# jbelyeu/unfazed

Hardware: AMD Instinct MI355X
Metric: phased DNMs/sec (higher is better)
Workload: dtype u8/int32 (+f64 allele balance); 1 GPU; 100k synthetic SNV/INDEL DNMs, whole-genome sites VCF, --no-extended off (BASELINE configs[2]); staged: H2D of the pre-decoded columns inside the timed region; dnms_per_gpu=100000, sites=20000000, coverage=30x, search_dist=5000, dnm_placement=uniform, read_clusters=67821, alignment_records=186931612, parallelism=dnm-shard x1, no collective

## Files before the change

include/unfazed_hip.h:

```cpp
#ifndef UNFAZED_HIP_H
#define UNFAZED_HIP_H

#include <stddef.h>
#include <stdint.h>

#include "uz_types.h"
#include "uz_bamwalk.h"

#ifdef __cplusplus
extern "C" {
#endif

#define UZ_E_ARG (-1)
#define UZ_E_HIP (-2)
#define UZ_E_NODEVICE (-3)
#define UZ_E_STATE (-4)
#define UZ_E_RANGE (-5)

#define UZ_FIND_WHOLE_REGION 1
#define UZ_FIND_SECOND_WINDOW 2

#define UZ_K_SITE_SCAN 0
#define UZ_K_WINDOW_COUNT 1
#define UZ_K_WINDOW_FILL 2
// ... 22 lines not shown

typedef struct uz_ctx uz_ctx;

int uz_create(int device, uz_ctx **out);
void uz_destroy(uz_ctx *ctx);
const char *uz_last_error(const uz_ctx *ctx);
int uz_sync(uz_ctx *ctx);
int uz_set_params(uz_ctx *ctx, const uz_params *p);

int uz_sites_upload(uz_ctx *ctx, const uz_sites_view *sites, int *sites_id);
int uz_family_upload(uz_ctx *ctx, int sites_id, const uz_family_view *fam, int *fam_id);
int uz_sites_family_upload_async(uz_ctx *ctx, const uz_sites_view *sites, const uz_family_view *fam, int *sites_id, int *fam_id);
int uz_samples_upload(uz_ctx *ctx, int sites_id, const uz_samples_view *samples, int *samples_id);
int uz_families_from_samples(uz_ctx *ctx, int samples_id, int32_t n, const int32_t *kid, const int32_t *dad, const int32_t *mom, int *fam_ids );
int uz_family_fetch(uz_ctx *ctx, int fam_id, uint8_t *gt, uint16_t *cols );
int uz_samples_from_text(uz_ctx *ctx, int sites_id, const uz_vcf_text_view *text, int32_t n_pick, const int32_t *pick, int *samples_id, int64_t *n_unsettled);
int uz_samples_from_bcf(uz_ctx *ctx, int sites_id, const uz_vcf_bcf_view *bcf, int32_t n_pick, const int32_t *pick, int *samples_id, int64_t *n_unsettled);
int uz_samples_unsettled(uz_ctx *ctx, int samples_id, int64_t *site );
int uz_samples_settle(uz_ctx *ctx, int samples_id, int64_t n, const int64_t *site, const uz_samples_view *cells);
int uz_samples_free(uz_ctx *ctx, int samples_id);
int uz_reads_upload(uz_ctx *ctx, const uz_reads_view *reads, int *reads_id);
int uz_reads_upload_packed(uz_ctx *ctx, const uz_reads_packed_view *reads, int *reads_id);
int uz_reads_wait(uz_ctx *ctx, int reads_id);
int uz_reads_headers(uz_ctx *ctx, int reads_id, int32_t *start, int32_t *end, int32_t *tlen, int32_t *mate, uint32_t *qname);
int uz_reads_columns(uz_ctx *ctx, int reads_id, int64_t sizes[4], uint32_t *fm, uint16_t *l_seq, uint16_t *n_cigar, uint32_t *cigar_off, uint32_t *sq_off,
                     uint32_t *qoff, uint32_t *cigar, uint8_t *seq4, uint32_t *qlow);
int uz_reads_marks(uz_ctx *ctx, int reads_id, uint16_t *umask, uint8_t *nlow);
int uz_bgzf_inflate(uz_ctx *ctx, const uint8_t *comp, int64_t comp_bytes, int64_t n_blocks, const int64_t *in_off, const int64_t *out_off,
                    uint8_t *out, int repeat, double *kernel_ms);
int uz_bgzf_inflate_to_host(uz_ctx *ctx, const uint8_t *comp, int64_t comp_bytes, int64_t n_blocks, const int64_t *in_off, const int64_t *out_off,
                            uint8_t *out);
int uz_bam_walk(uz_ctx *ctx, const uint8_t *comp, int64_t comp_bytes, int64_t n_blocks, const int64_t *in_off, const int64_t *out_off, const int64_t *blk_coff,
                const uint32_t *blk_crc ,
                int32_t n_tasks, const int32_t *task, int64_t n_spans, const int64_t *span, int64_t n_reach, const int32_t *reach, int64_t n_fetch,
                const int32_t *fetch, int *walk_id, int64_t *n_desc);
#define UZ_HEAD_NONE 0
#define UZ_HEAD_DONE 1
#define UZ_HEAD_END 2
#define UZ_HEAD_BAD 3
int uz_head_walk(uz_ctx *ctx, int *head_id, int32_t n_files, const uint8_t *comp, int64_t comp_bytes, int64_t n_blocks, const int64_t *in_off,
                 const int32_t *isize, const uint32_t *crc, const int64_t *blk_first, const int64_t *start, const int64_t *want, const int64_t *have,
                 int64_t *taken, int64_t *cursor, int32_t *state);
int uz_head_rank(uz_ctx *ctx, int head_id, int32_t readlen, const int64_t *k, uint32_t *a, uint32_t *b);
int uz_head_fetch(uz_ctx *ctx, int head_id, int32_t file, int32_t *out, int64_t cap, int64_t *n);
int uz_head_free(uz_ctx *ctx, int head_id);
int uz_crc32_blocks(uz_ctx *ctx, const uint8_t *data, int64_t n_blocks, const int64_t *off, const uint32_t *want, int64_t *first_bad);
int uz_bam_walk_many(uz_ctx *ctx, const uint8_t *comp, int64_t comp_bytes, int64_t n_blocks, const int64_t *in_off, const int64_t *out_off, const int64_t *blk_coff,
                     const uint32_t *blk_crc, int32_t n_tasks, const int32_t *task, int64_t n_spans, const int64_t *span, int64_t n_reach, const int32_t *reach,
                     int64_t n_fetch, const int32_t *fetch, int32_t n_files, const int64_t *file_base, const int32_t *ref_base, const uint64_t *salt1,
                     const uint32_t *salt2, int *walk_id, int64_t *n_desc);
int uz_reads_files(uz_ctx *ctx, int reads_id, int32_t n_files, const int32_t *ref_base, int64_t *rec_first, int64_t *name_first);
int uz_bam_walk_fetch(uz_ctx *ctx, int walk_id, uz_walk_desc *desc, int64_t *d_first, int32_t *d_flags, int64_t *d_walked);
int uz_bam_walk_release(uz_ctx *ctx, int walk_id);
int uz_bam_walk_flags(uz_ctx *ctx, int walk_id, int32_t *d_flags, int64_t *d_walked);
int uz_bam_join(uz_ctx *ctx, int walk_id, int32_t n_host, const int32_t *h_flags, int32_t n_ref, int all_bases, const uz_walk_desc *xdesc, int64_t n_x, const uint8_t *xaux,
                int64_t xaux_bytes, const int32_t *look_tid, int64_t n_look, const int32_t *need_jtask, int64_t *n_need, int64_t totals[8]);
int uz_bam_join_needs(uz_ctx *ctx, int walk_id, uz_need_rec *need);
int uz_bam_join_fetch(uz_ctx *ctx, int walk_id, uint64_t *voff, uint32_t *qname, int32_t *mate, uint8_t *bases, uz_kept_rec *kept, int64_t *contig_off, int32_t *max_span);
int uz_reads_from_walk(uz_ctx *ctx, int walk_id, int32_t min_base_qual, int want_names, int *reads_id, int64_t totals[8]);
int uz_reads_names(uz_ctx *ctx, int reads_id, const uint32_t *ids, int64_t n, int64_t *off ,
                   const uint8_t **bytes );
int uz_walk_slot_stats(uz_ctx *ctx, int64_t out[8]);
int uz_walk_reserve(uz_ctx *ctx, int n_slots);
int uz_reads_from_bam(uz_ctx *ctx, int walk_id, const uz_kept_rec *kept, int64_t n, const uint8_t *aux, int64_t aux_bytes, const int64_t *contig_off,
                      const int32_t *max_span, int32_t n_contigs, int64_t n_cigar_total, int64_t n_row_units, int64_t n_seq_units, uint32_t n_qnames,
                      int32_t min_base_qual, uint8_t *names_out ,
                      int64_t names_bytes, int *reads_id);
int uz_pinned_alloc(size_t bytes, void **out);
void uz_pinned_free(void *p);
int uz_sites_adopt_device(uz_ctx *ctx, const uz_sites_view *sites, int *sites_id);
int uz_family_adopt_device(uz_ctx *ctx, int sites_id, const uz_family_view *fam, int *fam_id);
int uz_reads_adopt_device(uz_ctx *ctx, const uz_reads_packed_view *reads, int *reads_id);
int uz_drop_derived(uz_ctx *ctx);
int uz_sites_free(uz_ctx *ctx, int sites_id);
int uz_reads_free(uz_ctx *ctx, int reads_id);

int uz_site_scan(uz_ctx *ctx, int fam_id);
int uz_site_scan_many(uz_ctx *ctx, const int32_t *fam_ids, int32_t n_fam);
int uz_site_classes(uz_ctx *ctx, int fam_id, uint8_t *cls_out );

int uz_find(uz_ctx *ctx, int fam_id, const uz_dnms_view *dnms, int mode,
            int64_t *cand_off , int64_t *het_off );
int uz_find_fetch(uz_ctx *ctx, int32_t *cand_idx, uint8_t *cand_flags, int32_t *het_idx);
int uz_find_cohort(uz_ctx *ctx, const uz_cohort_group *groups, int32_t n_groups, const uz_dnms_view *dnms, int mode,
                   int64_t *cand_off , int64_t *het_off );

int uz_phase(uz_ctx *ctx, int fam_id, int reads_id, const uz_dnms_view *dnms, int find_mode,
             int32_t *status , int32_t *counts ,
             int32_t *origin , int32_t *evidence );
int uz_phase_begin(uz_ctx *ctx, int fam_id, int reads_id, const uz_dnms_view *dnms, int find_mode);
int uz_phase_end(uz_ctx *ctx, int fam_id, int reads_id, const uz_dnms_view *dnms, int find_mode,
                 int32_t *status, int32_t *counts, int32_t *origin, int32_t *evidence);
int uz_phase_cohort(uz_ctx *ctx, const uz_cohort_group *groups, int32_t n_groups, const uz_dnms_view *dnms, int find_mode,
                    int32_t *status, int32_t *counts, int32_t *origin, int32_t *evidence);
int uz_phase_cohort_joined(uz_ctx *ctx, int reads_id, const uz_cohort_group *groups, int32_t n_groups, const int32_t *group_ref_base, const uz_dnms_view *dnms,
                           int find_mode, int32_t *status, int32_t *counts, int32_t *origin, int32_t *evidence);
int uz_phase_votes(uz_ctx *ctx, int64_t *vote_off , int32_t *vote_val);
int uz_phase_groups(uz_ctx *ctx, int64_t *grp_off , int32_t *grp_q);
#define UZ_SIZING_REDUCED_WORDS 263
int uz_phase_sizing_fetch(uz_ctx *ctx, int32_t *bounds , int32_t *pre_win , int32_t *pre_ha ,
                          int32_t *pre_hl , int64_t *reduced );

int uz_bed_rows(uz_ctx *ctx, const uz_bed_view *rows, int verbose, int include_ambiguous, int64_t *off , const uint8_t **bytes);
int uz_bed_rows_lists(uz_ctx *ctx, const uz_bed_view *rows, int verbose, int include_ambiguous, int32_t n_dnms, const int32_t *status,
                      const int64_t *list_off, const int32_t *list_val, uint32_t n_qnames, const uint32_t *name_off, const uint8_t *name_bytes,
                      int32_t evidence_min_ratio, int64_t *off , const uint8_t **bytes);

int uz_vcf_rows(uz_ctx *ctx, const uz_vcf_text_view *text, const int64_t *line_at , const int64_t *ann_off ,
                const int32_t *ann_col, const uint8_t *ann_gt, const int32_t *ann_uops, const int8_t *ann_uet, int64_t *off ,
                const uint8_t **bytes, uint8_t *handed_back );

int uz_bcf_rows(uz_ctx *ctx, const uz_bcf_lines_view *records, int64_t *off , uint64_t *samp_at ,
                const uint8_t **bytes, uint8_t *handed_back );

int uz_bgzf_deflate(uz_ctx *ctx, const uint8_t *data , int64_t n_bytes, int64_t *n_blocks, const uint8_t **bgzf, int64_t *bgzf_bytes,
                    int repeat, double *kernel_ms);

int uz_phase_cnv(uz_ctx *ctx, int fam_id, const uz_dnms_view *dnms, const int32_t *rb_counts, int32_t *cnv_counts ,
                 int32_t *origin , int32_t *evidence , int32_t *etype );
int uz_phase_cnv_cohort(uz_ctx *ctx, const uz_cohort_group *groups, int32_t n_groups, const uz_dnms_view *dnms, const int32_t *rb_counts,
                        int32_t *cnv_counts , int32_t *origin , int32_t *evidence , int32_t *etype );
int uz_phase_cnv_sites(uz_ctx *ctx, int64_t *off , int32_t *pos);

int uz_prof_enable(uz_ctx *ctx, int on);
int uz_prof_reset(uz_ctx *ctx);
int uz_prof_get(uz_ctx *ctx, int kernel, double *total_ms, int64_t *launches);
int uz_prof_units(uz_ctx *ctx, int kernel, int64_t *units);

#ifdef __cplusplus
}
#endif
#endif
```

unfazed_amd/csrc/abi.hip:

```cpp
#include "uz_ctx.hpp"

#include <chrono>
#include <algorithm>
#include <map>
#include <mutex>

void uz_fold_complex(uz_ctx *c, uint8_t *gt, const uint8_t *sflags, int64_t n);
bool uz_site_scan_fresh(const uz_ctx *c, const FamilyDev &f, bool need_cnv);

namespace {

void set_error(uz_ctx *c, const std::string &msg) {
    std::lock_guard<std::mutex> lk(c->err_mu);
    c->err = msg;
}

template <typename F>
int guarded(uz_ctx *c, F &&fn) {
    if (!c) return UZ_E_ARG;
    try {
        (void)hipSetDevice(c->device);
        fn();
        return 0;
    } catch (const UzError &e) {
        set_error(c, e.msg);
        return e.code;
    } catch (const std::exception &e) {
        set_error(c, e.what());
        return UZ_E_ARG;
    } catch (...) {
        set_error(c, "unknown error");
        return UZ_E_ARG;
    }
}

static std::mutex g_pinned_mu;
static std::map<uintptr_t, size_t> g_pinned;
static bool inside_one_pinned_block(const uint8_t *lo, const uint8_t *hi) {
    std::lock_guard<std::mutex> g(g_pinned_mu);
    auto it = g_pinned.upper_bound((uintptr_t)lo);
    if (it == g_pinned.begin()) return false;
    --it;
    return (uintptr_t)lo >= it->first && (uintptr_t)hi <= it->first + it->second;
}

struct SlabPlan {
    int mode = 1;
    const uint8_t *lo = nullptr, *hi = nullptr;
    size_t sum = 0;
    std::vector<const uint8_t *> at;
    uint8_t *dev = nullptr;
    void add(const void *p, size_t bytes) {
        const uint8_t *q = (const uint8_t *)p;
        if (!lo || q < lo) lo = q;
        if (!hi || q + bytes > hi) hi = q + bytes;
        sum += bytes;
        at.push_back(q);
    }
    size_t span() const { return (size_t)(hi - lo); }
    bool worth() const {
        if (at.size() < 2 || span() > sum + sum / 8 + 1024 * at.size()) return false;
        for (const uint8_t *q : at)
            if ((size_t)(q - lo) % 256) return false;
        return inside_one_pinned_block(lo, hi);
    }
};
static thread_local SlabPlan *g_slab = nullptr;
struct SlabScope {
    explicit SlabScope(SlabPlan *p) { g_slab = p; }
    ~SlabScope() { g_slab = nullptr; }
};
static const bool g_slab_off = getenv("UZ_NO_SLAB_COPY") != nullptr;

template <typename T>
const T *h2d(hipStream_t st, T *dst, const T *host, size_t n) {
    if (n) {
        UZ_REQUIRE(host != nullptr, UZ_E_ARG, "null column pointer");
        if (g_slab && g_slab->mode == 1) { g_slab->add(host, n * sizeof(T)); return dst; }
        if (g_slab && g_slab->mode == 2) return reinterpret_cast<const T *>(g_slab->dev + ((const uint8_t *)host - g_slab->lo));
        UZ_HIP(hipMemcpyAsync(dst, host, n * sizeof(T), hipMemcpyHostToDevice, st));
    }
    return dst;
}
// ... 43 lines not shown

void free_family(uz_ctx *c, FamilyDev &f) {
    if (f.ready) { (void)hipEventSynchronize(f.ready); (void)hipEventDestroy(f.ready); f.ready = nullptr; }
    f.pending = false;
    if (f.samples_id >= 0 && f.samples_id < (int)c->samples.size()) c->samples[(size_t)f.samples_id].live_fams--;
    uz_block_put(c, f.block);
    uz_block_put(c, f.wide_block);
    f = FamilyDev();
}
void free_samples(uz_ctx *c, SamplesDev &m) {
    if (m.ready) { (void)hipEventSynchronize(m.ready); (void)hipEventDestroy(m.ready); }
    uz_block_put(c, m.block);
    uz_block_put(c, m.wide_block);
    for (DevBlock &b : m.fam_blocks) uz_block_put(c, b);
    m = SamplesDev();
}
SamplesDev &samples_of(uz_ctx *c, int id) {
    UZ_REQUIRE(id >= 0 && id < (int)c->samples.size() && c->samples[id].live, UZ_E_ARG, "unknown sample table handle");
    return c->samples[id];
}
void free_sites(uz_ctx *c, SitesDev &s) {
    if (s.ready) { (void)hipEventSynchronize(s.ready); (void)hipEventDestroy(s.ready); }
    uz_block_put(c, s.block);
    uz_block_put(c, s.mirror);
    s = SitesDev();
}
void free_reads(uz_ctx *c, ReadsDev &r) {
    if (r.built) { (void)hipEventSynchronize(r.built); (void)hipEventDestroy(r.built); }
    if (r.ready) (void)hipEventDestroy(r.ready);
    uz_block_put(c, r.block);
    uz_block_put(c, r.mirror);
    r = ReadsDev();
}

struct Carver {
    uint8_t *base;
    size_t off = 0;
    explicit Carver(uint8_t *b) : base(b) {}
    template <typename T>
    T *take(size_t n) {
        off = (off + 255) & ~(size_t)255;
        T *p = base ? reinterpret_cast<T *>(base + off) : nullptr;
        off += (n ? n : 1) * sizeof(T) + 64;
        return p;
    }
};

template <typename F>
void samples_from_records(uz_ctx *c, int sites_id, int64_t n_sites, int32_t n_pick, int *id, int64_t *n_unsettled, F parse) {
    size_t chunk = (size_t)32 << 20;
    if (const char *e = getenv("UZ_VCF_CHUNK_BYTES")) {
        const long long v = atoll(e);
        if (v > 0) chunk = (size_t)v;
    }
    chunk = std::min<size_t>(chunk, (size_t)1 << 31);
    const size_t n = (size_t)n_sites, ns = (size_t)n_pick;
    SamplesDev m;
    m.live = true; m.sites_id = sites_id; m.n_samples = n_pick; m.n_wide = 0;
    m.stride = (n + 64 + 255) & ~(size_t)255;
    for (int pass = 0; pass < 2; pass++) {
        Carver cv(pass ? m.block.p : nullptr);
        m.gt = cv.take<uint8_t>(ns * m.stride);
        m.rd = cv.take<uint16_t>(ns * m.stride); m.ad = cv.take<uint16_t>(ns * m.stride); m.gq = cv.take<uint16_t>(ns * m.stride);
        if (!pass) m.block = uz_block_get(c, cv.off + 256);
    }
    try {
        parse(m, chunk);
    } catch (...) { uz_block_put(c, m.block); throw; }
    m.need_settle = !m.unsettled.empty();
    *n_unsettled = (int64_t)m.unsettled.size();
    const int k = new_slot(c->samples);
    c->samples[(size_t)k] = m;
    *id = k;
}

}

template <typename W>
__global__ __launch_bounds__(256) void k_copy(W *__restrict__ dst, const W *__restrict__ src, size_t n) {
    for (size_t i = (size_t)blockIdx.x * 256 + threadIdx.x; i < n; i += (size_t)gridDim.x * 256) dst[i] = src[i];
}
void uz_kcopy(uz_ctx *c, void *dst, const void *src, size_t bytes) {
    if (!bytes) return;
    const uintptr_t a = (uintptr_t)dst | (uintptr_t)src | (uintptr_t)bytes;
    auto grid = [](size_t n) { return dim3((unsigned)std::min<size_t>((n + 255) / 256, 1024)); };
    if (a % 16 == 0) hipLaunchKernelGGL(k_copy<uint4>, grid(bytes / 16), dim3(256), 0, c->stream, (uint4 *)dst, (const uint4 *)src, bytes / 16);
    else if (a % 4 == 0) hipLaunchKernelGGL(k_copy<uint32_t>, grid(bytes / 4), dim3(256), 0, c->stream, (uint32_t *)dst, (const uint32_t *)src, bytes / 4);
    else hipLaunchKernelGGL(k_copy<uint8_t>, grid(bytes), dim3(256), 0, c->stream, (uint8_t *)dst, (const uint8_t *)src, bytes);
    UZ_HIP(hipGetLastError());
}

__global__ __launch_bounds__(1024) void k_scan_len(int64_t n, const uint32_t *__restrict__ len, uint32_t add, int64_t *__restrict__ off) {
    __shared__ unsigned long long wave_sum[16];
    __shared__ unsigned long long carry_s;
    const uint32_t t = threadIdx.x, l = t & 63u, wv = t >> 6;
    if (t == 0) carry_s = 0;
    __syncthreads();
    for (int64_t base = 0; base < n; base += 1024) {
        const int64_t i = base + t;
        const unsigned long long v = i < n ? (unsigned long long)len[i] + add : 0ull;
        unsigned long long x = v;
#pragma unroll
        for (uint32_t d = 1; d < 64; d <<= 1) {
            const unsigned long long y = (unsigned long long)__shfl_up((long long)x, d, 64);
            if (l >= d) x += y;
        }
        if (l == 63) wave_sum[wv] = x;
        __syncthreads();
        unsigned long long before = carry_s;
        for (uint32_t k = 0; k < wv; k++) before += wave_sum[k];
        if (i < n) off[i] = (int64_t)(before + x - v);
        __syncthreads();
        if (t == 1023) carry_s = before + x;
        __syncthreads();
    }
    if (t == 0) off[n] = (int64_t)carry_s;
}
void uz_len_scan(uz_ctx *c, hipStream_t st, int64_t n, const uint32_t *len, uint32_t add, int64_t *off) {
    hipLaunchKernelGGL(k_scan_len, dim3(1), dim3(1024), 0, st, n, len, add, off);
    UZ_HIP(hipGetLastError());
}

DevBlock uz_block_get(uz_ctx *c, size_t bytes) {
    int best = -1;
    for (size_t i = 0; i < c->block_pool.size(); i++)
        if (c->block_pool[i].cap >= bytes && (best < 0 || c->block_pool[i].cap < c->block_pool[best].cap)) best = (int)i;
    if (best >= 0 && c->block_pool[best].cap <= 2 * bytes + (1 << 20)) {
        DevBlock b = c->block_pool[best];
        c->block_pool.erase(c->block_pool.begin() + best);
        return b;
    }
    DevBlock b;
    b.cap = bytes + bytes / 16 + 4096;
    UZ_HIP(hipMalloc((void **)&b.p, b.cap));
    return b;
}
void uz_block_put(uz_ctx *c, DevBlock b) {
    if (!b.p) return;
    c->block_pool.push_back(b);
    while (c->block_pool.size() > 64) {
        size_t k = 0;
        for (size_t i = 1; i < c->block_pool.size(); i++)
            if (c->block_pool[i].cap < c->block_pool[k].cap) k = i;
        (void)hipFree(c->block_pool[k].p);
        c->block_pool.erase(c->block_pool.begin() + k);
    }
}

void uz_prof_begin(uz_ctx *c, int kernel, hipEvent_t *a, hipEvent_t *b) {
    *a = *b = nullptr;
    if (!(c->prof_mask >> kernel & 1u)) return;
    for (hipEvent_t *e : {a, b}) {
        if (!c->event_pool.empty()) { *e = c->event_pool.back(); c->event_pool.pop_back(); }
        else UZ_HIP(hipEventCreate(e));
    }
    UZ_HIP(hipEventRecord(*a, c->stream));
}
void uz_prof_end(uz_ctx *c, int kernel, hipEvent_t a, hipEvent_t b) {
    if (!a) return;
    (void)hipEventRecord(b, c->stream);
    c->prof_pending.push_back(ProfPending{kernel, a, b});
}
void uz_prof_drain(uz_ctx *c) {
    for (auto &p : c->prof_pending) {
        float ms = 0;
        if (hipEventSynchronize(p.b) == hipSuccess && hipEventElapsedTime(&ms, p.a, p.b) == hipSuccess) {
            c->prof[p.kernel].total_ms += ms;
            c->prof[p.kernel].launches += 1;
        }
        c->event_pool.push_back(p.a);
        c->event_pool.push_back(p.b);
// ... 1453 lines not shown
        std::lock_guard<std::mutex> g(g_pinned_mu);
        g_pinned.erase((uintptr_t)p);
    }
    (void)hipHostFree(p);
}

int uz_drop_derived(uz_ctx *c) {
    return guarded(c, [&] {
        for (auto &f : c->fams) f.cls_valid = false;
        find_forget(c, -1);
    });
}

int uz_sites_free(uz_ctx *c, int sites_id) {
    return guarded(c, [&] {
        SitesDev &s = sites_of(c, sites_id);
        UZ_HIP(hipStreamSynchronize(c->stream));
        for (size_t k = 0; k < c->fams.size(); k++)
            if (c->fams[k].live && c->fams[k].sites_id == sites_id) { find_forget(c, (int)k); free_family(c, c->fams[k]); }
        for (auto &m : c->samples)
            if (m.live && m.sites_id == sites_id) free_samples(c, m);
        free_sites(c, s);
    });
}
int uz_reads_free(uz_ctx *c, int reads_id) {
    return guarded(c, [&] {
        ReadsDev &r = reads_of(c, reads_id);
        if (r.ready) UZ_HIP(hipEventSynchronize(r.ready));
        if (r.built) UZ_HIP(hipEventSynchronize(r.built));
        UZ_HIP(hipStreamSynchronize(c->stream));
        const bool member = std::find(c->cohort_ids.begin(), c->cohort_ids.end(), reads_id) != c->cohort_ids.end();
        if (reads_id == c->cohort_reads) { c->cohort_reads = -1; c->cohort_ids.clear(); }
        else if (member && c->cohort_reads >= 0) {
            free_reads(c, c->reads[(size_t)c->cohort_reads]);
            c->cohort_reads = -1;
            c->cohort_ids.clear();
        }
        free_reads(c, r);
    });
}

int uz_site_scan(uz_ctx *c, int fam_id) {
    return guarded(c, [&] {
        FamilyDev &f = fam_of(c, fam_id);
        uz_launch_site_scan(c, f, sites_of(c, f.sites_id), !f.het_only);
    });
}

int uz_site_scan_many(uz_ctx *c, const int32_t *fam_ids, int32_t n_fam) {
    return guarded(c, [&] {
        UZ_REQUIRE(n_fam >= 0 && (n_fam == 0 || fam_ids != nullptr), UZ_E_ARG, "bad family list");
        if (n_fam == 0) return;
        std::vector<FamilyDev *> fams;
        for (int32_t k = 0; k < n_fam; k++) {
            FamilyDev &f = fam_of(c, fam_ids[k]);
            refuse_het_only(f, "uz_site_scan_many");
            UZ_REQUIRE(f.sites_id == fam_of(c, fam_ids[0]).sites_id, UZ_E_ARG, "the families of one cohort scan must share a sites table");
            for (int32_t j = 0; j < k; j++) UZ_REQUIRE(fam_ids[j] != fam_ids[k], UZ_E_ARG, "family listed twice");
            fams.push_back(&f);
        }
        uz_launch_site_scan_many(c, fams.data(), n_fam, sites_of(c, fams[0]->sites_id), true);
    });
}

int uz_site_classes(uz_ctx *c, int fam_id, uint8_t *out) {
    return guarded(c, [&] {
        FamilyDev &f = fam_of(c, fam_id);
        SitesDev &s = sites_of(c, f.sites_id);
        UZ_REQUIRE(out != nullptr, UZ_E_ARG, "null output");
        const bool cnv = !f.het_only;
        if (!uz_site_scan_fresh(c, f, cnv)) uz_launch_site_scan(c, f, s, cnv);
        if (s.n) UZ_HIP(hipMemcpyAsync(out, f.cls, (size_t)s.n, hipMemcpyDeviceToHost, c->stream));
        UZ_HIP(hipStreamSynchronize(c->stream));
        if (f.het_only) uz_check_upload_flag(c);
    });
}

int uz_find(uz_ctx *c, int fam_id, const uz_dnms_view *d, int mode, int64_t *cand_off, int64_t *het_off) {
    return guarded(c, [&] {
        FamilyDev &f = fam_of(c, fam_id);
        SitesDev &s = sites_of(c, f.sites_id);
        UZ_REQUIRE(d != nullptr && d->n >= 0, UZ_E_ARG, "bad DNM view");
        c->phase_valid = false;
        const bool cnv = (mode & UZ_FIND_WHOLE_REGION) != 0;
        if (cnv) refuse_het_only(f, "a whole-region find");
        if (!uz_site_scan_fresh(c, f, cnv)) uz_launch_site_scan(c, f, s, cnv);
        uz_stage_dnms(c, d);
        const FindKey key = find_key_of(c, fam_id, mode, d);
        find_target(c);
        uz_launch_find(c, f, s, mode);
        if (f.het_only) uz_check_upload_flag(c);
        find_done(c, key);
        c->find_fam = fam_id;
        if (cand_off) memcpy(cand_off, c->cand_off_h.data(), ((size_t)d->n + 1) * sizeof(int64_t));
        if (het_off) memcpy(het_off, c->het_off_h.data(), ((size_t)d->n + 1) * sizeof(int64_t));
    });
}

int uz_find_fetch(uz_ctx *c, int32_t *cand_idx, uint8_t *cand_flags, int32_t *het_idx) {
    return guarded(c, [&] {
        UZ_REQUIRE(c->find_valid, UZ_E_STATE, "uz_find_fetch before uz_find");
        const bool pinned = (!cand_idx || !c->n_cand || inside_one_pinned_block((const uint8_t *)cand_idx, (const uint8_t *)(cand_idx + c->n_cand))) &&
                            (!cand_flags || !c->n_cand || inside_one_pinned_block(cand_flags, cand_flags + c->n_cand)) &&
                            (!het_idx || !c->n_het || inside_one_pinned_block((const uint8_t *)het_idx, (const uint8_t *)(het_idx + c->n_het)));
        if (pinned) {
            if (cand_idx && c->n_cand) uz_kcopy(c, cand_idx, c->cand_idx.p, (size_t)c->n_cand * sizeof(int32_t));
            if (cand_flags && c->n_cand) uz_kcopy(c, cand_flags, c->cand_flags.p, (size_t)c->n_cand);
            if (het_idx && c->n_het) uz_kcopy(c, het_idx, c->het_idx.p, (size_t)c->n_het * sizeof(int32_t));
            UZ_HIP(hipStreamSynchronize(c->stream));
            return;
        }
        if (cand_idx && c->n_cand)
            UZ_HIP(hipMemcpyAsync(cand_idx, c->cand_idx.p, (size_t)c->n_cand * sizeof(int32_t), hipMemcpyDeviceToHost, c->stream));
        if (cand_flags && c->n_cand)
            UZ_HIP(hipMemcpyAsync(cand_flags, c->cand_flags.p, (size_t)c->n_cand, hipMemcpyDeviceToHost, c->stream));
        if (het_idx && c->n_het)
            UZ_HIP(hipMemcpyAsync(het_idx, c->het_idx.p, (size_t)c->n_het * sizeof(int32_t), hipMemcpyDeviceToHost, c->stream));
        UZ_HIP(hipStreamSynchronize(c->stream));
    });
}

static void phase_whole(uz_ctx *c, int fam_id, int reads_id, const uz_dnms_view *d, int find_mode, int32_t *status, int32_t *counts, int32_t *origin,
                        int32_t *evidence, bool defer) {
    FamilyDev &f = fam_of(c, fam_id);
    SitesDev &s = sites_of(c, f.sites_id);
    ReadsDev &r = reads_of(c, reads_id);
    UZ_REQUIRE(d != nullptr, UZ_E_ARG, "null DNM view");
    UZ_REQUIRE(!(find_mode & UZ_FIND_WHOLE_REGION), UZ_E_ARG, "the read stage runs on SNV / breakpoint windows");
    c->phase_valid = false;
    c->phase_qbase.clear();
    static const bool trace = getenv("UZ_PHASE_HOST_TRACE") != nullptr;
    const auto t0 = std::chrono::steady_clock::now();
    auto us = [&] { return std::chrono::duration<double, std::micro>(std::chrono::steady_clock::now() - t0).count(); };
    if (!uz_site_scan_fresh(c, f, false)) uz_launch_site_scan(c, f, s, false);
    const double t_scan0 = us();
    uz_stage_dnms(c, d);
    const double t_stage0 = us() - t_scan0, t_scan = us();
    const FindKey key = find_key_of(c, fam_id, find_mode, d);
    const double t_key = us() - t_scan, t_stage = us();
    const bool have = find_recall(c, key);
    if (!have) find_target(c);
    if (!have) {
        uz_launch_find(c, f, s, find_mode, false);
        find_done(c, key);
    }
    const double t_find = us();
    c->find_fam = fam_id;
    uz_launch_phase(c, f, s, r, status, counts, origin, evidence, defer);
    if (trace) fprintf(stderr, "[uz] read-stage call, host us: site scan queued %.0f | stage dnms %.0f | key %.0f | find %.0f | phase (launches, waits, results) %.0f\n", t_scan0,
                       t_stage0, t_key, t_find - t_stage, us() - t_find);
}
int uz_phase(uz_ctx *c, int fam_id, int reads_id, const uz_dnms_view *d, int find_mode, int32_t *status,
             int32_t *counts, int32_t *origin, int32_t *evidence) {
    return guarded(c, [&] {
        UZ_REQUIRE(!c->phase_open, UZ_E_STATE, "uz_phase: a batch is still open (uz_phase_end)");
        phase_whole(c, fam_id, reads_id, d, find_mode, status, counts, origin, evidence, false);
    });
}
int uz_phase_begin(uz_ctx *c, int fam_id, int reads_id, const uz_dnms_view *d, int find_mode) {
    return guarded(c, [&] {
        UZ_REQUIRE(!c->phase_open, UZ_E_STATE, "uz_phase_begin: the batch before this one is still open (uz_phase_end)");
        phase_whole(c, fam_id, reads_id, d, find_mode, nullptr, nullptr, nullptr, nullptr, true);
        c->phase_open = true;
    });
}
int uz_phase_end(uz_ctx *c, int fam_id, int reads_id, const uz_dnms_view *d, int find_mode, int32_t *status, int32_t *counts, int32_t *origin,
                 int32_t *evidence) {
    return guarded(c, [&] {
        UZ_REQUIRE(c->phase_open, UZ_E_STATE, "uz_phase_end without uz_phase_begin");
        c->phase_open = false;
        if (uz_finish_phase(c, status, counts, origin, evidence)) return;
        phase_whole(c, fam_id, reads_id, d, find_mode, status, counts, origin, evidence, false);
    });
}

struct CohortMode {
    uz_ctx *c;
    explicit CohortMode(uz_ctx *c_) : c(c_) { c->cohort_on = true; }
    ~CohortMode() { c->cohort_on = false; }
};
struct ZeroSearchDist {
    uz_ctx *c;
    const int32_t sd;
    explicit ZeroSearchDist(uz_ctx *c_) : c(c_), sd(c_->P.search_dist) { c->P.search_dist = 0; }
    ~ZeroSearchDist() { c->P.search_dist = sd; }
};

struct CohortBatch {
    const uz_cohort_group *groups = nullptr; int32_t n_groups = 0;
    const uz_dnms_view *d = nullptr; bool cnv = false;
    FamilyDev *f0 = nullptr; SitesDev *s = nullptr;
    std::vector<int32_t> fam;
    std::vector<uint8_t *> cls;
    std::vector<FamilyDev *> stale;
};

static CohortBatch cohort_batch(uz_ctx *c, const uz_cohort_group *groups, int32_t n_groups, const uz_dnms_view *d, bool cnv) {
    UZ_REQUIRE(groups && n_groups > 0 && d && d->n >= 0, UZ_E_ARG, "bad cohort batch");
    CohortBatch b;
    b.groups = groups; b.n_groups = n_groups; b.d = d; b.cnv = cnv;
    b.f0 = &fam_of(c, groups[0].fam_id);
// ... 618 lines not shown
```

unfazed_amd/csrc/k_reads.hip:

```cpp
#include "uz_ctx.hpp"
#include "phase_body.hpp"

#include <algorithm>
#include <chrono>
#include <cstdio>
#include <cstdlib>

#define UZ_TRACE(name) do { if (getenv("UZ_TRACE")) { (void)hipStreamSynchronize(c->stream); fprintf(stderr, "[uz] before %s\n", name); fflush(stderr); } } while (0)

namespace {


#ifndef UZ_BW_LANES
#define UZ_BW_LANES 16
#endif
#ifndef UZ_BW_MIN_WAVES
#define UZ_BW_MIN_WAVES 1
#endif
#ifndef UZ_BW_STAGE
#define UZ_BW_STAGE 64
#endif
template <int GL, typename F>
__device__ __forceinline__ int32_t grp_lower_bound(F ld, int32_t a, int32_t b, int32_t v, int lane, int gbase) {
    constexpr int SH = GL == 64 ? 6 : GL == 32 ? 5 : GL == 16 ? 4 : GL == 8 ? 3 : GL == 4 ? 2 : GL == 2 ? 1 : 0;
    const unsigned long long gmask = GL == 64 ? ~0ull : ((1ull << GL) - 1ull);
    while (a < b) {
        const int32_t chunk = ((b - a) + GL - 1) >> SH;
        const int32_t q = a + lane * chunk;
        const bool below = q < b && ld(q) < v;
        const int cnt = __popcll((__ballot(below) >> gbase) & gmask);
        const int32_t a0 = a;
        if (cnt > 0) a = a0 + (cnt - 1) * chunk + 1;
        if (cnt < GL && a0 + cnt * chunk < b) b = a0 + cnt * chunk;
    }
    return a;
}
__global__ __launch_bounds__(256, UZ_BW_MIN_WAVES) void k_phase_bounds(PhaseArgs a, int32_t *bounds ) {
    constexpr int GL = UZ_BW_LANES, NCH = 2 * UZ_BW_SITES;
    static_assert(GL == 1 || GL == 2 || GL == 4 || GL == 8 || GL == 16 || GL == 32 || GL == 64, "a group is a power of two inside a wavefront");
    __shared__ int32_t s_stage[256 / GL][UZ_BW_STAGE];
    const int64_t g = ((int64_t)blockIdx.x * blockDim.x + threadIdx.x) / GL;
    const int lane = threadIdx.x & (GL - 1), gbase = (threadIdx.x & 63) & ~(GL - 1);
    const int d = g < a.n ? (int)g : a.n - 1;
    long long tp = 0;
    int mh = 0;
    int32_t *b = bounds + 5 * (size_t)d;
    if (g < a.n) {
        const int nc = (int)(a.cand_off[d + 1] - a.cand_off[d]), nh = (int)(a.het_off[d + 1] - a.het_off[d]);
        if (lane == 0) {
            b[0] = b[1] = b[4] = 0;
            b[2] = nh; b[3] = nc;
            for (int k = 0; k < 4; k++) a.pre_win[4 * d + k] = 0;
        }
        const RD &R = a.R;
        const int tid = a.rcontig[d];
        const bool tid_ok = tid >= 0 && tid < R.n_contigs;
        const int32_t clo = tid_ok ? (int32_t)R.contig_off[tid] : 0, chi = tid_ok ? (int32_t)R.contig_off[tid + 1] : 0;
        if (nc > 0 && (!R.mid || !tid_ok || chi - clo <= 128)) {
            uz_phase_bounds_w(a, d, b, lane, GL, tp, mh,
                              [&R, clo, chi](const long long (&v)[NCH], const bool (&on)[NCH], long long (&r)[NCH]) { uz_lower_bounds_c<NCH>(R, clo, chi, v, on, r); });
        } else if (nc > 0) {
            const long long span = R.max_span[tid];
            const bool point = a.vartype[d] == UZ_VT_POINT;
            long long vmin_ = 0x7FFFFFFFLL;
            if (point) {
                const long long position = a.dstart[d];
                vmin_ = ((a.dflags[d] & UZ_DF_FETCH_FALLBACK) ? position : position - 1) - span;
            }
            if (!a.no_extended && nh > 0) {
                const long long v0 = (long long)a.spos[a.het_idx[a.het_off[d]]] - span;
                if (v0 < vmin_) vmin_ = v0;
            }
            const int32_t vmin = uz_clamp_i32(vmin_);
            int32_t lo0 = clo, hi0 = chi;
            if (R.coarse && chi - clo > 8192) {
                const int32_t kl = (clo + 4095) >> 12, kh = chi >> 12;
                const int32_t *cx = R.coarse;
                const int32_t a0 = grp_lower_bound<GL>([cx](int32_t k) { return cx[k]; }, kl, kh > kl ? kh : kl, vmin, lane, gbase);
                if (kh > kl) { lo0 = a0 > kl ? ((a0 - 1) << 12) : clo; hi0 = a0 < kh ? (a0 << 12) : chi; }
            }
            const int32_t *mx = R.mid;
            const int32_t kl_m = (clo + 63) >> 6, kh_m = chi >> 6;
            const int32_t ml = (lo0 + 63) >> 6, mhi = hi0 >> 6;
            int32_t lo1 = lo0;
            if (mhi > ml) {
                const int32_t m0 = grp_lower_bound<GL>([mx](int32_t k) { return mx[k]; }, ml, mhi, vmin, lane, gbase);
                if (m0 > ml) lo1 = (m0 - 1) << 6;
            }
            int32_t s0 = (lo1 + 63) >> 6;
            if (s0 < kl_m) s0 = kl_m;
            int32_t s_end = s0 + UZ_BW_STAGE < kh_m ? s0 + UZ_BW_STAGE : kh_m;
            if (s_end < s0) s_end = s0;
            const int32_t cnt = s_end - s0;
            int32_t *sm = s_stage[threadIdx.x / GL];
            for (int i = lane; i < cnt; i += GL) sm[i] = mx[s0 + i];
            __builtin_amdgcn_fence(__ATOMIC_RELEASE, "wavefront");
            __builtin_amdgcn_wave_barrier();
            __builtin_amdgcn_fence(__ATOMIC_ACQUIRE, "wavefront");
            const bool whole = s_end == kh_m;
            uz_phase_bounds_w(a, d, b, lane, GL, tp, mh, [&R, clo, chi, sm, s0, cnt, lo1, whole](const long long (&v_)[NCH], const bool (&on)[NCH], long long (&r)[NCH]) {
                int32_t x[NCH], y[NCH], v[NCH];
                bool far[NCH], any_far = false;
#pragma unroll
                for (int s = 0; s < NCH; s++) { v[s] = uz_clamp_i32(v_[s]); x[s] = 0; y[s] = on[s] ? cnt : 0; }
                uz_lb_level<NCH>([sm](int32_t k) { return sm[k]; }, x, y, v, 0);
#pragma unroll
                for (int s = 0; s < NCH; s++) {
                    const int32_t k = x[s];
                    far[s] = on[s] && k == cnt && !whole;
                    any_far |= far[s];
                    x[s] = k > 0 ? ((s0 + k - 1) << 6) : lo1;
                    y[s] = (on[s] && !far[s]) ? (k < cnt ? ((s0 + k) << 6) : chi) : x[s];
                    if (!on[s]) x[s] = y[s] = clo;
                }
                if (R.mid8) uz_mid8_refine<NCH>(R.mid8, x, y, v);
                const RecA *rx = R.ra;
                uz_lb_level<NCH>([rx](int32_t k) { return rx[k].start; }, x, y, v, clo);
#pragma unroll
                for (int s = 0; s < NCH; s++) r[s] = x[s];
                if (any_far) {
                    long long rf[NCH];
                    uz_lower_bounds_c<NCH>(R, clo, chi, v_, far, rf);
#pragma unroll
                    for (int s = 0; s < NCH; s++) if (far[s]) r[s] = rf[s];
                }
            });
        }
    }
#pragma unroll
    for (int o = GL >> 1; o > 0; o >>= 1) {
        tp += __shfl_xor(tp, o, GL);
        const int m2 = __shfl_xor(mh, o, GL);
        mh = m2 > mh ? m2 : mh;
    }
    if (g < a.n && lane == 0) {
        b[1] = (int32_t)(tp > 0x7FFFFFF0LL ? 0x7FFFFFF0LL : tp);
        b[4] = mh;
    }
}

#ifndef UZ_PHASE_PARTS
#define UZ_PHASE_PARTS 8
#endif
#ifndef UZ_PHASE_MIN_WAVES
#define UZ_PHASE_MIN_WAVES 4
#endif
template <bool LDS>
__global__ __launch_bounds__(WG_NT, LDS ? UZ_PHASE_MIN_WAVES : 5) void k_phase(PhaseArgs a_by_value) {
    __shared__ WgSharedT<LDS ? 1 : WG_SORT_LDS_CAP> sh;
    extern __shared__ __attribute__((aligned(16))) uint8_t uz_lds_arena[];
    (void)a_by_value;
    const PhaseArgsK ap = (PhaseArgsK)__builtin_amdgcn_kernarg_segment_ptr();
    uint8_t *const scr_base = uz_g(ap->scratch) + (size_t)blockIdx.x * ap->scratch_per_wg;
#ifdef UZ_PHASE_TIMING
    if (threadIdx.x < 24) sh.tick[threadIdx.x] = 0;
    struct TickFlush {
        decltype(sh) *s; unsigned long long *t;
        __device__ ~TickFlush() { __syncthreads(); if (threadIdx.x < 24 && s->tick[threadIdx.x]) atomicAdd(&t[threadIdx.x], s->tick[threadIdx.x]); }
    } tick_flush{&sh, uz_g(ap->timing)};
#endif
    const bool from_list = ap->from_list != 0;
    int part = from_list ? ap->cursor_slot : (int)(blockIdx.x % UZ_PHASE_PARTS);
    int tried = 0;
    for (;;) {
        __syncthreads();
        if (threadIdx.x == 0) {
            const int k = atomicAdd(uz_g(ap->work_cursor) + 16 * part, 1);
            if (from_list) sh.bcast[0] = k < *uz_g(ap->src_count) ? uz_g(ap->src_list)[k] : -1;
            else {
                const int n = ap->n;
                const int lo = (int)((long long)n * part / UZ_PHASE_PARTS), hi = (int)((long long)n * (part + 1) / UZ_PHASE_PARTS);
                sh.bcast[0] = lo + k < hi ? lo + k : -1;
            }
        }
        __syncthreads();
        const int d = sh.bcast[0];
        if (d < 0) {
            if (from_list || ++tried >= UZ_PHASE_PARTS) break;
            part = (part + 1) % UZ_PHASE_PARTS;
            continue;
        }
        if (uz_phase_dnm<LDS>(ap, scr_base, &sh, LDS ? uz_lds_arena : nullptr, d)) {
            if (threadIdx.x == 0) uz_g(ap->retry_list)[atomicAdd(uz_g(ap->retry_count), 1)] = d;
        }
    }
}

struct PhaseState {
    DevBuf<uint8_t> scratch;
    DevBuf<int32_t> bounds, bounds_red, res, cursor, pool, list_len, pre_win, pre_h, retry;
    DevBuf<long long> list_start;
    unsigned long long *pool_cursor = nullptr;
    DevBuf<unsigned int> need_count;
    int32_t *bounds_h = nullptr;
    size_t bounds_h_cap = 0;
    int32_t *res_h = nullptr;
    size_t res_h_cap = 0;
    bool spec_valid = false;
    Caps spec_caps = {0, 0, 0, 0, 0, 0};
    int spec_arena = 0, spec_arena2 = 0;
    double spec_sumP_per_dnm = 0.0;
    long long spec_runs = 0, spec_misses = 0;
    hipEvent_t bounds_ready = nullptr;
    int n_cus = 0;
    std::vector<long long> list_start_h;
    std::vector<int32_t> list_len_h;
    bool have_lists = false;
    int32_t n = 0;
    int64_t n_het = 0;
    bool pending = false;
    Caps pend_caps = {0, 0, 0, 0, 0, 0};
    size_t pend_pool_cap = 0;
    int pend_want_lists = 0;
    bool force_exact = false;
};

RD make_rd(const ReadsDev &r) {
    RD R;
    R.ra = (const RecA *)r.rec_a; R.rb = (const RecB *)r.rec_b; R.fm = r.fm;
    R.contig_off = r.contig_off; R.max_span = r.max_span; R.n_contigs = r.n_contigs;
    R.cigar = r.cigar; R.seq4 = r.seq4; R.qlow = r.qlow; R.qoff = r.qoff; R.nlow = r.nlow; R.umask = r.umask; R.qs = r.qs; R.min_map_qual = 0; R.coarse = r.coarse; R.mid = r.mid; R.mid8 = r.mid8;
    R.err = nullptr;
    return R;
}

int next_pow2(long long v) {
    long long p = 1;
    while (p < v) p <<= 1;
    return (int)p;
}

}

void uz_phase_state_free(uz_ctx *c) {
    PhaseState *st = (PhaseState *)c->phase_state;
// ... 49 lines not shown
            left &= ~m;
        }
        bin = -1;
    }
    for (int o = 32; o > 0; o >>= 1) {
        mA = max(mA, __shfl_xor(mA, o, 64)); mT = max(mT, __shfl_xor(mT, o, 64)); mH = max(mH, __shfl_xor(mH, o, 64)); mC = max(mC, __shfl_xor(mC, o, 64));
        mM = max(mM, __shfl_xor(mM, o, 64)); sumP += __shfl_xor(sumP, o, 64); active += __shfl_xor(active, o, 64);
    }
    const int w = threadIdx.x >> 6;
    if ((threadIdx.x & 63) == 0) {
        part[w][0] = (unsigned long long)mA; part[w][1] = (unsigned long long)mT; part[w][2] = (unsigned long long)mH; part[w][3] = (unsigned long long)mC;
        part[w][4] = (unsigned long long)mM; part[w][5] = (unsigned long long)sumP; part[w][6] = (unsigned long long)active;
    }
    __syncthreads();
    if (threadIdx.x == 0) {
        unsigned long long r[7];
        for (int k = 0; k < 7; k++) { r[k] = part[0][k]; for (int q = 1; q < 4; q++) r[k] = k < 5 ? max(r[k], part[q][k]) : r[k] + part[q][k]; }
        atomicMax(&out->mA, (int32_t)r[0]); atomicMax(&out->mT, (int32_t)r[1]); atomicMax(&out->mH, (int32_t)r[2]); atomicMax(&out->mC, (int32_t)r[3]);
        atomicMax(&out->mM, r[4]); atomicAdd(&out->sumP, r[5]); atomicAdd(&out->active, (int32_t)r[6]);
    }
    if (hist[threadIdx.x]) atomicAdd(&out->hist[threadIdx.x], hist[threadIdx.x]);
}
static Sizes phase_exact_sizes(const BoundsRed *br, int32_t n) {
    const long long mA = br->mA, mT = br->mT, mH = br->mH, mC = br->mC, mM = (long long)br->mM, sumP = (long long)br->sumP;
    Sizes z;
    z.caps.A = (int32_t)mA; z.caps.T = (int32_t)mT; z.caps.H = (int32_t)mH; z.caps.C = (int32_t)mC;
    z.caps.I = (int32_t)(4 * mA);
    z.caps.M = next_pow2(std::min<long long>(std::max<long long>(mM, 2), 1 << 20));
    z.sumP = sumP;
    z.arena = arena_env;
    if (z.arena < 0) {
        const int32_t *hist = br->hist;
        const int32_t active = br->active;
        int u = 16, seen = 0, umax = 16;
        for (int k = 0; k < 256; k++) if (hist[k]) umax = k;
        for (int k = 0; k < 256; k++) {
            seen += hist[k];
            if (hist[k]) u = std::max(u, k);
            if ((long long)seen * 1000 >= (long long)active * arena_permille) break;
        }
        z.arena = std::min(u * 256, 62 * 1024);
        z.arena2 = std::min(std::max(2 * z.arena, umax * 256 + 1024), 62 * 1024);
    } else
        z.arena2 = std::min(2 * z.arena, 62 * 1024);
    return z;
}

void uz_launch_phase(uz_ctx *c, FamilyDev &f, const SitesDev &s, ReadsDev &r, int32_t *status, int32_t *counts,
                     int32_t *origin, int32_t *evidence, bool defer) {
    if (!c->phase_state) c->phase_state = new PhaseState();
    PhaseState *st = (PhaseState *)c->phase_state;
    const int32_t n = c->dn.n;
    st->n = n;
    st->have_lists = false;
    st->pending = false;
    c->phase_n = n;
    if (n <= 0) { c->phase_valid = true; return; }
    static const bool host_trace = getenv("UZ_PHASE_HOST_TRACE") != nullptr;
    const auto host_t0 = std::chrono::steady_clock::now();
    auto host_us = [&] { return std::chrono::duration<double, std::micro>(std::chrono::steady_clock::now() - host_t0).count(); };
    double t_queued = 0, t_synced = 0, t_sized = 0;
    uz_reads_ready_for_threshold(c, r, "the reads table");

    PhaseArgs a;
    memset(&a, 0, sizeof(a));
    a.n = n;
    a.min_gt_qual = c->P.min_gt_qual; a.readlen = c->P.readlen; a.no_extended = c->P.no_extended;
    a.read_goal = c->P.read_goal; a.evidence_min_ratio = c->P.evidence_min_ratio; a.split_error_margin = c->P.split_error_margin;
    a.cutoff = c->dn.cutoff;
    a.cutoff_d = c->cohort_on ? c->dn_cutoff.p : nullptr;
    a.spos = s.pos; a.sref = s.ref_base; a.salt = s.alt_base;
    a.cand_off = c->cand_off.p; a.het_off = c->het_off.p;
    a.cand_idx = c->cand_idx.p; a.het_idx = c->het_idx.p; a.cand_flags = c->cand_flags.p;
    a.rcontig = c->dn.rcontig.p; a.dstart = c->dn.start.p; a.dend = c->dn.end.p; a.dflags = c->dn.dflags.p; a.vartype = c->dn.vartype.p;
    a.allele_off = c->dn.allele_off.p; a.alleles = c->dn.alleles.p;
    a.R = make_rd(r);
    a.R.err = c->hflags + 1;
    a.R.min_map_qual = c->P.min_map_qual;

    st->bounds.ensure((size_t)5 * n);
    st->pre_win.ensure((size_t)4 * n); st->pre_h.ensure(2 * ((size_t)c->n_het + 1));
    a.pre_win = st->pre_win.p; a.pre_ha = st->pre_h.p; a.pre_hl = st->pre_h.p + (size_t)c->n_het + 1;
    st->n_het = c->n_het;
    UZ_HIP(hipMemsetAsync(st->pre_h.p, 0, 2 * ((size_t)c->n_het + 1) * sizeof(int32_t), c->stream));
    {
        const unsigned nb = (unsigned)(((int64_t)n * UZ_BW_LANES + 255) / 256);
        ProfScope ps(c, UZ_K_SIZING);
        UZ_TRACE("k_phase_bounds");
        hipLaunchKernelGGL(k_phase_bounds, dim3(nb), dim3(256), 0, c->stream, a, st->bounds.p);
        UZ_HIP(hipGetLastError());
    }
    if (st->bounds_h_cap < sizeof(BoundsRed) / sizeof(int32_t)) {
        if (st->bounds_h) (void)hipHostFree(st->bounds_h);
        st->bounds_h = nullptr;
        st->bounds_h_cap = sizeof(BoundsRed) / sizeof(int32_t) + 64;
        UZ_HIP(hipHostMalloc((void **)&st->bounds_h, st->bounds_h_cap * sizeof(int32_t), hipHostMallocDefault));
    }
    st->bounds_red.ensure(sizeof(BoundsRed) / sizeof(int32_t) + 16);
    UZ_HIP(hipMemsetAsync(st->bounds_red.p, 0, sizeof(BoundsRed), c->stream));
    hipLaunchKernelGGL(k_bounds_reduce, dim3((unsigned)std::max(1, std::min(UZ_BR_BLOCKS, (n + 255) / 256))), dim3(256), 0, c->stream, (const int32_t *)st->bounds.p, n,
                       reinterpret_cast<BoundsRed *>(st->bounds_red.p));
    UZ_HIP(hipGetLastError());
    const BoundsRed *const bh_own = reinterpret_cast<const BoundsRed *>(st->bounds_h);
    uz_kcopy(c, st->bounds_h, st->bounds_red.p, sizeof(BoundsRed));
    if (!st->bounds_ready) UZ_HIP(hipEventCreateWithFlags(&st->bounds_ready, hipEventDisableTiming));
    UZ_HIP(hipEventRecord(st->bounds_ready, c->stream));
    auto check_upload_flags = [&] { uz_check_upload_flag(c); };
    auto exact_sizes = [&](const BoundsRed *bh) { return phase_exact_sizes(bh, n); };
    if (st->n_cus <= 0) {
        hipDeviceProp_t prop;
        UZ_HIP(hipGetDeviceProperties(&prop, c->device));
        st->n_cus = prop.multiProcessorCount;
    }
    static const bool no_spec = getenv("UZ_PHASE_NO_SPEC") != nullptr;
    const bool hooks = getenv("UZ_TEST_CAP_T") || getenv("UZ_TEST_PHASE_ARENA");
    bool speculative = st->spec_valid && !no_spec && !hooks && !st->force_exact;
    st->force_exact = false;
    const size_t res_ints = (size_t)7 * n + ((7 * (size_t)n) & 1);
    st->res.ensure(res_ints + 4);
    st->pool_cursor = (unsigned long long *)(st->res.p + res_ints);
    st->cursor.ensure(16 * (UZ_PHASE_PARTS + 2) + 32);
    st->retry.ensure(2 * ((size_t)n + 16));
    int32_t *const retry1_list = st->retry.p, *const retry2_list = st->retry.p + (size_t)n + 16;
    int32_t *const retry1 = st->cursor.p + 16 * (UZ_PHASE_PARTS + 2), *const retry2 = retry1 + 16;
    a.retry_count = retry1; a.retry_list = retry1_list;
    a.from_list = 0; a.cursor_slot = 0; a.src_count = nullptr; a.src_list = nullptr;
    a.status = st->res.p; a.counts = st->res.p + n; a.origin = st->res.p + (size_t)5 * n; a.evidence = st->res.p + (size_t)6 * n;
    a.work_cursor = st->cursor.p;
    a.want_lists = uz_want_lists;
    st->list_start.ensure(n); st->list_len.ensure((size_t)6 * n);
    a.pool_cursor = st->pool_cursor;
    a.list_start = st->list_start.p; a.list_len = st->list_len.p;
#ifdef UZ_PHASE_TIMING
    static DevBuf<unsigned long long> timing;
    timing.ensure(32);
    UZ_HIP(hipMemsetAsync(timing.p, 0, 32 * sizeof(unsigned long long), c->stream));
    a.timing = timing.p;
#endif
    {
        const size_t need = (size_t)7 * n + 16;
        if (st->res_h_cap < need) {
            if (st->res_h) (void)hipHostFree(st->res_h);
            st->res_h = nullptr;
            st->res_h_cap = need + (size_t)n;
            UZ_HIP(hipHostMalloc((void **)&st->res_h, st->res_h_cap * sizeof(int32_t), hipHostMallocDefault));
        }
    }
    int32_t *const hres = st->res_h;
    unsigned long long *const hused = (unsigned long long *)(hres + (size_t)7 * n + ((7 * (size_t)n) & 1));
    for (int round = 0; round < 2; round++) {
        Sizes z;
        if (speculative) {
            z.caps = st->spec_caps; z.arena = st->spec_arena; z.arena2 = st->spec_arena2;
            z.sumP = (long long)(st->spec_sumP_per_dnm * (double)n) + 4096;
        } else {
            UZ_HIP(hipEventSynchronize(st->bounds_ready));
            check_upload_flags();
            z = exact_sizes(bh_own);
            if (const char *e = getenv("UZ_TEST_CAP_T")) {
                const int32_t t = (int32_t)atoi(e);
                if (t < z.caps.T) z.caps.T = t;
            }
        }
        const Caps caps = z.caps;
        int arena_used = z.arena;
        ScrOff so_hbm;
        const size_t per_wg = uz_scratch_layout(caps, a.so, true), per_wg_hbm = uz_scratch_layout(caps, so_hbm, false);
        if (const char *e = getenv("UZ_TEST_PHASE_ARENA")) {
            const int t = atoi(e);
            if (t >= 0 && t < arena_used) arena_used = t;
        }
        int wgs_per_cu;
        {
            static const int wgs_env = [] { const char *e = getenv("UZ_PHASE_WGS_PER_CU"); return e ? atoi(e) : 0; }();
            const int by_lds = (160 * 1024) / (arena_used + (int)sizeof(WgSharedT<1>) + 512);
            const int by_regs = UZ_PHASE_MIN_WAVES * 4 / (WG_NT / 64);
            wgs_per_cu = wgs_env > 0 ? wgs_env : std::max(1, std::min(by_lds, by_regs));
            if (arena_env < 0 && wgs_env <= 0) {
                const int room = ((160 * 1024) / wgs_per_cu - (int)sizeof(WgSharedT<1>) - 512) & ~255;
                if (room > arena_used && !getenv("UZ_TEST_PHASE_ARENA")) arena_used = std::min(room, 62 * 1024);
            }
        }
        a.lds_arena_bytes = arena_used;
        int grid = st->n_cus * wgs_per_cu;
        if (grid > n) grid = n;
        const size_t budget = (size_t)8 << 30;
        while (grid > 1 && (size_t)grid * per_wg > budget) grid /= 2;
        int grid_hbm = std::min(grid, 8 * st->n_cus);
        while (grid_hbm > 1 && (size_t)grid_hbm * per_wg_hbm > budget) grid_hbm /= 2;
        st->scratch.ensure(std::max((size_t)grid * per_wg, (size_t)grid_hbm * per_wg_hbm));
        a.scratch = st->scratch.p; a.scratch_per_wg = per_wg; a.caps = caps;
        size_t pool_cap = (size_t)std::min<long long>(4 * z.sumP + 1024, (long long)1 << 31);
        st->pool.ensure(pool_cap);
        a.pool = st->pool.p; a.pool_cap = pool_cap;
        for (int attempt = 0; attempt < 4; attempt++) {
            UZ_HIP(hipMemsetAsync(st->cursor.p, 0, (16 * (UZ_PHASE_PARTS + 2) + 32) * sizeof(int32_t), c->stream));
            UZ_HIP(hipMemsetAsync(st->pool_cursor, 0, 2 * sizeof(unsigned long long), c->stream));
            {
                ProfScope ps(c, UZ_K_PHASE);
                UZ_TRACE("k_phase");
                hipLaunchKernelGGL((k_phase<true>), dim3((unsigned)grid), dim3(WG_NT), (size_t)a.lds_arena_bytes, c->stream, a);
                UZ_HIP(hipGetLastError());
                PhaseArgs a2 = a;
                a2.from_list = 1; a2.cursor_slot = UZ_PHASE_PARTS; a2.src_count = retry1; a2.src_list = retry1_list;
                a2.retry_count = retry2; a2.retry_list = retry2_list;
                a2.lds_arena_bytes = getenv("UZ_TEST_PHASE_ARENA") ? arena_used
                                                                    : std::max(arena_used, std::min(z.arena2, 62 * 1024));
                const int per_cu2 = std::max(1, (160 * 1024) / (a2.lds_arena_bytes + (int)sizeof(WgSharedT<1>) + 512));
                hipLaunchKernelGGL((k_phase<true>), dim3((unsigned)std::min(grid, per_cu2 * st->n_cus)), dim3(WG_NT), (size_t)a2.lds_arena_bytes, c->stream, a2);
                UZ_HIP(hipGetLastError());
                PhaseArgs a3 = a2;
                a3.cursor_slot = UZ_PHASE_PARTS + 1; a3.src_count = retry2; a3.src_list = retry2_list;
                a3.so = so_hbm; a3.scratch_per_wg = per_wg_hbm;
                hipLaunchKernelGGL((k_phase<false>), dim3((unsigned)grid_hbm), dim3(WG_NT), 0, c->stream, a3);
                UZ_HIP(hipGetLastError());
            }
            UZ_TRACE("after k_phase");
            *hused = 0;
            uz_kcopy(c, hres, st->res.p, res_ints * sizeof(int32_t) + sizeof(unsigned long long));
            int32_t *const hretry = (int32_t *)(hused + 1);
            *hretry = 0;
            uz_kcopy(c, hretry, retry2, sizeof(int32_t));
            if (defer && speculative) {
                st->pending = true;
                st->pend_caps = caps; st->pend_pool_cap = a.pool_cap; st->pend_want_lists = a.want_lists;
                return;
            }
            if (host_trace) t_queued = host_us();
            UZ_HIP(hipStreamSynchronize(c->stream));
            if (host_trace) t_synced = host_us();
            if (speculative) check_upload_flags();
            if (c->hflags[1]) {
                const int f = c->hflags[1];
                c->hflags[1] = 0;
                throw UzError{UZ_E_STATE, f == 4 ? "the read stage asked for a base of a record whose bases were staged as a list (bl_*), and the list does not hold it: the fetch points that staged the table do not cover this batch"
                                        : f == 3 ? "the read stage asked for a base (or its quality bit) in a 32-base unit that was not staged (umask): the fetch points that staged the table do not cover this batch"
                                        : f == 2 ? "the read stage asked for a base-quality bit of a record staged without its quality row (more than 10 low-quality bases, or no bases): such a record can never pass goodread -- the staging rule and the kernel disagree"
                                                 : "the read stage asked for the bases of a record staged without them (UZ_AUX_NO_SEQ): the selection that staged the table does not cover this batch's fetches"};
            }
            const unsigned long long used = *hused;
            c->prof[UZ_K_PHASE].last_units = (int64_t)*(const int32_t *)(hused + 1);
            if (!a.want_lists || used <= a.pool_cap) break;
            pool_cap = (size_t)used + 1024;
            st->pool.ensure(pool_cap);
            a.pool = st->pool.p; a.pool_cap = pool_cap;
        }
        const Sizes real = exact_sizes(bh_own);
        if (host_trace) t_sized = host_us();
        auto room = [](int32_t v) { return (int32_t)std::min<long long>((long long)v + v / 8 + 8, 0x3FFFFFFF); };
        st->spec_caps.A = room(real.caps.A); st->spec_caps.T = room(real.caps.T); st->spec_caps.H = room(real.caps.H); st->spec_caps.C = room(real.caps.C);
        st->spec_caps.I = 4 * st->spec_caps.A;
        st->spec_caps.M = real.caps.M;
        st->spec_arena = real.arena; st->spec_arena2 = real.arena2;
        st->spec_sumP_per_dnm = 1.25 * (double)real.sumP / (double)n;
        st->spec_valid = true;
        static const bool spec_log = getenv("UZ_PHASE_SPEC_LOG") != nullptr;
        if (spec_log)
            fprintf(stderr, "[uz_launch_phase] n %d speculative %d caps A %d T %d H %d C %d M %d arena %d grid %d per_wg %zu pool %zu | real A %d T %d H %d C %d M %d arena %d\n", n,
                    (int)speculative, caps.A, caps.T, caps.H, caps.C, caps.M, arena_used, grid, per_wg, pool_cap, real.caps.A, real.caps.T, real.caps.H, real.caps.C, real.caps.M, real.arena);
        if (!speculative) break;
        const bool fits = real.caps.A <= caps.A && real.caps.T <= caps.T && real.caps.H <= caps.H && real.caps.C <= caps.C && real.caps.M <= caps.M;
        st->spec_runs++;
        if (fits) break;
        st->spec_misses++;
        speculative = false;
    }
#ifdef UZ_PHASE_TIMING
    {
        unsigned long long t[32];
        UZ_HIP(hipMemcpy(t, timing.p, sizeof(t), hipMemcpyDeviceToHost));
        const char *nm[17] = {"A.classify", "A.lists+C", "-", "B.overlap", "B.finish", "S.keys", "S.sort", "P.count", "P.scatter", "P.pairs", "D.finder",
                              "E.setup", "E.expand", "E.winners", "E.frontier", "F.join", "F.count"};
        unsigned long long tot = 0;
        for (int k = 0; k < 17; k++) tot += t[k];
        fprintf(stderr, "[phase timing]");
        for (int k = 0; k < 17; k++) fprintf(stderr, " %s %.1f%%", nm[k], 100.0 * (double)t[k] / (double)(tot ? tot : 1));
        fprintf(stderr, " | ticks/DNM %.0f\n", (double)tot / n);
    }
#endif
    if (status) memcpy(status, hres, (size_t)n * sizeof(int32_t));
    if (counts) memcpy(counts, hres + n, (size_t)4 * n * sizeof(int32_t));
    if (origin) memcpy(origin, hres + (size_t)5 * n, (size_t)n * sizeof(int32_t));
    if (evidence) memcpy(evidence, hres + (size_t)6 * n, (size_t)n * sizeof(int32_t));
    st->have_lists = a.want_lists != 0;
    c->phase_valid = true;
    if (host_trace)
        fprintf(stderr, "[uz] uz_launch_phase, host us: everything queued %.0f | waited for the device %.0f | exact sizes %.0f | results copied out %.0f\n", t_queued, t_synced - t_queued,
                t_sized - t_synced, host_us() - t_sized);
}

bool uz_finish_phase(uz_ctx *c, int32_t *status, int32_t *counts, int32_t *origin, int32_t *evidence) {
    PhaseState *st = (PhaseState *)c->phase_state;
    UZ_REQUIRE(st != nullptr, UZ_E_STATE, "uz_phase_end without uz_phase_begin");
    const int32_t n = st->n;
    if (n <= 0) { c->phase_valid = true; return true; }
    int32_t *const hres = st->res_h;
    if (st->pending) {
        st->pending = false;
        UZ_HIP(hipStreamSynchronize(c->stream));
        uz_check_upload_flag(c);
        if (c->hflags[1]) {
            c->hflags[1] = 0;
            st->force_exact = true;
            return false;
        }
// ... 104 lines not shown
```

unfazed_amd/csrc/k_sites.hip:

```cpp
#include "uz_ctx.hpp"

#include <algorithm>
#include <cstdlib>
#include <vector>

namespace {

struct SiteParams {
    int32_t min_gt_qual, min_depth;
    double lo_ref, hi_ref, lo_het, hi_het, lo_alt, hi_alt;
};

__device__ __forceinline__ int dec16(uint32_t v) { return (int)(int16_t)(uint16_t)v; }

#define UZ_AB_T_MIN (-2)
#define UZ_AB_T_MAX 65534
#define UZ_AB_LUT_N (UZ_AB_T_MAX - UZ_AB_T_MIN + 1)
#define UZ_AB_A_MIN (-1)
#define UZ_AB_A_MAX 32767
__device__ __forceinline__ double ab_lo(const SiteParams &P, int gt) { return gt == UZ_HOM_REF ? P.lo_ref : (gt == UZ_HOM_ALT ? P.lo_alt : P.lo_het); }
__device__ __forceinline__ double ab_hi(const SiteParams &P, int gt) { return gt == UZ_HOM_REF ? P.hi_ref : (gt == UZ_HOM_ALT ? P.hi_alt : P.hi_het); }

#define UZ_AB_LDS_T 512
__global__ void k_build_ab_lut(SiteParams P, int2 *lut, uint32_t *small, int *t0_special) {
    const int i = blockIdx.x * blockDim.x + threadIdx.x;
    if (i >= 4 * UZ_AB_LUT_N) return;
    const int gt = i / UZ_AB_LUT_N, t = i % UZ_AB_LUT_N + UZ_AB_T_MIN;
    const double lo = ab_lo(P, gt), hi = ab_hi(P, gt);
    int2 r = make_int2(0x7FFFFFFF, -0x7FFFFFFF);
    if (gt != UZ_GT_UNKNOWN && t >= P.min_depth) {
        if (t > 0) {
            int l = UZ_AB_A_MIN, h = UZ_AB_A_MAX + 1;
            while (l < h) { const int m = l + ((h - l) >> 1); if (lo <= (double)m / (double)t) h = m; else l = m + 1; }
            const int amin = l;
            l = UZ_AB_A_MIN - 1; h = UZ_AB_A_MAX;
            while (l < h) { const int m = l + ((h - l + 1) >> 1); if ((double)m / (double)t <= hi) l = m; else h = m - 1; }
            if (amin <= UZ_AB_A_MAX && l >= UZ_AB_A_MIN) r = make_int2(amin, l);
        } else if (t < 0) {
            int amin = 0x7FFFFFFF, amax = -0x7FFFFFFF;
            for (int a = -1; a <= 0; a++) {
                const double ab = (double)a / (double)t;
                if (lo <= ab && ab <= hi) { if (a < amin) amin = a; if (a > amax) amax = a; }
            }
            r = make_int2(amin, amax);
        } else {
            const double pinf = 1.0 / 0.0, ninf = -1.0 / 0.0;
            const bool neg = lo <= ninf && ninf <= hi, pos = lo <= pinf && pinf <= hi;
            if (neg && pos) { r = make_int2(-1, 1); atomicOr(t0_special, 1); }
            else if (neg) r = make_int2(-1, -1);
            else if (pos) r = make_int2(1, 1);
        }
    }
    lut[i] = r;
    if (t - UZ_AB_T_MIN < UZ_AB_LDS_T) {
        const int lo16 = r.x > 32767 ? 32767 : r.x, hi16 = r.y < -32768 ? -32768 : r.y;
        small[gt * UZ_AB_LDS_T + (t - UZ_AB_T_MIN)] = ((uint32_t)lo16 & 0xFFFFu) | ((uint32_t)hi16 << 16);
    }
}

template <bool T0>
__device__ __forceinline__ bool hq(const SiteParams &P, const int2 *__restrict__ lut, const uint32_t *lds, int gt, int rd, int ad, int gq) {
    const int t = rd + ad;
    const uint32_t ti = (uint32_t)(t - UZ_AB_T_MIN);
    int amin, amax;
    if (ti < UZ_AB_LDS_T) {
        const uint32_t e = lds[gt * UZ_AB_LDS_T + ti];
        amin = (int)(int16_t)(e & 0xFFFFu);
        amax = (int)(int16_t)(e >> 16);
    } else {
        const int2 b = lut[gt * UZ_AB_LUT_N + ti];
        amin = b.x; amax = b.y;
    }
    bool ok = (gq >= P.min_gt_qual) & (ad >= amin) & (ad <= amax);
    if (T0) ok &= !((t == 0) & (ad == 0));
    return ok;
}

__device__ __forceinline__ bool hq_wide(const SiteParams &P, int gt, int rd, int ad, int gq) {
    if (gt == UZ_GT_UNKNOWN) return false;
    const long long t = (long long)rd + (long long)ad;
    if (gq < P.min_gt_qual || t < (long long)P.min_depth) return false;
    const double ab = (double)ad / (double)t;
    return ab_lo(P, gt) <= ab && ab <= ab_hi(P, gt);
// ... 319 lines not shown
                        }
                    }
                    nc += __popcll(bc); nh += __popcll(bh);
                }
                if (!FILL && lane == 0) { a.range[4 * (int64_t)d + 2 * k] = lo; a.range[4 * (int64_t)d + 2 * k + 1] = hi; }
            }
            nc *= mult; nh *= mult;
        }
    }
    if (!FILL && lane == 0) { cnt_c[d] = (int32_t)nc; cnt_h[d] = (int32_t)nh; }
}

template <bool FILL>
__global__ __launch_bounds__(256) void k_window_region(WinArgs a, int32_t *cnt_c, int32_t *cnt_h, const int64_t *off_c, const int64_t *off_h,
                                                       int32_t *cand_idx, uint8_t *cand_flags, int32_t *het_idx) {
    const int32_t d = (int32_t)(((int64_t)blockIdx.x * blockDim.x + threadIdx.x) >> 6);
    const int lane = threadIdx.x & 63;
    if (d >= a.n) return;
    if (FILL && (off_c[d + 1] > a.cap_c || off_h[d + 1] > a.cap_h)) return;
    int64_t nc = 0, nh = 0;
    const int32_t c = a.contig[d];
    const uint8_t *__restrict__ cls = a.fam_idx ? a.cls_of[a.fam_idx[d]] : a.cls;
    if (c >= 0 && c < a.n_contigs) {
        const int64_t clo = a.contig_off[c], chi = a.contig_off[c + 1];
        const int64_t st = a.start[d], en = a.end[d];
        int64_t w0 = st - a.sd;
        const int64_t w1 = en + a.sd;
        if (w0 < 1) w0 = 1;
        const int vt = a.vartype[d];
        const int mult = a.mult[d];
        const bool small_event = (en - st) < 20;
        int64_t lo, hi;
        if (FILL) { lo = a.range[4 * (int64_t)d]; hi = a.range[4 * (int64_t)d + 1]; }
        else {
            lo = lower_bound_wave(a.pos, clo, chi, w0 - 1, lane);
            hi = lower_bound_wave(a.pos, lo, chi, w1, lane);
            if (lane == 0) { a.range[4 * (int64_t)d] = lo; a.range[4 * (int64_t)d + 1] = hi; }
        }
        const int64_t oc = FILL ? off_c[d] : 0, oh = FILL ? off_h[d] : 0;
        const unsigned long long below = lane ? (~0ULL >> (64 - lane)) : 0ULL;
        for (int64_t b = lo; b < hi; b += 64) {
            const int64_t sidx = b + lane;
            bool is_c = false, is_h = false;
            uint32_t cl = 0, ka = 0;
            if (sidx < hi) {
                cl = cls[sidx];
                const int32_t p = a.pos[sidx];
                if (cl && !(small_event && p >= st && p < en)) {
                    if (vt == UZ_VT_DEL) ka = (cl >> UZ_CL_DEL_SHIFT) & 3;
                    else if (vt == UZ_VT_DUP) ka = (cl >> UZ_CL_DUP_SHIFT) & 3;
                    is_c = ka != 0;
                    is_h = (cl & UZ_CL_HET) != 0;
                }
            }
            const unsigned long long bc = __ballot(is_c), bh = __ballot(is_h);
            if (FILL) {
                if (is_h) for (int r = 0; r < mult; r++) het_idx[oh + (nh + __popcll(bh & below)) * mult + r] = (int32_t)sidx;
                if (is_c) {
                    const uint8_t fl = (uint8_t)(((cl & UZ_CL_ALT_DAD) ? UZ_CF_ALT_DAD : 0) | (ka << UZ_CF_KA_SHIFT));
                    for (int r = 0; r < mult; r++) {
                        const int64_t at = oc + (nc + __popcll(bc & below)) * mult + r;
                        cand_idx[at] = (int32_t)sidx;
                        cand_flags[at] = fl;
                    }
                }
            }
            nc += __popcll(bc); nh += __popcll(bh);
        }
        nc *= mult; nh *= mult;
    }
    if (!FILL && lane == 0) { cnt_c[d] = (int32_t)nc; cnt_h[d] = (int32_t)nh; }
}

__device__ __forceinline__ void scan2_load(int32_t n, int32_t i0, const int32_t *c0, const int32_t *c1, int (&v0)[4], int (&v1)[4]) {
    v0[0] = v0[1] = v0[2] = v0[3] = 0; v1[0] = v1[1] = v1[2] = v1[3] = 0;
    if (i0 + 3 < n) {
        const int4 a = *reinterpret_cast<const int4 *>(c0 + i0), b = *reinterpret_cast<const int4 *>(c1 + i0);
        v0[0] = a.x; v0[1] = a.y; v0[2] = a.z; v0[3] = a.w;
        v1[0] = b.x; v1[1] = b.y; v1[2] = b.z; v1[3] = b.w;
    } else {
        for (int k = 0; k < 4; k++) if (i0 + k < n) { v0[k] = c0[i0 + k]; v1[k] = c1[i0 + k]; }
    }
}
__global__ __launch_bounds__(1024) void k_scan2_sums(int32_t n, const int32_t *c0, const int32_t *c1, int64_t *part ) {
    __shared__ long long wsum[2][16];
    const int t = threadIdx.x, lane = t & 63, wv = t >> 6;
    int v0[4], v1[4];
    scan2_load(n, (int32_t)blockIdx.x * 4096 + 4 * t, c0, c1, v0, v1);
    long long s0 = (long long)v0[0] + v0[1] + v0[2] + v0[3], s1 = (long long)v1[0] + v1[1] + v1[2] + v1[3];
#pragma unroll
    for (int off = 32; off > 0; off >>= 1) { s0 += __shfl_xor(s0, off, 64); s1 += __shfl_xor(s1, off, 64); }
    if (lane == 0) { wsum[0][wv] = s0; wsum[1][wv] = s1; }
    __syncthreads();
    if (t < 2) {
        long long a = 0;
        for (int w = 0; w < 16; w++) a += wsum[t][w];
        part[2 * (size_t)blockIdx.x + t] = a;
    }
}
__global__ __launch_bounds__(1024) void k_scan2(int32_t n, const int32_t *c0, const int32_t *c1, const int64_t *__restrict__ part, int64_t *o0, int64_t *o1) {
    __shared__ int wsum[2][16];
    __shared__ long long csum[2][16];
    const int t = threadIdx.x, lane = t & 63, wv = t >> 6;
    const int32_t i0 = (int32_t)blockIdx.x * 4096 + 4 * t;
    int v0[4], v1[4];
    scan2_load(n, i0, c0, c1, v0, v1);
    long long q0 = 0, q1 = 0;
    for (int b = t; b < (int)blockIdx.x; b += 1024) { q0 += part[2 * (size_t)b]; q1 += part[2 * (size_t)b + 1]; }
#pragma unroll
    for (int off = 32; off > 0; off >>= 1) { q0 += __shfl_xor(q0, off, 64); q1 += __shfl_xor(q1, off, 64); }
    const int s0 = v0[0] + v0[1] + v0[2] + v0[3], s1 = v1[0] + v1[1] + v1[2] + v1[3];
    int in0 = s0, in1 = s1;
#pragma unroll
    for (int off = 1; off < 64; off <<= 1) {
        const int u0 = __shfl_up(in0, off, 64), u1 = __shfl_up(in1, off, 64);
        if (lane >= off) { in0 += u0; in1 += u1; }
    }
    if (lane == 63) { wsum[0][wv] = in0; wsum[1][wv] = in1; }
    if (lane == 0) { csum[0][wv] = q0; csum[1][wv] = q1; }
    __syncthreads();
    int64_t base0 = 0, base1 = 0, pre0 = 0, pre1 = 0, tot0 = 0, tot1 = 0;
#pragma unroll
    for (int w = 0; w < 16; w++) {
        const int a = wsum[0][w], b = wsum[1][w];
        if (w < wv) { pre0 += a; pre1 += b; }
        tot0 += a; tot1 += b;
        base0 += csum[0][w]; base1 += csum[1][w];
    }
    int64_t p0 = base0 + pre0 + (in0 - s0), p1 = base1 + pre1 + (in1 - s1);
    for (int k = 0; k < 4; k++) {
        if (i0 + k < n) { o0[i0 + k] = p0; o1[i0 + k] = p1; }
        p0 += v0[k]; p1 += v1[k];
    }
    if (t == 0 && blockIdx.x == gridDim.x - 1) { o0[n] = base0 + tot0; o1[n] = base1 + tot1; }
}

__global__ __launch_bounds__(256) void k_cnv_count(int32_t n, const int64_t *__restrict__ cand_off, const int32_t *__restrict__ cand_idx,
                                                   const uint8_t *__restrict__ cand_flags, const int32_t *__restrict__ spos,
                                                   const uint8_t *__restrict__ vartype, const int32_t *__restrict__ rb_counts, int ratio,
                                                   int32_t *cnv_counts, int32_t *cnv_pos, int32_t *origin, int32_t *evidence, int32_t *etype) {
    const int32_t d = (int32_t)(((int64_t)blockIdx.x * blockDim.x + threadIdx.x) >> 6);
    const int lane = threadIdx.x & 63;
    if (d >= n) return;
    const int64_t c0 = cand_off[d], c1 = cand_off[d + 1];
    const int vt = vartype[d];
    const bool cnv = vt == UZ_VT_DEL || vt == UZ_VT_DUP;
    int n_dad = 0, n_mom = 0;
    if (cnv) {
        for (int64_t b = c0; b < c1; b += 64) {
            const int64_t i = b + lane;
            bool dad = false, mom = false;
            if (i < c1) {
                const uint32_t fl = cand_flags[i];
                const uint32_t ka = (fl >> UZ_CF_KA_SHIFT) & 3u;
                const bool alt_dad = (fl & UZ_CF_ALT_DAD) != 0;
                const bool is_dad = (ka == UZ_KA_ALT_PARENT) == alt_dad;
                dad = ka != 0 && is_dad; mom = ka != 0 && !is_dad;
            }
            n_dad += __popcll(__ballot(dad)); n_mom += __popcll(__ballot(mom));
        }
        int o_dad = 0, o_mom = 0;
        for (int64_t b = c0; b < c1; b += 64) {
            const int64_t i = b + lane;
            bool dad = false, mom = false;
            int32_t p = 0;
            if (i < c1) {
// ... 351 lines not shown
    UZ_HIP(hipGetLastError());
}

__device__ __forceinline__ uint32_t gt_pack4(uint32_t k, uint32_t d, uint32_t m, uint32_t s) {
    return (k & 0x03030303u) | ((d & 0x03030303u) << 2) | ((m & 0x03030303u) << 4) | ((s & 0x01010101u * UZ_SF_COMPLEX) << 6);
}
__global__ __launch_bounds__(256) void k_family_gt_pack(int64_t n, const uint8_t *__restrict__ gt, size_t stride, const int32_t *__restrict__ trio,
                                                        const uint8_t *__restrict__ sflags, uint8_t *__restrict__ out, size_t out_stride) {
    const size_t t = blockIdx.y;
    const uint8_t *__restrict__ gk = gt + (size_t)trio[3 * t] * stride;
    const uint8_t *__restrict__ gd = gt + (size_t)trio[3 * t + 1] * stride;
    const uint8_t *__restrict__ gm = gt + (size_t)trio[3 * t + 2] * stride;
    uint8_t *__restrict__ o = out + t * out_stride;
    const int64_t n_chunks = (n + 256 * 16 - 1) / (256 * 16);
    for (int64_t chunk = blockIdx.x; chunk < n_chunks; chunk += gridDim.x) {
        const int64_t base = (chunk * 256 + threadIdx.x) * 16;
        if (base >= n) continue;
        if (base + 16 <= n) {
            const uint4 k = *reinterpret_cast<const uint4 *>(gk + base), d = *reinterpret_cast<const uint4 *>(gd + base);
            const uint4 m = *reinterpret_cast<const uint4 *>(gm + base), s = *reinterpret_cast<const uint4 *>(sflags + base);
            *reinterpret_cast<uint4 *>(o + base) = make_uint4(gt_pack4(k.x, d.x, m.x, s.x), gt_pack4(k.y, d.y, m.y, s.y), gt_pack4(k.z, d.z, m.z, s.z),
                                                              gt_pack4(k.w, d.w, m.w, s.w));
        } else {
            for (int64_t i = base; i < n; i++) o[i] = (uint8_t)gt_pack4(gk[i], gd[i], gm[i], sflags[i]);
        }
    }
}
__global__ __launch_bounds__(256) void k_family_wide_gather(int64_t n_wide, const int32_t *__restrict__ wrd, const int32_t *__restrict__ wad,
                                                            const int32_t *__restrict__ trio, int32_t *__restrict__ out) {
    const size_t t = blockIdx.y;
    const int64_t k = (int64_t)blockIdx.x * 256 + threadIdx.x;
    if (k >= n_wide) return;
    int32_t *__restrict__ o = out + t * 6 * (size_t)n_wide;
#pragma unroll
    for (int m = 0; m < 3; m++) {
        const size_t row = (size_t)trio[3 * t + m] * (size_t)n_wide;
        o[(size_t)m * n_wide + k] = wrd[row + k];
        o[(size_t)(3 + m) * n_wide + k] = wad[row + k];
    }
}
void uz_launch_family_pack(uz_ctx *c, const SamplesDev &sm, const SitesDev &s, int32_t n, const int32_t *trio, uint8_t *gt_out, size_t gt_stride, int32_t *wide_out) {
    if (n <= 0) return;
    UZ_REQUIRE((uintptr_t)s.sflags % 16 == 0, UZ_E_ARG, "the site flags of an adopted sites table must be 16-byte aligned for uz_families_from_samples");
    ProfScope ps(c, UZ_K_FAMILY_PACK);
    const int32_t y_max = 65535;
    for (int32_t t0 = 0; t0 < n; t0 += y_max) {
        const int32_t ny = std::min<int32_t>(y_max, n - t0);
        if (s.n > 0) {
            const int64_t n_chunks = (s.n + 256 * 16 - 1) / (256 * 16);
            const int64_t nb = std::max<int64_t>(1, std::min<int64_t>(n_chunks, std::max<int64_t>(4096 / ny, 16)));
            hipLaunchKernelGGL(k_family_gt_pack, dim3((unsigned)nb, (unsigned)ny), dim3(256), 0, c->stream, s.n, (const uint8_t *)sm.gt, sm.stride, trio + 3 * (size_t)t0,
                               (const uint8_t *)s.sflags, gt_out + (size_t)t0 * gt_stride, gt_stride);
            UZ_HIP(hipGetLastError());
        }
        if (sm.n_wide > 0) {
            hipLaunchKernelGGL(k_family_wide_gather, dim3((unsigned)((sm.n_wide + 255) / 256), (unsigned)ny), dim3(256), 0, c->stream, sm.n_wide, (const int32_t *)sm.wide_rd,
                               (const int32_t *)sm.wide_ad, trio + 3 * (size_t)t0, wide_out + (size_t)t0 * 6 * (size_t)sm.n_wide);
            UZ_HIP(hipGetLastError());
        }
    }
}

bool uz_site_scan_fresh(const uz_ctx *c, const FamilyDev &f, bool need_cnv) {
    return f.cls_valid && (f.cls_has_cnv || !need_cnv) && site_params_equal(f.cls_params, c->P);
}

#ifndef UZ_SITE_SPT
#define UZ_SITE_SPT 8
#endif

namespace {

void ensure_ab_lut(uz_ctx *c, const SiteParams &sp) {
    if (c->ab_lut_valid && site_params_equal(c->ab_lut_params, c->P)) return;
    c->ab_lut.ensure((size_t)4 * UZ_AB_LUT_N * 2 + 4 + 4 * UZ_AB_LDS_T);
    int *flag = c->ab_lut.p + (size_t)4 * UZ_AB_LUT_N * 2;
    UZ_HIP(hipMemsetAsync(flag, 0, sizeof(int), c->stream));
    hipLaunchKernelGGL(k_build_ab_lut, dim3((4 * UZ_AB_LUT_N + 255) / 256), dim3(256), 0, c->stream, sp, (int2 *)c->ab_lut.p,
                       (uint32_t *)(flag + 4), flag);
    UZ_HIP(hipGetLastError());
    int special = 0;
    UZ_HIP(hipMemcpyAsync(&special, flag, sizeof(int), hipMemcpyDeviceToHost, c->stream));
    UZ_HIP(hipStreamSynchronize(c->stream));
    c->ab_lut_t0_special = special != 0;
    c->ab_lut_valid = true;
    c->ab_lut_params = c->P;
}

FamPtrs fam_ptrs(const FamilyDev &f) {
    FamPtrs fp;
    fp.gt = f.gt;
    for (int m = 0; m < 3; m++) { fp.rd[m] = f.rd[m]; fp.ad[m] = f.ad[m]; fp.gq[m] = f.gq[m]; }
    return fp;
}

void launch_site_scan(uz_ctx *c, const FamPtrs &fp, uint8_t *cls, int64_t n, bool with_cnv, const FamBatchItem *batch, int n_fam) {
    const SiteParams sp = make_site_params(c->P);
    ensure_ab_lut(c, sp);
    static const int spt = [] { const char *e = getenv("UZ_SITE_SPT"); return e ? atoi(e) : UZ_SITE_SPT; }();
    ProfScope ps(c, UZ_K_SITE_SCAN);
    auto launch = [&](auto kern, int SPT) {
        const int64_t n_chunks = (n + 256 * SPT - 1) / (256 * SPT);
        static const int wgs = [] { const char *e = getenv("UZ_SITE_WGS"); return e ? atoi(e) : 4096; }();
        int64_t nb = n_chunks < wgs ? n_chunks : wgs;
        if (batch && n_fam > 1) {
            const int64_t per = (wgs + n_fam - 1) / n_fam;
            nb = std::max<int64_t>(1, std::min<int64_t>(n_chunks, std::max<int64_t>(per, 16)));
        }
        hipLaunchKernelGGL(kern, dim3((unsigned)nb, (unsigned)(batch ? n_fam : 1)), dim3(256), 0, c->stream, fp, cls, n, sp,
                           (const int2 *)c->ab_lut.p, (const uint32_t *)(c->ab_lut.p + (size_t)4 * UZ_AB_LUT_N * 2 + 4), batch);
    };
    const bool t0 = c->ab_lut_t0_special;
#define UZ_K1_PICK(SPTV, BATCHV)                                                                                              \
    do {                                                                                                                        \
        if (with_cnv) { if (t0) launch(k_site_scan<SPTV, true, true, BATCHV>, SPTV); else launch(k_site_scan<SPTV, true, false, BATCHV>, SPTV); } \
        else { if (t0) launch(k_site_scan<SPTV, false, true, BATCHV>, SPTV); else launch(k_site_scan<SPTV, false, false, BATCHV>, SPTV); }        \
    } while (0)
    if (batch) { if (spt == 16) UZ_K1_PICK(16, true); else UZ_K1_PICK(8, true); }
    else { if (spt == 16) UZ_K1_PICK(16, false); else UZ_K1_PICK(8, false); }
#undef UZ_K1_PICK
    UZ_HIP(hipGetLastError());
}

}

static void launch_site_scan_wide(uz_ctx *c, FamilyDev &f, bool with_cnv) {
    if (f.n_wide <= 0) return;
    const SiteParams P = make_site_params(c->P);
    const unsigned nb = (unsigned)((f.n_wide + 255) / 256);
    if (with_cnv) hipLaunchKernelGGL(k_site_scan_wide<true>, dim3(nb), dim3(256), 0, c->stream, fam_ptrs(f), f.cls, f.n_wide, f.wide_site, f.wide_depth, P);
    else hipLaunchKernelGGL(k_site_scan_wide<false>, dim3(nb), dim3(256), 0, c->stream, fam_ptrs(f), f.cls, f.n_wide, f.wide_site, f.wide_depth, P);
    UZ_HIP(hipGetLastError());
}

static void check_gq_clamp(const uz_ctx *c, const FamilyDev &f) {
    UZ_REQUIRE(!f.gq_clamped || c->P.min_gt_qual <= 254, UZ_E_STATE,
               "this family was staged with eight-bit genotype qualities (clamped at 254): --min-gt-qual above 254 needs the 16-bit columns");
}
static void check_het_only(const FamilyDev &f, bool with_cnv) {
    UZ_REQUIRE(!(with_cnv && f.het_only), UZ_E_STATE,
               "this family was staged in the het form (genotype columns of the kid-het sites only): the DEL / DUP classes need every site's columns");
}
void uz_launch_site_scan(uz_ctx *c, FamilyDev &f, const SitesDev &s, bool with_cnv) {
    check_gq_clamp(c, f);
    check_het_only(f, with_cnv);
    if (s.n > 0) { launch_site_scan(c, fam_ptrs(f), f.cls, s.n, with_cnv, nullptr, 1); launch_site_scan_wide(c, f, with_cnv); }
    f.cls_has_cnv = with_cnv;
    f.cls_valid = true;
    f.cls_params = c->P;
}

void uz_launch_site_scan_many(uz_ctx *c, FamilyDev *const *fams, int n_fam, const SitesDev &s, bool with_cnv) {
    if (n_fam <= 0) return;
    for (int k = 0; k < n_fam; k++) { check_gq_clamp(c, *fams[k]); check_het_only(*fams[k], with_cnv); }
    if (s.n > 0) {
        std::vector<FamBatchItem> items((size_t)n_fam);
        for (int k = 0; k < n_fam; k++) { items[(size_t)k].f = fam_ptrs(*fams[k]); items[(size_t)k].cls = fams[k]->cls; }
        c->fam_batch.ensure((size_t)n_fam * sizeof(FamBatchItem));
        UZ_HIP(hipMemcpyAsync(c->fam_batch.p, items.data(), items.size() * sizeof(FamBatchItem), hipMemcpyHostToDevice, c->stream));
        UZ_HIP(hipStreamSynchronize(c->stream));
        launch_site_scan(c, items[0].f, items[0].cls, s.n, with_cnv, (const FamBatchItem *)c->fam_batch.p, n_fam);
        for (int k = 0; k < n_fam; k++) launch_site_scan_wide(c, *fams[k], with_cnv);
    }
    for (int k = 0; k < n_fam; k++) {
        fams[k]->cls_has_cnv = with_cnv;
        fams[k]->cls_valid = true;
        fams[k]->cls_params = c->P;
    }
}

void uz_launch_find(uz_ctx *c, FamilyDev &f, const SitesDev &s, int mode, bool host_offsets) {
    const int32_t n = c->dn.n;
    c->cnt_c.ensure((size_t)n + 1);
    c->cnt_h.ensure((size_t)n + 1);
    c->cand_off.ensure((size_t)n + 1);
    c->het_off.ensure((size_t)n + 1);
    if (host_offsets || n <= 0) { c->cand_off_h.assign((size_t)n + 1, 0); c->het_off_h.assign((size_t)n + 1, 0); }
    else { c->cand_off_h.resize((size_t)n + 1); c->het_off_h.resize((size_t)n + 1); }
    c->n_cand = c->n_het = 0;
    if (n > 0) {
        WinArgs a;
        a.n = n;
        a.contig = c->dn.contig.p; a.start = c->dn.start.p; a.end = c->dn.end.p;
        a.vartype = c->dn.vartype.p; a.mult = c->dn.mult.p;
        a.contig_off = s.contig_off; a.n_contigs = s.n_contigs;
        a.pos = s.pos; a.cls = f.cls;
        a.cls_of = c->cohort_on ? (const uint8_t *const *)c->fam_cls.p : nullptr;
        a.fam_idx = c->cohort_on ? c->dn_fam.p : nullptr;
        a.sd = c->P.search_dist;
        a.mode = mode;
        c->win_range.ensure((size_t)4 * n + 4);
        a.range = c->win_range.p;
        const unsigned nbw = (unsigned)(((int64_t)n * 64 + 255) / 256);
        {
            ProfScope ps(c, UZ_K_WINDOW_COUNT);
            if (mode & UZ_FIND_WHOLE_REGION)
                hipLaunchKernelGGL(k_window_region<false>, dim3(nbw), dim3(256), 0, c->stream, a, c->cnt_c.p, c->cnt_h.p,
                                   (const int64_t *)nullptr, (const int64_t *)nullptr, (int32_t *)nullptr, (uint8_t *)nullptr,
                                   (int32_t *)nullptr);
            else
                hipLaunchKernelGGL(k_window_wave<false>, dim3(nbw), dim3(256), 0, c->stream, a, c->cnt_c.p, c->cnt_h.p,
                                   (const int64_t *)nullptr, (const int64_t *)nullptr, (int32_t *)nullptr,
                                   (uint8_t *)nullptr, (int32_t *)nullptr);
            UZ_HIP(hipGetLastError());
            const unsigned tiles = (unsigned)(((int64_t)n + 4095) / 4096);
            c->scan_part.ensure((size_t)2 * tiles);
            hipLaunchKernelGGL(k_scan2_sums, dim3(tiles), dim3(1024), 0, c->stream, n, c->cnt_c.p, c->cnt_h.p, c->scan_part.p);
            UZ_HIP(hipGetLastError());
            hipLaunchKernelGGL(k_scan2, dim3(tiles), dim3(1024), 0, c->stream, n, c->cnt_c.p, c->cnt_h.p, (const int64_t *)c->scan_part.p, c->cand_off.p,
                               c->het_off.p);
            UZ_HIP(hipGetLastError());
        }
        auto fill = [&](int64_t cap_c, int64_t cap_h) {
            a.cap_c = cap_c; a.cap_h = cap_h;
            ProfScope ps(c, UZ_K_WINDOW_FILL);
            if (mode & UZ_FIND_WHOLE_REGION)
                hipLaunchKernelGGL(k_window_region<true>, dim3(nbw), dim3(256), 0, c->stream, a, (int32_t *)nullptr, (int32_t *)nullptr,
                                   (const int64_t *)c->cand_off.p, (const int64_t *)c->het_off.p, c->cand_idx.p, c->cand_flags.p,
                                   c->het_idx.p);
            else
                hipLaunchKernelGGL(k_window_wave<true>, dim3(nbw), dim3(256), 0, c->stream, a, (int32_t *)nullptr,
                                   (int32_t *)nullptr, (const int64_t *)c->cand_off.p, (const int64_t *)c->het_off.p,
                                   c->cand_idx.p, c->cand_flags.p, c->het_idx.p);
            UZ_HIP(hipGetLastError());
        };
        int64_t room_c = (int64_t)std::min(c->cand_idx.cap, c->cand_flags.cap) - 1, room_h = (int64_t)c->het_idx.cap - 1;
        if (const char *e = getenv("UZ_TEST_FIND_CAP")) { room_c = std::min<int64_t>(room_c, atoll(e)); room_h = std::min<int64_t>(room_h, atoll(e)); }
        const bool tried = room_c > 0 && room_h > 0;
        if (tried) fill(room_c, room_h);
        if (host_offsets) {
            const size_t ob = ((size_t)n + 1) * sizeof(int64_t), obr = (ob + 255) & ~(size_t)255;
            c->find_pin.room(2 * obr);
            uz_kcopy(c, c->find_pin.p, c->cand_off.p, ob);
            uz_kcopy(c, c->find_pin.p + obr, c->het_off.p, ob);
            UZ_HIP(hipStreamSynchronize(c->stream));
            memcpy(c->cand_off_h.data(), c->find_pin.p, ob);
            memcpy(c->het_off_h.data(), c->find_pin.p + obr, ob);
        } else {
            int64_t *box = reinterpret_cast<int64_t *>(c->hflags + 4);
            uz_kcopy(c, box, c->cand_off.p + n, sizeof(int64_t));
            uz_kcopy(c, box + 1, c->het_off.p + n, sizeof(int64_t));
            UZ_HIP(hipStreamSynchronize(c->stream));
            c->cand_off_h[n] = box[0];
            c->het_off_h[n] = box[1];
        }
        c->n_cand = c->cand_off_h[n];
        c->n_het = c->het_off_h[n];
        if (!tried || c->n_cand > room_c || c->n_het > room_h) {
            c->cand_idx.ensure((size_t)c->n_cand + 1);
            c->cand_flags.ensure((size_t)c->n_cand + 1);
            c->het_idx.ensure((size_t)c->n_het + 1);
            fill(INT64_MAX, INT64_MAX);
        }
    }
    c->find_valid = true;
    c->find_mode = mode;
}

void uz_launch_cnv(uz_ctx *c, const SitesDev &s, const int32_t *rb_counts_dev, int32_t *cnv_counts, int32_t *cnv_pos, int32_t *origin,
                   int32_t *evidence, int32_t *etype) {
    const int32_t n = c->dn.n;
    if (n <= 0) return;
    ProfScope ps(c, UZ_K_CNV);
    hipLaunchKernelGGL(k_cnv_count, dim3((unsigned)(((int64_t)n * 64 + 255) / 256)), dim3(256), 0, c->stream, n, (const int64_t *)c->cand_off.p,
                       (const int32_t *)c->cand_idx.p, (const uint8_t *)c->cand_flags.p, (const int32_t *)s.pos, (const uint8_t *)c->dn.vartype.p,
                       rb_counts_dev, (int)c->P.evidence_min_ratio, cnv_counts, cnv_pos, origin, evidence, etype);
    UZ_HIP(hipGetLastError());
}

void uz_launch_cnv_dense(uz_ctx *c, const int32_t *cnv_counts, const int32_t *cnv_pos, int64_t *cnv_off, int32_t *dense) {
    const int32_t n = c->dn.n;
    if (n <= 0) return;
    UZ_REQUIRE(n < (1 << 30), UZ_E_RANGE, "too many DNMs for one allele-balance batch");
    const int32_t m = 2 * n;
    const unsigned tiles = (unsigned)(((int64_t)m + 4095) / 4096);
    c->scan_part.ensure((size_t)2 * tiles);
    ProfScope ps(c, UZ_K_CNV_DENSE);
    hipLaunchKernelGGL(k_scan1_sums, dim3(tiles), dim3(1024), 0, c->stream, m, cnv_counts, c->scan_part.p);
    UZ_HIP(hipGetLastError());
    hipLaunchKernelGGL(k_scan1, dim3(tiles), dim3(1024), 0, c->stream, m, cnv_counts, (const int64_t *)c->scan_part.p, cnv_off);
    UZ_HIP(hipGetLastError());
    hipLaunchKernelGGL(k_cnv_dense, dim3((unsigned)(((int64_t)n * 64 + 255) / 256)), dim3(256), 0, c->stream, n, (const int64_t *)c->cand_off.p,
                       (const int64_t *)cnv_off, cnv_pos, dense);
    UZ_HIP(hipGetLastError());
}
```

unfazed_amd/csrc/uz_ctx.hpp:

```cpp
#pragma once
#include <hip/hip_runtime.h>

#include <cstdint>
#include <cstring>
#include <functional>
#include <mutex>
#include <string>
#include <memory>
#include <vector>

#include "unfazed_hip.h"
#include "uz_bamwalk.h"
#include "bgzf_batch.hpp"
#include "walk_book.hpp"

struct UzError {
    int code;
    std::string msg;
};

#define UZ_HIP(call)                                                                                   \
    do {                                                                                               \
        hipError_t e__ = (call);                                                                       \
        if (e__ != hipSuccess)                                                                         \
// ... 216 lines not shown
    uint8_t *nlow = nullptr;
    int64_t n_qlow_pos = 0;
    int64_t n_plane_units = 0;
    const uint32_t *cigar = nullptr;
    const uint8_t *seq4 = nullptr;
    uint8_t *qlow = nullptr;
    int32_t qlow_thr = 0;
    bool qlow_valid = false;
    uint8_t *qual8 = nullptr;
    uint32_t *qual_off16 = nullptr;
    uint16_t *qs = nullptr;
    int32_t *coarse = nullptr;
    int32_t *mid = nullptr;
    int32_t *mid8 = nullptr;
    hipEvent_t ready = nullptr;
    bool pending = false;
    hipEvent_t built = nullptr;
    RecColumns cols;
    void *build_scratch = nullptr;
    int64_t n_cigar_staged = 0;
    const uint8_t *seq2_staged = nullptr;
    const uint32_t *exc_rec = nullptr;
    const uint16_t *exc_pos = nullptr;
    const uint8_t *exc_code = nullptr;
    int64_t n_exc = 0;
    int64_t n_bl = 0, n_bl_units = 0;
    const uz_kept_rec *kept_list = nullptr;
    const uint32_t *name_rec = nullptr;
    const uint8_t *names = nullptr;
    int64_t names_bytes = 0;
};

template <typename T>
struct DevPtr { T *p = nullptr; };
struct DnmsDev {
    int32_t n = 0;
    DevBuf<uint8_t> block;
    DevPtr<int32_t> contig, rcontig, start, end;
    DevPtr<uint8_t> vartype, dflags, mult;
    DevPtr<uint32_t> allele_off;
    DevPtr<uint8_t> alleles;
    double cutoff = 0;
};

struct ProfSlot {
    double total_ms = 0;
    int64_t launches = 0;
    int64_t last_units = 0;
};
struct ProfPending {
    int kernel;
    hipEvent_t a, b;
};

struct uz_ctx {
    int device = 0;
    hipStream_t stream = nullptr;
    hipStream_t copy_stream = nullptr;
    hipStream_t build_stream = nullptr;
    int32_t *hflags = nullptr;
    std::vector<DevBlock> block_pool;
    uz_params P;
    std::string err;
    std::mutex err_mu;
    std::vector<SitesDev> sites;
    std::vector<FamilyDev> fams;
    std::vector<ReadsDev> reads;
    std::vector<SamplesDev> samples;
    DevBuf<int32_t> trio_idx;
    uint8_t *vcf_pin[2] = {nullptr, nullptr};
    size_t vcf_pin_cap[2] = {0, 0};

    DevBuf<int32_t> ab_lut;
    DevBuf<uint8_t> fam_batch;
    bool ab_lut_valid = false;
    bool ab_lut_t0_special = false;
    uz_params ab_lut_params;

    bool find_valid = false;
    int find_fam = -1, find_mode = 0;
    DnmsDev dn;
    uint8_t *dn_stage = nullptr;
    PinBuf find_pin;
    size_t dn_stage_cap = 0;
    hipEvent_t dn_stage_done = nullptr;
    DevBuf<int64_t> scan_part;
    DevBuf<int32_t> cnt_c, cnt_h;
    DevBuf<int64_t> win_range;
    DevBuf<int64_t> cand_off, het_off;
    DevBuf<int32_t> cand_idx, het_idx;
    DevBuf<uint8_t> cand_flags;
    int64_t n_cand = 0, n_het = 0;
    std::vector<int64_t> cand_off_h, het_off_h;
    FindKey find_key;
    unsigned long long find_stamp = 0, find_counter = 0;
    FindSlot find_alt[UZ_FIND_ALTS];

    bool cohort_on = false;
    DevBuf<int32_t> dn_fam;
    DevBuf<double> dn_cutoff;
    DevBuf<uint8_t *> fam_cls;
    std::vector<uint32_t> phase_qbase;
    int cohort_reads = -1;
    std::vector<int> cohort_ids;

    bool cnv_valid = false;
    int32_t cnv_n = 0;
    DevBuf<int32_t> cnv_counts, cnv_pos, cnv_origin, cnv_evidence, cnv_etype, cnv_rb;
    DevBuf<int64_t> cnv_off;
    DevBuf<int32_t> cnv_dense;
    std::vector<int32_t> cnv_counts_h;
    std::vector<int64_t> cnv_off_h;

    DevBuf<uint8_t> inf_comp, inf_out;
    DevBuf<int64_t> inf_in, inf_off;
    DevBuf<int32_t> inf_flags;
    hipStream_t inf_stream = nullptr, inf_stream2 = nullptr;
    hipEvent_t inf_ready = nullptr;

    struct WalkSlot {
#define UZ_X(T, name) DevBuf<T> name;
        UZ_WALK_BUFS(UZ_X)
        int64_t n_blocks = 0, out_bytes = 0, n_desc = 0, n_desc_all = 0, n_reach = 0;
        int32_t n_tasks = 0, max_host = -1;
        hipStream_t s0 = nullptr, s1 = nullptr;
        hipEvent_t ev = nullptr;
        struct Join {
            int64_t n_dev = 0, n_all = 0, aux_bytes = 0;
            int32_t n_host = 0, n_look = 0, n_ref = 0, round = 0, trips = 0;
            int64_t n_need = 0;
            bool filled = false, started = false, done = false, all_bases = false;
            UZ_JOIN_BUFS(UZ_X)
#undef UZ_X
            int64_t tot_h[16] = {0, 0, 0, 0, 0, 0, 0, 0, 0, 0, 0, 0, 0, 0, 0, 0};
            std::vector<int64_t> contig_off_h;
            std::vector<int32_t> max_span_h;
        } join;
    };
    static constexpr int WALK_SLOTS = WalkBook::SLOTS;
    WalkSlot walk[WALK_SLOTS];
    WalkBook book;

    struct HeadDev {
        bool live = false;
        int32_t n_files = 0;
        std::vector<int64_t> want, have, first;
        DevBuf<int32_t> tlen;
        DevBuf<int64_t> first_d;
    };
    std::vector<HeadDev> heads;
    DevBuf<uint8_t> hd_comp, hd_out;
    DevBuf<int64_t> hd_i64;
    DevBuf<int32_t> hd_i32;
    DevBuf<uint32_t> hd_u32;

    DevBuf<uint32_t> nm_ids, nm_len, nm_off;
    DevBuf<int64_t> rf_first;
    DevBuf<uint32_t> rf_mm;
    DevBuf<uint8_t> nm_out;
    PinBuf nm_pin;

    DevBuf<uint8_t> bed_in, bed_hook, bed_out;
    DevBuf<uint32_t> bed_len;
    DevBuf<int64_t> bed_off;
    PinBuf bed_pin;
    OutBufs vo, bo, df;
    DevBuf<uint8_t> df_slots;

    bool phase_valid = false;
    bool phase_open = false;
    int32_t phase_n = 0;
    void *phase_state = nullptr;

    uint32_t prof_mask = 0;
    ProfSlot prof[UZ_K_COUNT];
    std::vector<ProfPending> prof_pending;
    std::vector<hipEvent_t> event_pool;
};

template <typename T>
inline void uz_walk_grow(uz_ctx *c, DevBuf<T> &b, WalkKind kind, size_t n, size_t used = 0, hipStream_t st = nullptr) {
    const size_t hi = c->book.note(kind, n);
    std::pair<void *, size_t> old;
    if (b.ensure_parked(n, hi, &old, used, st)) c->book.grew(old.first, old.second);
}
#define UZ_WGROW(w, name, ...) uz_walk_grow(c, (w).name, WK_##name, __VA_ARGS__)
#define UZ_JGROW(J, name, ...) uz_walk_grow(c, (J).name, JK_##name, __VA_ARGS__)

template <typename V>
int new_slot(std::vector<V> &v) {
    for (size_t i = 0; i < v.size(); i++)
        if (!v[i].live) return (int)i;
    v.emplace_back();
    return (int)v.size() - 1;
}

void uz_prof_begin(uz_ctx *c, int kernel, hipEvent_t *a, hipEvent_t *b);
void uz_prof_end(uz_ctx *c, int kernel, hipEvent_t a, hipEvent_t b);
void uz_prof_drain(uz_ctx *c);

struct ProfScope {
    uz_ctx *c;
    int k;
    hipEvent_t a = nullptr, b = nullptr;
    ProfScope(uz_ctx *c_, int k_) : c(c_), k(k_) { uz_prof_begin(c, k, &a, &b); }
    ~ProfScope() { uz_prof_end(c, k, a, b); }
};

DevBlock uz_block_get(uz_ctx *c, size_t bytes);
void uz_block_put(uz_ctx *c, DevBlock b);

void uz_kcopy(uz_ctx *c, void *dst, const void *src, size_t bytes);
void uz_len_scan(uz_ctx *c, hipStream_t st, int64_t n, const uint32_t *len, uint32_t add, int64_t *off);
void uz_reads_make_ready(uz_ctx *c, ReadsDev &r);
void uz_reads_ready_for_threshold(uz_ctx *c, ReadsDev &r, const char *what);
void uz_check_upload_flag(uz_ctx *c);
size_t uz_rec_scratch_bytes(int64_t n);
void uz_build_records(uz_ctx *c, hipStream_t st, ReadsDev &r, const RecColumns &col, void *off_scratch);
void uz_pack_ascii_rows(uz_ctx *c, hipStream_t st, ReadsDev &r, const uint32_t *cigar_in, const uint32_t *cigar_off_in,
                        const uint8_t *seq_in, const uint32_t *sq_off16_in, uint32_t *cigar_out, uint8_t *seq4_out);
void uz_build_qlow(uz_ctx *c, hipStream_t st, ReadsDev &r, int min_base_qual);
void uz_concat_table(uz_ctx *c, hipStream_t st, ReadsDev &dst, const ReadsDev &src, int64_t rec_base, int64_t cigar_base, int64_t unit_base,
                     int64_t seq_base, uint32_t qname_base);
void uz_finish_table(uz_ctx *c, hipStream_t st, ReadsDev &r);
void uz_family_widen(uz_ctx *c, FamilyDev &f, int64_t n_sites);
void uz_sites_expand(uz_ctx *c, SitesDev &s, FamilyDev *f);
void uz_launch_family_pack(uz_ctx *c, const SamplesDev &sm, const SitesDev &s, int32_t n, const int32_t *trio, uint8_t *gt_out, size_t gt_stride, int32_t *wide_out);
void uz_vcf_parse_text(uz_ctx *c, const uz_vcf_text_view *t, int32_t n_pick, const int32_t *pick, SamplesDev &m, size_t chunk_bytes, std::vector<int64_t> &unsettled);
void uz_vcf_parse_bcf(uz_ctx *c, const uz_vcf_bcf_view *t, int32_t n_pick, const int32_t *pick, SamplesDev &m, size_t chunk_bytes, std::vector<int64_t> &unsettled);
void uz_launch_vcf_settle(uz_ctx *c, int64_t n, int32_t n_rows, const int64_t *site, const uint8_t *gt_in, const uint16_t *rd_in, const uint16_t *ad_in,
                          const uint16_t *gq_in, SamplesDev &m);
void uz_launch_site_scan(uz_ctx *c, FamilyDev &f, const SitesDev &s, bool with_cnv);
void uz_launch_site_scan_many(uz_ctx *c, FamilyDev *const *fams, int n_fam, const SitesDev &s, bool with_cnv);
void uz_launch_find(uz_ctx *c, FamilyDev &f, const SitesDev &s, int mode, bool host_offsets = true);
void uz_stage_dnms(uz_ctx *c, const uz_dnms_view *d);
void uz_launch_cnv(uz_ctx *c, const SitesDev &s, const int32_t *rb_counts_dev, int32_t *cnv_counts, int32_t *cnv_pos, int32_t *origin,
                   int32_t *evidence, int32_t *etype);
void uz_launch_cnv_dense(uz_ctx *c, const int32_t *cnv_counts, const int32_t *cnv_pos, int64_t *cnv_off, int32_t *dense);
void uz_launch_phase(uz_ctx *c, FamilyDev &f, const SitesDev &s, ReadsDev &r, int32_t *status, int32_t *counts,
                     int32_t *origin, int32_t *evidence, bool defer = false);
bool uz_finish_phase(uz_ctx *c, int32_t *status, int32_t *counts, int32_t *origin, int32_t *evidence);
void uz_launch_inflate(uz_ctx *c, hipStream_t st, int64_t n_blocks, const uint8_t *comp, int64_t comp_bytes_padded, const int64_t *in_off,
                       const int64_t *out_off, uint8_t *out, int32_t *cursor_and_err);
struct InflateBatch {
    const uint8_t *comp; int64_t comp_bytes, n_blocks; const int64_t *in_off, *out_off;
    uint8_t *d_comp; int64_t *d_in, *d_off; uint8_t *d_out; int32_t *d_flags;
    hipStream_t st[2]; hipEvent_t ev;
    bool tables_there = false;
    std::function<void(size_t, hipStream_t)> before, after;
};
void uz_queue_inflate(uz_ctx *c, const InflateBatch &b, const std::vector<int64_t> &cut);
void uz_launch_bam_walk(uz_ctx *c, hipStream_t st, int n_tasks, const uint8_t *buf, const int64_t *blk_at, const int64_t *blk_coff, const int32_t *task,
                        const int64_t *span, const int32_t *reach, const int32_t *fetch, int64_t *count, const int64_t *first, int64_t *walked, int32_t *flags,
                        uz_walk_desc *out, int64_t *n_direct, int64_t *tab_first, const uz_walk_file *tfile = nullptr);
void uz_launch_desc_filter(uz_ctx *c, hipStream_t st, bool fill, int n_tasks, const uz_walk_desc *in, const int64_t *first, const int64_t *count,
                           const int32_t *task, const int64_t *tab_first, unsigned long long *tab, int64_t *kcount, int64_t *kfirst, uz_walk_desc *out);
size_t uz_bam_walk_pad();
enum { JT_N = 0, JT_QNAMES = 1, JT_CIGAR = 2, JT_UNITS = 3, JT_SEQ_UNITS = 4, JT_NAME_BYTES = 5, JT_ERR = 6, JT_COUNT = 8 };
struct JoinPlanHost {
    int32_t n_host = 0, n_ref = 0;
    const int32_t *h_flags = nullptr;
    bool all_bases = false;
};
void uz_join_run(uz_ctx *c, uz_ctx::WalkSlot &w, const JoinPlanHost &P, const uz_walk_desc *x, int64_t n_x, const uint8_t *xaux, int64_t xaux_bytes,
                 const int32_t *look_tid, int64_t n_look, const int32_t *need_jtask);
void uz_join_needs(uz_ctx *c, uz_ctx::WalkSlot &w, uz_need_rec *out);
void uz_join_fetch(uz_ctx *c, uz_ctx::WalkSlot &w, uint64_t *voff, uint32_t *qname, int32_t *mate, uint8_t *bases, uz_kept_rec *kept);
void uz_launch_reads_files(uz_ctx *c, hipStream_t st, int32_t n_files, const void *rec_b, const int64_t *rec_first, uint32_t *mn, uint32_t *mx);
void uz_launch_name_lens(uz_ctx *c, hipStream_t st, int64_t n_ids, const uint32_t *ids, const uint32_t *name_rec, const uz_kept_rec *kept, int64_t n_recs, int64_t names_bytes,
                         uint32_t *len);
void uz_launch_name_gather(uz_ctx *c, hipStream_t st, int64_t n_ids, const uint32_t *ids, const uint32_t *name_rec, const uz_kept_rec *kept, const uint8_t *names,
                           const uint32_t *len, const uint32_t *off, uint8_t *out);
void uz_scan_u32(uz_ctx *c, hipStream_t st, const uint32_t *in, uint32_t *out, int64_t n, uz_ctx::WalkSlot::Join &J);
void uz_launch_bam_extract(uz_ctx *c, hipStream_t st, int64_t n, const uint8_t *buf, int64_t buf_bytes, const uint8_t *aux, int64_t aux_bytes, const uz_kept_rec *kept,
                           int thr, int32_t *start, int32_t *tlen, int32_t *mate, uint32_t *qname, uint16_t *flag, uint16_t *l_seq, uint16_t *n_cigar, uint8_t *mapq,
                           uint8_t *aux_col, uint32_t *cigar, uint8_t *seq4, uint32_t *plane, int32_t *err, uint8_t *names, int64_t n_cigar_total, int64_t n_row_units,
                           int64_t n_seq_units, int64_t names_bytes);
void uz_launch_crc32(uz_ctx *c, hipStream_t st, int64_t n_blocks, const uint8_t *out, const int64_t *out_off, const uint32_t *want, int32_t *err);
int uz_phase_votes_impl(uz_ctx *c, int64_t *vote_off, int32_t *vote_val);
int uz_phase_groups_impl(uz_ctx *c, int64_t *grp_off, int32_t *grp_q);
int uz_phase_sizing_fetch_impl(uz_ctx *c, int32_t *bounds, int32_t *pre_win, int32_t *pre_ha, int32_t *pre_hl, int64_t *reduced);
void uz_phase_state_free(uz_ctx *c);
void uz_phase_lists_dev(uz_ctx *c, int32_t *n, const int32_t **status, const int32_t **counts, const int32_t **pool, const long long **list_start,
                        const int32_t **list_len);
int uz_bed_rows_impl(uz_ctx *c, const uz_bed_view *rows, int verbose, int include_ambiguous, int64_t *off, const uint8_t **bytes);
int uz_bed_rows_lists_impl(uz_ctx *c, const uz_bed_view *rows, int verbose, int include_ambiguous, int32_t n_dnms, const int32_t *status, const int64_t *list_off,
                           const int32_t *list_val, uint32_t n_qnames, const uint32_t *name_off, const uint8_t *name_bytes, int32_t ratio, int64_t *off,
                           const uint8_t **bytes);
int uz_vcf_rows_impl(uz_ctx *c, const uz_vcf_text_view *text, const int64_t *line_at, const int64_t *ann_off, const int32_t *ann_col, const uint8_t *ann_gt,
                     const int32_t *ann_uops, const int8_t *ann_uet, int64_t *off, const uint8_t **bytes, uint8_t *handed_back);
void uz_bgzf_inflate_impl(uz_ctx *c, const uint8_t *comp, int64_t comp_bytes, int64_t n_blocks, const int64_t *in_off, const int64_t *out_off, uint8_t *out,
                         int repeat, double *kernel_ms);
void uz_bgzf_inflate_to_host_impl(uz_ctx *c, const uint8_t *comp, int64_t comp_bytes, int64_t n_blocks, const int64_t *in_off, const int64_t *out_off,
                                 uint8_t *out);
void uz_crc32_blocks_impl(uz_ctx *c, const uint8_t *data, int64_t n_blocks, const int64_t *off, const uint32_t *want, int64_t *first_bad);
void uz_head_walk_impl(uz_ctx *c, int *head_id, int32_t n_files, const uint8_t *comp, int64_t comp_bytes, int64_t n_blocks, const int64_t *in_off,
                      const int32_t *isize, const uint32_t *crc, const int64_t *blk_first, const int64_t *start, const int64_t *want, const int64_t *have,
                      int64_t *taken, int64_t *cursor, int32_t *state);
void uz_head_rank_impl(uz_ctx *c, int head_id, int32_t readlen, const int64_t *k, uint32_t *a, uint32_t *b);
void uz_head_fetch_impl(uz_ctx *c, int head_id, int32_t file, int32_t *out, int64_t cap, int64_t *n);
void uz_head_free_impl(uz_ctx *c, int head_id);
int uz_bgzf_deflate_impl(uz_ctx *c, const uint8_t *data, int64_t n_bytes, int64_t *n_blocks, const uint8_t **bgzf, int64_t *bgzf_bytes, int repeat, double *kernel_ms);
int uz_bcf_rows_impl(uz_ctx *c, const uz_bcf_lines_view *records, int64_t *off, uint64_t *samp_at, const uint8_t **bytes, uint8_t *handed_back);
```

unfazed_amd/engine.py:

```python
from __future__ import annotations

import ctypes as C
import os
from typing import List, Optional

import numpy as np

from . import abi

_HERE = os.path.dirname(os.path.abspath(__file__))
LIB_PATH = os.environ.get("UZ_HIP_LIB", os.path.join(_HERE, "libunfazed_hip.so"))

SIZING_REDUCED_WORDS = 263
K_SITE_SCAN, K_WINDOW_COUNT, K_WINDOW_FILL, K_PHASE, K_SIZING, K_CNV, K_FAMILY_PACK, K_CNV_DENSE = 0, 1, 2, 3, 4, 5, 6, 7
K_VCF_TABS, K_VCF_CELLS, K_VCF_COPY = 8, 9, 10
K_BCF_CELLS, K_BCF_COPY = 11, 12
K_HEAD_INFLATE, K_HEAD_WALK, K_HEAD_RANK = 13, 14, 15
K_BED_SIZE, K_BED_FILL = 16, 17
K_VCFOUT_SIZE, K_VCFOUT_FILL = 18, 19
K_BCFOUT_SIZE, K_BCFOUT_FILL = 20, 21
K_DEFLATE, K_DEFLATE_FRAME = 22, 23
HEAD_NONE, HEAD_DONE, HEAD_END, HEAD_BAD = 0, 1, 2, 3
HEAD_MAX_BYTES = 8 << 30
HEAD_MAX_ROUNDS = 8

EXPORTS = [
    "uz_create", "uz_destroy", "uz_last_error", "uz_sync", "uz_set_params",
    "uz_sites_upload", "uz_family_upload", "uz_sites_family_upload_async", "uz_samples_upload", "uz_samples_from_text", "uz_samples_from_bcf", "uz_samples_unsettled", "uz_samples_settle", "uz_families_from_samples", "uz_family_fetch", "uz_samples_free", "uz_reads_upload", "uz_reads_upload_packed", "uz_reads_wait", "uz_reads_headers", "uz_reads_columns", "uz_reads_marks", "uz_bgzf_inflate", "uz_bgzf_inflate_to_host", "uz_bam_walk", "uz_bam_walk_many", "uz_reads_files", "uz_crc32_blocks", "uz_bam_walk_fetch", "uz_bam_walk_release", "uz_reads_from_bam",
    "uz_bam_walk_flags", "uz_bam_join", "uz_bam_join_needs", "uz_bam_join_fetch", "uz_reads_from_walk", "uz_reads_names", "uz_walk_slot_stats", "uz_walk_reserve",
    "uz_pinned_alloc", "uz_pinned_free",
    "uz_sites_adopt_device", "uz_family_adopt_device", "uz_reads_adopt_device",
    "uz_sites_free", "uz_reads_free", "uz_drop_derived",
    "uz_site_scan", "uz_site_scan_many", "uz_site_classes", "uz_find", "uz_find_fetch", "uz_find_cohort",
    "uz_phase", "uz_phase_begin", "uz_phase_end", "uz_phase_cohort", "uz_phase_cohort_joined", "uz_phase_votes", "uz_phase_groups", "uz_phase_sizing_fetch", "uz_phase_cnv", "uz_phase_cnv_cohort", "uz_phase_cnv_sites",
    "uz_bed_rows", "uz_bed_rows_lists", "uz_vcf_rows", "uz_bcf_rows", "uz_bgzf_deflate",
    "uz_prof_enable", "uz_prof_reset", "uz_prof_get", "uz_prof_units",
    "uz_head_walk", "uz_head_rank", "uz_head_fetch", "uz_head_free",
]

_lib = None


class UnfazedHipError(RuntimeError):
    pass


def load_library(path: Optional[str] = None):
    global _lib
    if _lib is not None and path is None:
        return _lib
    p = path or LIB_PATH
    if not os.path.exists(p):
        raise UnfazedHipError(
            "%s not found: build it with `python -m unfazed_amd.build` (hipcc, gfx950). "
            "There is no CPU fallback for the phasing path." % p
        )
    L = C.CDLL(p)
    vp, i32, i64p = C.c_void_p, C.c_int, C.c_void_p
    L.uz_create.argtypes = [C.c_int, C.POINTER(vp)]
    L.uz_destroy.argtypes = [vp]
    L.uz_destroy.restype = None
    L.uz_last_error.argtypes = [vp]
    L.uz_last_error.restype = C.c_char_p
    L.uz_sync.argtypes = [vp]
    L.uz_set_params.argtypes = [vp, vp]
    L.uz_reads_wait.argtypes = [vp, C.c_int]
    L.uz_reads_headers.argtypes = [vp, C.c_int, vp, vp, vp, vp, vp]
    L.uz_reads_columns.argtypes = [vp, C.c_int] + [vp] * 10
    L.uz_reads_marks.argtypes = [vp, C.c_int, vp, vp]
    L.uz_bgzf_inflate.argtypes = [vp, vp, C.c_int64, C.c_int64, vp, vp, vp, C.c_int, C.POINTER(C.c_double)]
    L.uz_bgzf_inflate_to_host.argtypes = [vp, vp, C.c_int64, C.c_int64, vp, vp, vp]
    L.uz_crc32_blocks.argtypes = [vp, vp, C.c_int64, vp, vp, vp]
    L.uz_bam_walk.argtypes = [vp, vp, C.c_int64, C.c_int64, vp, vp, vp, vp, C.c_int32, vp, C.c_int64, vp, C.c_int64, vp, C.c_int64, vp, vp, vp]
    L.uz_bam_walk_many.argtypes = L.uz_bam_walk.argtypes[:-2] + [C.c_int32, vp, vp, vp, vp, vp, vp]
    L.uz_reads_files.argtypes = [vp, C.c_int, C.c_int32, vp, vp, vp]
    L.uz_bam_walk_fetch.argtypes = [vp, C.c_int, vp, vp, vp, vp]
    L.uz_bam_walk_release.argtypes = [vp, C.c_int]
    L.uz_reads_from_bam.argtypes = [vp, C.c_int, vp, C.c_int64, vp, C.c_int64, vp, vp, C.c_int32, C.c_int64, C.c_int64, C.c_int64, C.c_uint32, C.c_int32, vp, C.c_int64, vp]
    L.uz_bam_walk_flags.argtypes = [vp, C.c_int, vp, vp]
    L.uz_bam_join.argtypes = [vp, C.c_int, C.c_int32, vp, C.c_int32, C.c_int, vp, C.c_int64, vp, C.c_int64, vp, C.c_int64, vp, vp, vp]
    L.uz_bam_join_needs.argtypes = [vp, C.c_int, vp]
    L.uz_bam_join_fetch.argtypes = [vp, C.c_int, vp, vp, vp, vp, vp, vp, vp]
    L.uz_reads_from_walk.argtypes = [vp, C.c_int, C.c_int32, C.c_int, vp, vp]
    L.uz_reads_names.argtypes = [vp, C.c_int, vp, C.c_int64, vp, vp]
    L.uz_walk_slot_stats.argtypes = [vp, vp]
    L.uz_walk_reserve.argtypes = [vp, C.c_int]
    L.uz_pinned_alloc.argtypes = [C.c_size_t, C.POINTER(vp)]
    L.uz_pinned_free.argtypes = [vp]
    L.uz_pinned_free.restype = None
    for f in ("uz_sites_upload", "uz_reads_upload", "uz_reads_upload_packed", "uz_sites_adopt_device", "uz_reads_adopt_device"):
        getattr(L, f).argtypes = [vp, vp, C.POINTER(C.c_int)]
    for f in ("uz_family_upload", "uz_family_adopt_device"):
        getattr(L, f).argtypes = [vp, C.c_int, vp, C.POINTER(C.c_int)]
    L.uz_sites_family_upload_async.argtypes = [vp, vp, vp, C.POINTER(C.c_int), C.POINTER(C.c_int)]
    L.uz_samples_upload.argtypes = [vp, C.c_int, vp, C.POINTER(C.c_int)]
    L.uz_families_from_samples.argtypes = [vp, C.c_int, C.c_int32, vp, vp, vp, vp]
    L.uz_samples_from_text.argtypes = [vp, C.c_int, vp, C.c_int32, vp, C.POINTER(C.c_int), C.POINTER(C.c_int64)]
    L.uz_samples_from_bcf.argtypes = L.uz_samples_from_text.argtypes
    L.uz_samples_unsettled.argtypes = [vp, C.c_int, vp]
    L.uz_samples_settle.argtypes = [vp, C.c_int, C.c_int64, vp, vp]
    L.uz_family_fetch.argtypes = [vp, C.c_int, vp, vp]
    L.uz_samples_free.argtypes = [vp, C.c_int]
    L.uz_drop_derived.argtypes = [vp]
    L.uz_sites_free.argtypes = [vp, C.c_int]
    L.uz_reads_free.argtypes = [vp, C.c_int]
    L.uz_site_scan.argtypes = [vp, C.c_int]
    L.uz_site_scan_many.argtypes = [vp, vp, C.c_int32]
    L.uz_site_classes.argtypes = [vp, C.c_int, vp]
    L.uz_find.argtypes = [vp, C.c_int, vp, C.c_int, vp, vp]
    L.uz_find_fetch.argtypes = [vp, vp, vp, vp]
    L.uz_find_cohort.argtypes = [vp, vp, C.c_int32, vp, C.c_int, vp, vp]
    L.uz_phase.argtypes = [vp, C.c_int, C.c_int, vp, C.c_int, vp, vp, vp, vp]
    L.uz_phase_begin.argtypes = [vp, C.c_int, C.c_int, vp, C.c_int]
    L.uz_phase_end.argtypes = [vp, C.c_int, C.c_int, vp, C.c_int, vp, vp, vp, vp]
    L.uz_phase_cohort.argtypes = [vp, vp, C.c_int32, vp, C.c_int, vp, vp, vp, vp]
    L.uz_phase_cohort_joined.argtypes = [vp, C.c_int, vp, C.c_int32, vp, vp, C.c_int, vp, vp, vp, vp]
    L.uz_phase_cnv.argtypes = [vp, C.c_int, vp, vp, vp, vp, vp, vp]
    L.uz_phase_cnv_cohort.argtypes = [vp, vp, C.c_int32, vp, vp, vp, vp, vp, vp]
    L.uz_phase_cnv_sites.argtypes = [vp, vp, vp]
    L.uz_phase_votes.argtypes = [vp, vp, vp]
    L.uz_phase_groups.argtypes = [vp, vp, vp]
    L.uz_phase_sizing_fetch.argtypes = [vp, vp, vp, vp, vp, vp]
    L.uz_bed_rows.argtypes = [vp, vp, C.c_int, C.c_int, vp, vp]
    L.uz_bed_rows_lists.argtypes = [vp, vp, C.c_int, C.c_int, C.c_int32, vp, vp, vp, C.c_uint32, vp, vp, C.c_int32, vp, vp]
    L.uz_vcf_rows.argtypes = [vp, vp, vp, vp, vp, vp, vp, vp, vp, vp, vp]
    L.uz_bgzf_deflate.argtypes = [vp, vp, C.c_int64, vp, vp, vp, C.c_int, C.POINTER(C.c_double)]
    L.uz_bcf_rows.argtypes = [vp, vp, vp, vp, vp, vp]
    L.uz_head_walk.argtypes = [vp, C.POINTER(C.c_int), C.c_int32, vp, C.c_int64, C.c_int64, vp, vp, vp, vp, vp, vp, vp, vp, vp, vp]
    L.uz_head_rank.argtypes = [vp, C.c_int, C.c_int32, vp, vp, vp]
    L.uz_head_fetch.argtypes = [vp, C.c_int, C.c_int32, vp, C.c_int64, C.POINTER(C.c_int64)]
    L.uz_head_free.argtypes = [vp, C.c_int]
    L.uz_prof_enable.argtypes = [vp, C.c_int]
    L.uz_prof_reset.argtypes = [vp]
    L.uz_prof_get.argtypes = [vp, C.c_int, C.POINTER(C.c_double), C.POINTER(C.c_int64)]
    L.uz_prof_units.argtypes = [vp, C.c_int, C.POINTER(C.c_int64)]
    for name in EXPORTS:
        fn = getattr(L, name)
        if name not in ("uz_destroy", "uz_last_error", "uz_pinned_free"):
            fn.restype = C.c_int
    if path is None:
        _lib = L
    return L


class HipEngine:

    def __init__(self, device: int = 0):
        self.L = load_library()
        h = C.c_void_p()
        rc = self.L.uz_create(int(device), C.byref(h))
        if rc != 0:
            raise UnfazedHipError(
                "uz_create(device=%d) failed with %d: a gfx950 (MI355X) device is required; "
                "there is no CPU fallback" % (device, rc)
            )
        self.h = h
        self.device = device
        self._keep: List[object] = []
        self._staged = {}
        self._staged_sites = {}
        self._params = None
        import threading
        self._inflate_lock = threading.Lock()
        self._walked = 0
        self._walked_lock = threading.Lock()
        self._walk_sem = threading.BoundedSemaphore(int(os.environ.get("UZ_WALKS_AT_ONCE", "2")))
        self._slots = {}

    def close(self):
        for pool, pair in getattr(self, "_slots", {}).values():
            pool.free_all()
            pair.free_all()
        self._slots = {}
        if getattr(self, "_head_pin", None) is not None:
            self._head_pin[0].free_all()
            self._head_pin = None
        if getattr(self, "h", None):
            self.L.uz_destroy(self.h)
            self.h = None

    def __del__(self):
        try:
            self.close()
        except Exception:
            pass

    def _ck(self, rc, what):
        if rc != 0:
            msg = self.L.uz_last_error(self.h)
            raise UnfazedHipError("%s failed (%d): %s" % (what, rc, msg.decode() if msg else ""))

    def set_params(self, params: abi.Params):
        self._ck(self.L.uz_set_params(self.h, C.byref(params)), "uz_set_params")
# ... 341 lines not shown

    def crc32_blocks(self, data: np.ndarray, off: np.ndarray, want: np.ndarray) -> int:
        data = np.ascontiguousarray(data, np.uint8)
        off = np.ascontiguousarray(off, np.int64)
        want = np.ascontiguousarray(want, np.uint32)
        bad = C.c_int64(-1)
        self._ck(self.L.uz_crc32_blocks(self.h, data.ctypes.data, int(off.size) - 1, off.ctypes.data, want.ctypes.data, C.byref(bad)), "uz_crc32_blocks")
        return int(bad.value)

    def bam_walk_release(self, walk_id: int):
        self._ck(self.L.uz_bam_walk_release(self.h, int(walk_id)), "uz_bam_walk_release")

    def reads_from_bam(self, kb, names: bool = False) -> int:
        rid = C.c_int(-1)
        if getattr(kb, "joined", False):
            from . import io_native
            tot = np.zeros(8, np.int64)
            self._ck(self.L.uz_reads_from_walk(self.h, int(kb.token), int(kb.min_base_qual), 1 if names else 0, C.byref(rid), tot.ctypes.data), "uz_reads_from_walk")
            kb.token = None
            with self._walked_lock:
                self._walked += 1
                walked = self._walked
            if walked in (1, 2, 4):
                self._ck(self.L.uz_walk_reserve(self.h, 4), "uz_walk_reserve")
            if names:
                kb.qnames = io_native.DeviceNames(self, rid.value, int(kb.n_qnames))
            return rid.value
        nb = int(kb.n_name_bytes) if names else 0
        alloc = getattr(kb, "_alloc", None)
        buf = (alloc(max(1, nb)) if alloc is not None else np.empty(max(1, nb), np.uint8)) if names else None
        self._ck(self.L.uz_reads_from_bam(self.h, int(kb.token), kb.kept.ctypes.data, int(kb.n), kb.aux.ctypes.data, int(kb.n_aux), kb.contig_off.ctypes.data,
                                          kb.max_span.ctypes.data, int(kb.n_contigs), int(kb.n_cigar_total), int(kb.n_row_units), int(kb.n_seq_units),
                                          int(kb.n_qnames), int(kb.min_base_qual), buf.ctypes.data if names else None, nb, C.byref(rid)), "uz_reads_from_bam")
        kb.token = None
        if names:
            kb.set_names(buf[:nb])
        return rid.value

    def adopt_sites(self, view: abi.SitesView) -> int:
        sid = C.c_int(-1)
        self._ck(self.L.uz_sites_adopt_device(self.h, C.byref(view), C.byref(sid)), "uz_sites_adopt_device")
        return sid.value

    def adopt_family(self, sites_h: int, view: abi.FamilyView) -> int:
        fid = C.c_int(-1)
        self._ck(self.L.uz_family_adopt_device(self.h, int(sites_h), C.byref(view), C.byref(fid)), "uz_family_adopt_device")
        return fid.value

    def adopt_reads(self, view: abi.ReadsPackedView) -> int:
        rid = C.c_int(-1)
        self._ck(self.L.uz_reads_adopt_device(self.h, C.byref(view), C.byref(rid)), "uz_reads_adopt_device")
        return rid.value

    def free_sites(self, sid: int):
        self._ck(self.L.uz_sites_free(self.h, int(sid)), "uz_sites_free")
        self._samples = {k: x for k, x in getattr(self, "_samples", {}).items() if x[0] != int(sid)}
        self._staged_sites.pop(int(sid), None)

    def free_reads(self, rid: int):
        self._ck(self.L.uz_reads_free(self.h, int(rid)), "uz_reads_free")
        self._staged.pop(int(rid), None)

    def drop_derived(self):
        self._ck(self.L.uz_drop_derived(self.h), "uz_drop_derived")

    def sync(self):
        self._ck(self.L.uz_sync(self.h), "uz_sync")

    def site_scan(self, fam: int):
        self._ck(self.L.uz_site_scan(self.h, int(fam)), "uz_site_scan")

    def site_scan_many(self, fams):
        ids = np.ascontiguousarray(np.asarray(list(fams), dtype=np.int32))
        self._ck(self.L.uz_site_scan_many(self.h, ids.ctypes.data, int(ids.size)), "uz_site_scan_many")

    def classify(self, fam: int, params: abi.Params, n_sites: int) -> np.ndarray:
        self.set_params(params)
        out = np.zeros(max(1, n_sites), dtype=np.uint8)
        self._ck(self.L.uz_site_classes(self.h, int(fam), out.ctypes.data), "uz_site_classes")
        return out[:n_sites]

    def find(self, fam: int, dv: abi.Held, params: abi.Params, mode: int, fetch: bool = True, transient: bool = False):
        self.set_params(params)
        return self._find_out(dv.view.n, fetch, transient,
                              lambda co, ho: self._ck(self.L.uz_find(self.h, int(fam), dv.ref(), int(mode), co, ho), "uz_find"))

    def _find_out(self, n, fetch, transient, run):
        co = np.zeros(n + 1, dtype=np.int64)
        ho = np.zeros(n + 1, dtype=np.int64)
        run(co.ctypes.data, ho.ctypes.data)
        if not fetch:
            return co, None, None, ho, None
        ci, cf, hi = self._fetch(int(co[n]), int(ho[n]), transient=transient)
        return co, ci, cf, ho, hi

    @staticmethod
    def _groups(groups):
        arr = (abi.CohortGroup * max(1, len(groups)))()
        for k, g in enumerate(groups):
            fam, rh, first, count, cutoff = g if len(g) == 5 else (g[0], -1, g[1], g[2], 0.0)
            arr[k].fam_id, arr[k].reads_id, arr[k].dnm_first, arr[k].dnm_count, arr[k].cutoff = int(fam), int(rh), int(first), int(count), float(cutoff)
        return arr

    def find_cohort(self, groups, dv: abi.Held, params: abi.Params, mode: int, fetch: bool = True):
        self.set_params(params)
        arr = self._groups(groups)
        return self._find_out(dv.view.n, fetch, False,
                              lambda co, ho: self._ck(self.L.uz_find_cohort(self.h, arr, len(groups), dv.ref(), int(mode), co, ho), "uz_find_cohort"))

    def _fetch(self, nc: int, nh: int, transient: bool = False):
        if transient:
            if not hasattr(self, "_find_pins"):
                self._find_pins, self._find_turn = [None, None, None], 0
            self._find_turn = (self._find_turn + 1) % 3
            need = 4 * max(1, nc) + 256 + max(1, nc) + 256 + 4 * max(1, nh) + 256
            pin = self._find_pins[self._find_turn]
            if pin is None or pin[1].size < need:
                if pin is not None:
                    pin[0].free_all()
                pool = PinnedPool()
                pin = self._find_pins[self._find_turn] = (pool, pool.alloc(need + need // 4 + (1 << 16)))
            buf = pin[1]
            a = (4 * max(1, nc) + 255) & ~255
            b = a + ((max(1, nc) + 255) & ~255)
            ci, cf, hi = buf[: 4 * max(1, nc)].view(np.int32), buf[a: a + max(1, nc)], buf[b: b + 4 * max(1, nh)].view(np.int32)
        else:
            ci = np.zeros(max(1, nc), dtype=np.int32)
            cf = np.zeros(max(1, nc), dtype=np.uint8)
            hi = np.zeros(max(1, nh), dtype=np.int32)
        self._ck(self.L.uz_find_fetch(self.h, ci.ctypes.data, cf.ctypes.data, hi.ctypes.data), "uz_find_fetch")
        return ci[:nc], cf[:nc], hi[:nh]

    def _phase_out(self, n, run):
        status = np.empty(max(1, n), dtype=np.int32)
        counts = np.empty(max(1, 4 * n), dtype=np.int32)
        origin = np.empty(max(1, n), dtype=np.int32)
        evidence = np.empty(max(1, n), dtype=np.int32)
        run(status.ctypes.data, counts.ctypes.data, origin.ctypes.data, evidence.ctypes.data)
        return dict(status=status[:n], counts=counts[: 4 * n].reshape(n, 4), origin=origin[:n], evidence=evidence[:n])

    def _with_lists(self, r, n, want_lists):
        r["lists"] = None
        if want_lists:
            vo, vv = self.votes(n)
            r["lists"] = [tuple(vv[vo[4 * k + j]: vo[4 * k + j + 1]] for j in range(4)) for k in range(n)]
        return r

    def phase_raw(self, fam: int, reads_h: int, dv: abi.Held, params: abi.Params, find_mode: int):
        self.set_params(params)
        return self._phase_out(dv.view.n, lambda *out: self._ck(self.L.uz_phase(self.h, int(fam), int(reads_h), dv.ref(), int(find_mode), *out), "uz_phase"))

    def phase_begin(self, fam: int, reads_h: int, dv: abi.Held, params: abi.Params, find_mode: int):
        self.set_params(params)
        self._ck(self.L.uz_phase_begin(self.h, int(fam), int(reads_h), dv.ref(), int(find_mode)), "uz_phase_begin")

    def phase_end(self, fam: int, reads_h: int, dv: abi.Held, params: abi.Params, find_mode: int):
        return self._phase_out(dv.view.n, lambda *out: self._ck(self.L.uz_phase_end(self.h, int(fam), int(reads_h), dv.ref(), int(find_mode), *out), "uz_phase_end"))

    def phase_cohort(self, groups, dv: abi.Held, params: abi.Params, found_list=None, want_lists: bool = True,
                     find_mode: int = abi.FIND_SECOND_WINDOW, joined=None):
        self.set_params(params)
        n = dv.view.n
        arr = self._groups(groups)
        if joined is None:
            r = self._phase_out(n, lambda *out: self._ck(self.L.uz_phase_cohort(self.h, arr, len(groups), dv.ref(), int(find_mode), *out), "uz_phase_cohort"))
        else:
            rid, base = joined
            base = np.ascontiguousarray(base, np.int32)
            assert base.size == len(groups)
            r = self._phase_out(n, lambda *out: self._ck(self.L.uz_phase_cohort_joined(self.h, int(rid), arr, len(groups), base.ctypes.data, dv.ref(),
                                                                                       int(find_mode), *out), "uz_phase_cohort_joined"))
        return self._with_lists(r, n, want_lists)

    def phase_cohort_joined(self, rid: int, groups, group_ref_base, dv: abi.Held, params: abi.Params, found_list=None, want_lists: bool = True,
                            find_mode: int = abi.FIND_SECOND_WINDOW):
        return self.phase_cohort(groups, dv, params, found_list, want_lists, find_mode, joined=(rid, group_ref_base))

    def votes(self, n: int):
        vo = np.zeros(4 * n + 1, dtype=np.int64)
        self._ck(self.L.uz_phase_votes(self.h, vo.ctypes.data, None), "uz_phase_votes")
        vv = np.zeros(max(1, int(vo[-1])), dtype=np.int32)
        self._ck(self.L.uz_phase_votes(self.h, vo.ctypes.data, vv.ctypes.data), "uz_phase_votes")
        return vo, vv[: int(vo[-1])]

    def groups(self, n: int):
        go = np.zeros(2 * n + 1, dtype=np.int64)
        self._ck(self.L.uz_phase_groups(self.h, go.ctypes.data, None), "uz_phase_groups")
        gq = np.zeros(max(1, int(go[-1])), dtype=np.int32)
        self._ck(self.L.uz_phase_groups(self.h, go.ctypes.data, gq.ctypes.data), "uz_phase_groups")
        return go, gq[: int(go[-1])]

    def _bed_text(self, n: int, off, ptr):
        total = int(off[n])
        return (C.string_at(ptr.value, total) if total else b""), off

    def bed_rows(self, rows, str_off, str_bytes, verbose: bool, include_ambiguous: bool):
        v = abi.bed_view(rows, str_off, str_bytes)
        n = int(v.view.n_rows)
        off, ptr = np.zeros(n + 1, np.int64), C.c_void_p()
        self._ck(self.L.uz_bed_rows(self.h, v.ref(), int(bool(verbose)), int(bool(include_ambiguous)), off.ctypes.data, C.byref(ptr)), "uz_bed_rows")
        return self._bed_text(n, off, ptr)

    def bed_rows_lists(self, rows, str_off, str_bytes, verbose: bool, include_ambiguous: bool, status, list_off, list_val, name_off, name_bytes, ratio: int):
        v = abi.bed_view(rows, str_off, str_bytes)
        n = int(v.view.n_rows)
        status = np.ascontiguousarray(status, np.int32)
        list_off = np.ascontiguousarray(list_off, np.int64)
        list_val = np.ascontiguousarray(list_val, np.int32)
        off, ptr = np.zeros(n + 1, np.int64), C.c_void_p()
        if name_off is not None:
            name_off, name_bytes = np.ascontiguousarray(name_off, np.uint32), np.ascontiguousarray(name_bytes, np.uint8)
            nq, p_no, p_nb = int(name_off.size) - 1, name_off.ctypes.data, name_bytes.ctypes.data if name_bytes.size else None
# ... 336 lines not shown
```

Before: 12.40 million DNMs/s.

## Return find results in one pinned block and fold memsets into phase kernels

Adds a uz_find_answer entry point that writes offsets and candidate and het lists into a single caller-provided pinned block, so the host needs one sync instead of a find followed by a separate fetch round trip. It also batches several small device-to-pinned copies into one multi-segment copy kernel. In the phase sizing path, the buffer clears that used to be separate memsets now run inside k_phase_bounds, and the bounds readback is skipped when speculative sizing is in use. The cost is more complex control flow, plus a retry path when the answer block is too small.

```diff
diff --git a/include/unfazed_hip.h b/include/unfazed_hip.h
--- a/include/unfazed_hip.h
+++ b/include/unfazed_hip.h
@@ -128,6 +128,10 @@
 int uz_find(uz_ctx *ctx, int fam_id, const uz_dnms_view *dnms, int mode,
             int64_t *cand_off , int64_t *het_off );
 int uz_find_fetch(uz_ctx *ctx, int32_t *cand_idx, uint8_t *cand_flags, int32_t *het_idx);
+#define UZ_FA_GREW_LISTS 1
+#define UZ_FA_BLOCK_SMALL 2
+int uz_find_answer(uz_ctx *ctx, int fam_id, const uz_dnms_view *dnms, int mode, void *block, size_t block_bytes, int64_t out[4]);
+int uz_find_stats(uz_ctx *ctx, int64_t out[4]);
 int uz_find_cohort(uz_ctx *ctx, const uz_cohort_group *groups, int32_t n_groups, const uz_dnms_view *dnms, int mode,
                    int64_t *cand_off , int64_t *het_off );
 
diff --git a/unfazed_amd/csrc/abi.hip b/unfazed_amd/csrc/abi.hip
--- a/unfazed_amd/csrc/abi.hip
+++ b/unfazed_amd/csrc/abi.hip
@@ -1,4 +1,5 @@
 #include "uz_ctx.hpp"
+#include "find_answer.hpp"
 
 #include <chrono>
 #include <algorithm>
@@ -208,11 +209,43 @@
 }
 void uz_kcopy(uz_ctx *c, void *dst, const void *src, size_t bytes) {
     if (!bytes) return;
+    uz_find_launched(c, 1);
     const uintptr_t a = (uintptr_t)dst | (uintptr_t)src | (uintptr_t)bytes;
     auto grid = [](size_t n) { return dim3((unsigned)std::min<size_t>((n + 255) / 256, 1024)); };
     if (a % 16 == 0) hipLaunchKernelGGL(k_copy<uint4>, grid(bytes / 16), dim3(256), 0, c->stream, (uint4 *)dst, (const uint4 *)src, bytes / 16);
     else if (a % 4 == 0) hipLaunchKernelGGL(k_copy<uint32_t>, grid(bytes / 4), dim3(256), 0, c->stream, (uint32_t *)dst, (const uint32_t *)src, bytes / 4);
     else hipLaunchKernelGGL(k_copy<uint8_t>, grid(bytes), dim3(256), 0, c->stream, (uint8_t *)dst, (const uint8_t *)src, bytes);
+    UZ_HIP(hipGetLastError());
+}
+struct KCopySegs { KCopySeg s[UZ_KCOPY_SEGS]; };
+template <typename W>
+__device__ __forceinline__ void copy_seg(void *dst, const void *src, size_t n) {
+    W *__restrict__ d = (W *)dst;
+    const W *__restrict__ s = (const W *)src;
+    for (size_t i = (size_t)blockIdx.x * 256 + threadIdx.x; i < n; i += (size_t)gridDim.x * 256) d[i] = s[i];
+}
+__global__ __launch_bounds__(256) void k_copy_many(KCopySegs g) {
+    const KCopySeg sg = g.s[blockIdx.y];
+    const uintptr_t a = (uintptr_t)sg.dst | (uintptr_t)sg.src | (uintptr_t)sg.bytes;
+    if (a % 16 == 0) copy_seg<uint4>(sg.dst, sg.src, sg.bytes / 16);
+    else if (a % 4 == 0) copy_seg<uint32_t>(sg.dst, sg.src, sg.bytes / 4);
+    else copy_seg<uint8_t>(sg.dst, sg.src, sg.bytes);
+}
+void uz_kcopy_many(uz_ctx *c, const KCopySeg *segs, int n_segs) {
+    KCopySegs g;
+    int m = 0;
+    size_t units = 0;
+    for (int k = 0; k < n_segs; k++) {
+        if (!segs[k].bytes) continue;
+        UZ_REQUIRE(m < UZ_KCOPY_SEGS, UZ_E_ARG, "uz_kcopy_many: too many segments");
+        g.s[m++] = segs[k];
+        const uintptr_t a = (uintptr_t)segs[k].dst | (uintptr_t)segs[k].src | (uintptr_t)segs[k].bytes;
+        units = std::max(units, segs[k].bytes / (a % 16 == 0 ? 16 : a % 4 == 0 ? 4 : 1));
+    }
+    if (!m) return;
+    uz_find_launched(c, 1);
+    for (int k = m; k < UZ_KCOPY_SEGS; k++) g.s[k] = KCopySeg{nullptr, nullptr, 0};
+    hipLaunchKernelGGL(k_copy_many, dim3((unsigned)std::min<size_t>((units + 255) / 256, 1024), (unsigned)m), dim3(256), 0, c->stream, g);
     UZ_HIP(hipGetLastError());
 }
 
@@ -1832,6 +1865,9 @@
         SitesDev &s = sites_of(c, f.sites_id);
         UZ_REQUIRE(d != nullptr && d->n >= 0, UZ_E_ARG, "bad DNM view");
         c->phase_valid = false;
+        FindCount counting(c);
+        c->find_stat[0] = c->find_stat[1] = c->find_stat[2] = c->find_stat[3] = 0;
+        c->find_answer_again = false;
         const bool cnv = (mode & UZ_FIND_WHOLE_REGION) != 0;
         if (cnv) refuse_het_only(f, "a whole-region find");
         if (!uz_site_scan_fresh(c, f, cnv)) uz_launch_site_scan(c, f, s, cnv);
@@ -1847,17 +1883,70 @@
     });
 }
 
+int uz_find_answer(uz_ctx *c, int fam_id, const uz_dnms_view *d, int mode, void *block, size_t block_bytes, int64_t out[4]) {
+    return guarded(c, [&] {
+        FamilyDev &f = fam_of(c, fam_id);
+        SitesDev &s = sites_of(c, f.sites_id);
+        UZ_REQUIRE(d != nullptr && d->n >= 0, UZ_E_ARG, "bad DNM view");
+        FindCount counting(c);
+        UZ_REQUIRE(block != nullptr && (uintptr_t)block % UZ_FA_ALIGN == 0 && inside_one_pinned_block((const uint8_t *)block, (const uint8_t *)block + block_bytes),
+                   UZ_E_ARG, "uz_find_answer: the block must be page-locked memory of this library (uz_pinned_alloc), 256-byte aligned");
+        c->phase_valid = false;
+        const bool cnv = (mode & UZ_FIND_WHOLE_REGION) != 0;
+        if (cnv) refuse_het_only(f, "a whole-region find");
+        FindAnswer ans{(uint8_t *)block, block_bytes, 0, 0};
+        const size_t n = (size_t)d->n;
+        if (c->find_answer_again && n > 0 && find_recall(c, find_key_of(c, fam_id, mode, d)) &&
+            uz_find_answer_fits(uz_find_answer_layout(d->n, c->n_cand, c->n_het), block_bytes)) {
+            c->dn_n_of_find = d->n;
+            UZ_REQUIRE(uz_launch_find_answer(c, &ans, INT64_MAX, INT64_MAX), UZ_E_STATE, "uz_find_answer: the block reported as sufficient is not");
+        } else {
+            c->find_stat[0] = c->find_stat[1] = c->find_stat[2] = c->find_stat[3] = 0;
+            if (!uz_site_scan_fresh(c, f, cnv)) uz_launch_site_scan(c, f, s, cnv);
+            uz_stage_dnms(c, d);
+            const FindKey key = find_key_of(c, fam_id, mode, d);
+            find_target(c);
+            uz_launch_find(c, f, s, mode, true, &ans);
+            if (f.het_only) uz_check_upload_flag(c);
+            find_done(c, key);
+            c->find_fam = fam_id;
+            if (n == 0) {
+                const FindAnswerLayout L = uz_find_answer_layout(0, 0, 0);
+                ans.need = L.total;
+                if (!uz_find_answer_fits(L, block_bytes)) ans.code |= UZ_FA_BLOCK_SMALL;
+                else {
+                    memset(block, 0, (size_t)L.total);
+                    int64_t *head = (int64_t *)block;
+                    head[2] = 1; head[3] = (int64_t)L.total;
+                }
+            }
+        }
+        c->find_answer_again = ans.code != 0;
+        c->find_stat[2] |= ans.code;
+        c->find_stat[3] = (int64_t)ans.need;
+        if (out) { out[0] = ans.code; out[1] = (int64_t)ans.need; out[2] = c->n_cand; out[3] = c->n_het; }
+    });
+}
+int uz_find_stats(uz_ctx *c, int64_t out[4]) {
+    if (!c || !out) return UZ_E_ARG;
+    for (int k = 0; k < 4; k++) out[k] = c->find_stat[k];
+    return 0;
+}
+
 int uz_find_fetch(uz_ctx *c, int32_t *cand_idx, uint8_t *cand_flags, int32_t *het_idx) {
     return guarded(c, [&] {
         UZ_REQUIRE(c->find_valid, UZ_E_STATE, "uz_find_fetch before uz_find");
+        FindCount counting(c);
         const bool pinned = (!cand_idx || !c->n_cand || inside_one_pinned_block((const uint8_t *)cand_idx, (const uint8_t *)(cand_idx + c->n_cand))) &&
                             (!cand_flags || !c->n_cand || inside_one_pinned_block(cand_flags, cand_flags + c->n_cand)) &&
                             (!het_idx || !c->n_het || inside_one_pinned_block((const uint8_t *)het_idx, (const uint8_t *)(het_idx + c->n_het)));
         if (pinned) {
-            if (cand_idx && c->n_cand) uz_kcopy(c, cand_idx, c->cand_idx.p, (size_t)c->n_cand * sizeof(int32_t));
-            if (cand_flags && c->n_cand) uz_kcopy(c, cand_flags, c->cand_flags.p, (size_t)c->n_cand);
-            if (het_idx && c->n_het) uz_kcopy(c, het_idx, c->het_idx.p, (size_t)c->n_het * sizeof(int32_t));
+            const KCopySeg lists[3] = {{cand_idx, c->cand_idx.p, cand_idx ? (size_t)c->n_cand * sizeof(int32_t) : 0},
+                                       {cand_flags, c->cand_flags.p, cand_flags ? (size_t)c->n_cand : 0},
+                                       {het_idx, c->het_idx.p, het_idx ? (size_t)c->n_het * sizeof(int32_t) : 0}};
+            uz_kcopy_many(c, lists, 3);
             UZ_HIP(hipStreamSynchronize(c->stream));
+            uz_find_waited(c);
             return;
         }
         if (cand_idx && c->n_cand)
@@ -1867,6 +1956,7 @@
         if (het_idx && c->n_het)
             UZ_HIP(hipMemcpyAsync(het_idx, c->het_idx.p, (size_t)c->n_het * sizeof(int32_t), hipMemcpyDeviceToHost, c->stream));
         UZ_HIP(hipStreamSynchronize(c->stream));
+        uz_find_waited(c);
     });
 }
 
diff --git a/unfazed_amd/csrc/find_answer.hpp b/unfazed_amd/csrc/find_answer.hpp
--- /dev/null
+++ b/unfazed_amd/csrc/find_answer.hpp
@@ -0,0 +1,36 @@
+#pragma once
+#include <cstddef>
+#include <cstdint>
+
+#if defined(__HIPCC__)
+#define UZ_FA_HD __host__ __device__
+#else
+#define UZ_FA_HD
+#endif
+
+#define UZ_FA_PARTS 6
+#define UZ_FA_ALIGN 256
+#define UZ_FA_HEAD_WORDS 8
+
+struct FindAnswerLayout {
+    uint64_t off[UZ_FA_PARTS];
+    uint64_t bytes[UZ_FA_PARTS];
+    uint64_t total;
+};
+
+UZ_FA_HD inline uint64_t uz_fa_up(uint64_t v) { return (v + (UZ_FA_ALIGN - 1)) & ~(uint64_t)(UZ_FA_ALIGN - 1); }
+
+UZ_FA_HD inline FindAnswerLayout uz_find_answer_layout(int64_t n, int64_t n_cand, int64_t n_het) {
+    FindAnswerLayout L;
+    L.bytes[0] = UZ_FA_HEAD_WORDS * sizeof(int64_t);
+    L.bytes[1] = L.bytes[2] = ((uint64_t)n + 1) * sizeof(int64_t);
+    L.bytes[3] = (uint64_t)n_cand * sizeof(int32_t);
+    L.bytes[4] = (uint64_t)n_cand;
+    L.bytes[5] = (uint64_t)n_het * sizeof(int32_t);
+    uint64_t at = 0;
+    for (int k = 0; k < UZ_FA_PARTS; k++) { L.off[k] = at; at += uz_fa_up(L.bytes[k]); }
+    L.total = at;
+    return L;
+}
+UZ_FA_HD inline bool uz_find_answer_fits(const FindAnswerLayout &L, uint64_t block_bytes) { return L.total <= block_bytes; }
+UZ_FA_HD inline bool uz_find_answer_fits_offsets(const FindAnswerLayout &L, uint64_t block_bytes) { return L.off[3] <= block_bytes; }
diff --git a/unfazed_amd/csrc/k_reads.hip b/unfazed_amd/csrc/k_reads.hip
--- a/unfazed_amd/csrc/k_reads.hip
+++ b/unfazed_amd/csrc/k_reads.hip
@@ -35,10 +35,17 @@
     }
     return a;
 }
-__global__ __launch_bounds__(256, UZ_BW_MIN_WAVES) void k_phase_bounds(PhaseArgs a, int32_t *bounds ) {
+struct PhaseClears { int32_t *red; int32_t *cursor; unsigned long long *pool_cursor; int red_words, cursor_words; long long n_het; };
+__global__ __launch_bounds__(256, UZ_BW_MIN_WAVES) void k_phase_bounds(PhaseArgs a, int32_t *bounds , PhaseClears z) {
     constexpr int GL = UZ_BW_LANES, NCH = 2 * UZ_BW_SITES;
     static_assert(GL == 1 || GL == 2 || GL == 4 || GL == 8 || GL == 16 || GL == 32 || GL == 64, "a group is a power of two inside a wavefront");
     __shared__ int32_t s_stage[256 / GL][UZ_BW_STAGE];
+    if (blockIdx.x == 0) {
+        for (int i = threadIdx.x; i < z.red_words; i += 256) z.red[i] = 0;
+        for (int i = threadIdx.x; i < z.cursor_words; i += 256) z.cursor[i] = 0;
+        if (threadIdx.x < 2) z.pool_cursor[threadIdx.x] = 0;
+        if (threadIdx.x == 2) { a.pre_ha[z.n_het] = 0; a.pre_hl[z.n_het] = 0; }
+    }
     const int64_t g = ((int64_t)blockIdx.x * blockDim.x + threadIdx.x) / GL;
     const int lane = threadIdx.x & (GL - 1), gbase = (threadIdx.x & 63) & ~(GL - 1);
     const int d = g < a.n ? (int)g : a.n - 1;
@@ -51,6 +58,10 @@
             b[0] = b[1] = b[4] = 0;
             b[2] = nh; b[3] = nc;
             for (int k = 0; k < 4; k++) a.pre_win[4 * d + k] = 0;
+        }
+        if (nc <= 0 || a.no_extended) {
+            const long long h0 = a.het_off[d];
+            for (int h = lane; h < nh; h += GL) { a.pre_ha[h0 + h] = 0; a.pre_hl[h0 + h] = 0; }
         }
         const RD &R = a.R;
         const int tid = a.rcontig[d];
@@ -151,6 +162,9 @@
     extern __shared__ __attribute__((aligned(16))) uint8_t uz_lds_arena[];
     (void)a_by_value;
     const PhaseArgsK ap = (PhaseArgsK)__builtin_amdgcn_kernarg_segment_ptr();
+    if constexpr (!LDS) {
+        if (*uz_g(ap->src_count) <= 0) return;
+    }
     uint8_t *const scr_base = uz_g(ap->scratch) + (size_t)blockIdx.x * ap->scratch_per_wg;
 #ifdef UZ_PHASE_TIMING
     if (threadIdx.x < 24) sh.tick[threadIdx.x] = 0;
@@ -366,12 +380,18 @@
     st->pre_win.ensure((size_t)4 * n); st->pre_h.ensure(2 * ((size_t)c->n_het + 1));
     a.pre_win = st->pre_win.p; a.pre_ha = st->pre_h.p; a.pre_hl = st->pre_h.p + (size_t)c->n_het + 1;
     st->n_het = c->n_het;
-    UZ_HIP(hipMemsetAsync(st->pre_h.p, 0, 2 * ((size_t)c->n_het + 1) * sizeof(int32_t), c->stream));
+    const size_t res_ints = (size_t)7 * n + ((7 * (size_t)n) & 1);
+    st->res.ensure(res_ints + 4);
+    st->pool_cursor = (unsigned long long *)(st->res.p + res_ints);
+    constexpr int cursor_words = 16 * (UZ_PHASE_PARTS + 2) + 32;
+    st->cursor.ensure(cursor_words);
+    st->bounds_red.ensure(sizeof(BoundsRed) / sizeof(int32_t) + 16);
     {
         const unsigned nb = (unsigned)(((int64_t)n * UZ_BW_LANES + 255) / 256);
+        const PhaseClears z = {st->bounds_red.p, st->cursor.p, st->pool_cursor, (int)(sizeof(BoundsRed) / sizeof(int32_t)), cursor_words, (long long)c->n_het};
         ProfScope ps(c, UZ_K_SIZING);
         UZ_TRACE("k_phase_bounds");
-        hipLaunchKernelGGL(k_phase_bounds, dim3(nb), dim3(256), 0, c->stream, a, st->bounds.p);
+        hipLaunchKernelGGL(k_phase_bounds, dim3(nb), dim3(256), 0, c->stream, a, st->bounds.p, z);
         UZ_HIP(hipGetLastError());
     }
     if (st->bounds_h_cap < sizeof(BoundsRed) / sizeof(int32_t)) {
@@ -380,15 +400,10 @@
         st->bounds_h_cap = sizeof(BoundsRed) / sizeof(int32_t) + 64;
         UZ_HIP(hipHostMalloc((void **)&st->bounds_h, st->bounds_h_cap * sizeof(int32_t), hipHostMallocDefault));
     }
-    st->bounds_red.ensure(sizeof(BoundsRed) / sizeof(int32_t) + 16);
-    UZ_HIP(hipMemsetAsync(st->bounds_red.p, 0, sizeof(BoundsRed), c->stream));
     hipLaunchKernelGGL(k_bounds_reduce, dim3((unsigned)std::max(1, std::min(UZ_BR_BLOCKS, (n + 255) / 256))), dim3(256), 0, c->stream, (const int32_t *)st->bounds.p, n,
                        reinterpret_cast<BoundsRed *>(st->bounds_red.p));
     UZ_HIP(hipGetLastError());
     const BoundsRed *const bh_own = reinterpret_cast<const BoundsRed *>(st->bounds_h);
-    uz_kcopy(c, st->bounds_h, st->bounds_red.p, sizeof(BoundsRed));
-    if (!st->bounds_ready) UZ_HIP(hipEventCreateWithFlags(&st->bounds_ready, hipEventDisableTiming));
-    UZ_HIP(hipEventRecord(st->bounds_ready, c->stream));
     auto check_upload_flags = [&] { uz_check_upload_flag(c); };
     auto exact_sizes = [&](const BoundsRed *bh) { return phase_exact_sizes(bh, n); };
     if (st->n_cus <= 0) {
@@ -400,10 +415,12 @@
     const bool hooks = getenv("UZ_TEST_CAP_T") || getenv("UZ_TEST_PHASE_ARENA");
     bool speculative = st->spec_valid && !no_spec && !hooks && !st->force_exact;
     st->force_exact = false;
-    const size_t res_ints = (size_t)7 * n + ((7 * (size_t)n) & 1);
-    st->res.ensure(res_ints + 4);
-    st->pool_cursor = (unsigned long long *)(st->res.p + res_ints);
-    st->cursor.ensure(16 * (UZ_PHASE_PARTS + 2) + 32);
+    const bool bounds_early = !speculative;
+    if (bounds_early) {
+        uz_kcopy(c, st->bounds_h, st->bounds_red.p, sizeof(BoundsRed));
+        if (!st->bounds_ready) UZ_HIP(hipEventCreateWithFlags(&st->bounds_ready, hipEventDisableTiming));
+        UZ_HIP(hipEventRecord(st->bounds_ready, c->stream));
+    }
     st->retry.ensure(2 * ((size_t)n + 16));
     int32_t *const retry1_list = st->retry.p, *const retry2_list = st->retry.p + (size_t)n + 16;
     int32_t *const retry1 = st->cursor.p + 16 * (UZ_PHASE_PARTS + 2), *const retry2 = retry1 + 16;
@@ -438,7 +455,7 @@
             z.caps = st->spec_caps; z.arena = st->spec_arena; z.arena2 = st->spec_arena2;
             z.sumP = (long long)(st->spec_sumP_per_dnm * (double)n) + 4096;
         } else {
-            UZ_HIP(hipEventSynchronize(st->bounds_ready));
+            if (bounds_early) UZ_HIP(hipEventSynchronize(st->bounds_ready));
             check_upload_flags();
             z = exact_sizes(bh_own);
             if (const char *e = getenv("UZ_TEST_CAP_T")) {
@@ -478,8 +495,10 @@
         st->pool.ensure(pool_cap);
         a.pool = st->pool.p; a.pool_cap = pool_cap;
         for (int attempt = 0; attempt < 4; attempt++) {
-            UZ_HIP(hipMemsetAsync(st->cursor.p, 0, (16 * (UZ_PHASE_PARTS + 2) + 32) * sizeof(int32_t), c->stream));
-            UZ_HIP(hipMemsetAsync(st->pool_cursor, 0, 2 * sizeof(unsigned long long), c->stream));
+            if (round > 0 || attempt > 0) {
+                UZ_HIP(hipMemsetAsync(st->cursor.p, 0, cursor_words * sizeof(int32_t), c->stream));
+                UZ_HIP(hipMemsetAsync(st->pool_cursor, 0, 2 * sizeof(unsigned long long), c->stream));
+            }
             {
                 ProfScope ps(c, UZ_K_PHASE);
                 UZ_TRACE("k_phase");
@@ -501,10 +520,12 @@
             }
             UZ_TRACE("after k_phase");
             *hused = 0;
-            uz_kcopy(c, hres, st->res.p, res_ints * sizeof(int32_t) + sizeof(unsigned long long));
             int32_t *const hretry = (int32_t *)(hused + 1);
             *hretry = 0;
-            uz_kcopy(c, hretry, retry2, sizeof(int32_t));
+            const KCopySeg back[3] = {{hres, st->res.p, res_ints * sizeof(int32_t) + sizeof(unsigned long long)},
+                                      {hretry, retry2, sizeof(int32_t)},
+                                      {st->bounds_h, st->bounds_red.p, speculative ? sizeof(BoundsRed) : 0}};
+            uz_kcopy_many(c, back, 3);
             if (defer && speculative) {
                 st->pending = true;
                 st->pend_caps = caps; st->pend_pool_cap = a.pool_cap; st->pend_want_lists = a.want_lists;
diff --git a/unfazed_amd/csrc/k_sites.hip b/unfazed_amd/csrc/k_sites.hip
--- a/unfazed_amd/csrc/k_sites.hip
+++ b/unfazed_amd/csrc/k_sites.hip
@@ -1,4 +1,5 @@
 #include "uz_ctx.hpp"
+#include "find_answer.hpp"
 
 #include <algorithm>
 #include <cstdlib>
@@ -484,6 +485,67 @@
         for (int k = 0; k < 4; k++) if (i0 + k < n) { v0[k] = c0[i0 + k]; v1[k] = c1[i0 + k]; }
     }
 }
+#define UZ_SCAN2_TILE 2048
+#define UZ_SCAN2_ONE_MAX (16 * UZ_SCAN2_TILE)
+__global__ __launch_bounds__(256) void k_scan2_tile(int32_t n, const int32_t *__restrict__ c0, const int32_t *__restrict__ c1, int64_t *__restrict__ o0,
+                                                    int64_t *__restrict__ o1) {
+    constexpr int IPT = UZ_SCAN2_TILE / 256;
+    static_assert(IPT % 4 == 0 && IPT * 256 == UZ_SCAN2_TILE, "a lane loads whole int4s");
+    __shared__ int wsum[2][4];
+    __shared__ long long csum[2][4];
+    const int t = threadIdx.x, lane = t & 63, wv = t >> 6;
+    const int32_t tile0 = (int32_t)blockIdx.x * UZ_SCAN2_TILE;
+    long long q0 = 0, q1 = 0;
+    {
+        const int4 *__restrict__ a4 = reinterpret_cast<const int4 *>(c0), *__restrict__ b4 = reinterpret_cast<const int4 *>(c1);
+        const int32_t m = tile0 / 4;
+#pragma unroll 8
+        for (int32_t i = t; i < m; i += 256) {
+            const int4 a = a4[i], b = b4[i];
+            q0 += (long long)a.x + a.y + a.z + a.w;
+            q1 += (long long)b.x + b.y + b.z + b.w;
+        }
+    }
+#pragma unroll
+    for (int off = 32; off > 0; off >>= 1) { q0 += __shfl_xor(q0, off, 64); q1 += __shfl_xor(q1, off, 64); }
+    const int32_t i0 = tile0 + IPT * t;
+    int v0[IPT], v1[IPT];
+#pragma unroll
+    for (int k = 0; k < IPT; k += 4) {
+        int w0[4], w1[4];
+        scan2_load(n, i0 + k, c0, c1, w0, w1);
+#pragma unroll
+        for (int j = 0; j < 4; j++) { v0[k + j] = w0[j]; v1[k + j] = w1[j]; }
+    }
+    int s0 = 0, s1 = 0;
+#pragma unroll
+    for (int k = 0; k < IPT; k++) { s0 += v0[k]; s1 += v1[k]; }
+    int in0 = s0, in1 = s1;
+#pragma unroll
+    for (int off = 1; off < 64; off <<= 1) {
+        const int u0 = __shfl_up(in0, off, 64), u1 = __shfl_up(in1, off, 64);
+        if (lane >= off) { in0 += u0; in1 += u1; }
+    }
+    if (lane == 63) { wsum[0][wv] = in0; wsum[1][wv] = in1; }
+    if (lane == 0) { csum[0][wv] = q0; csum[1][wv] = q1; }
+    __syncthreads();
+    int64_t base0 = 0, base1 = 0, pre0 = 0, pre1 = 0, tot0 = 0, tot1 = 0;
+#pragma unroll
+    for (int w = 0; w < 4; w++) {
+        const int a = wsum[0][w], b = wsum[1][w];
+        if (w < wv) { pre0 += a; pre1 += b; }
+        tot0 += a; tot1 += b;
+        base0 += csum[0][w]; base1 += csum[1][w];
+    }
+    int64_t p0 = base0 + pre0 + (in0 - s0), p1 = base1 + pre1 + (in1 - s1);
+#pragma unroll
+    for (int k = 0; k < IPT; k++) {
+        if (i0 + k < n) { o0[i0 + k] = p0; o1[i0 + k] = p1; }
+        p0 += v0[k]; p1 += v1[k];
+    }
+    if (t == 0 && blockIdx.x == gridDim.x - 1) { o0[n] = base0 + tot0; o1[n] = base1 + tot1; }
+}
+
 __global__ __launch_bounds__(1024) void k_scan2_sums(int32_t n, const int32_t *c0, const int32_t *c1, int64_t *part ) {
     __shared__ long long wsum[2][16];
     const int t = threadIdx.x, lane = t & 63, wv = t >> 6;
@@ -1001,6 +1063,7 @@
     int special = 0;
     UZ_HIP(hipMemcpyAsync(&special, flag, sizeof(int), hipMemcpyDeviceToHost, c->stream));
     UZ_HIP(hipStreamSynchronize(c->stream));
+    uz_find_waited(c); uz_find_launched(c, 2);
     c->ab_lut_t0_special = special != 0;
     c->ab_lut_valid = true;
     c->ab_lut_params = c->P;
@@ -1026,6 +1089,7 @@
             const int64_t per = (wgs + n_fam - 1) / n_fam;
             nb = std::max<int64_t>(1, std::min<int64_t>(n_chunks, std::max<int64_t>(per, 16)));
         }
+        uz_find_launched(c, 1);
         hipLaunchKernelGGL(kern, dim3((unsigned)nb, (unsigned)(batch ? n_fam : 1)), dim3(256), 0, c->stream, fp, cls, n, sp,
                            (const int2 *)c->ab_lut.p, (const uint32_t *)(c->ab_lut.p + (size_t)4 * UZ_AB_LUT_N * 2 + 4), batch);
     };
@@ -1047,6 +1111,7 @@
     if (f.n_wide <= 0) return;
     const SiteParams P = make_site_params(c->P);
     const unsigned nb = (unsigned)((f.n_wide + 255) / 256);
+    uz_find_launched(c, 1);
     if (with_cnv) hipLaunchKernelGGL(k_site_scan_wide<true>, dim3(nb), dim3(256), 0, c->stream, fam_ptrs(f), f.cls, f.n_wide, f.wide_site, f.wide_depth, P);
     else hipLaunchKernelGGL(k_site_scan_wide<false>, dim3(nb), dim3(256), 0, c->stream, fam_ptrs(f), f.cls, f.n_wide, f.wide_site, f.wide_depth, P);
     UZ_HIP(hipGetLastError());
@@ -1088,13 +1153,71 @@
     }
 }
 
-void uz_launch_find(uz_ctx *c, FamilyDev &f, const SitesDev &s, int mode, bool host_offsets) {
+struct FindAnswerArgs {
+    uint8_t *block; uint64_t bytes;
+    int32_t n;
+    const int64_t *cand_off, *het_off;
+    const int32_t *cand_idx, *het_idx;
+    const uint8_t *cand_flags;
+    int64_t room_c, room_h;
+};
+template <typename W>
+__device__ __forceinline__ void answer_part(uint8_t *dst, const void *src, uint64_t n) {
+    W *__restrict__ d = (W *)dst;
+    const W *__restrict__ s = (const W *)src;
+    for (uint64_t i = (uint64_t)blockIdx.x * 256 + threadIdx.x; i < n; i += (uint64_t)gridDim.x * 256) d[i] = s[i];
+}
+__global__ __launch_bounds__(256) void k_find_answer(FindAnswerArgs g) {
+    const int64_t nc = g.cand_off[g.n], nh = g.het_off[g.n];
+    const FindAnswerLayout L = uz_find_answer_layout(g.n, nc, nh);
+    const bool fits = nc <= g.room_c && nh <= g.room_h && uz_find_answer_fits(L, g.bytes);
+    if (blockIdx.x == 0 && blockIdx.y == 0 && threadIdx.x < UZ_FA_HEAD_WORDS) {
+        const int64_t head[UZ_FA_HEAD_WORDS] = {nc, nh, fits ? 1 : 0, (int64_t)L.total, g.n, 0, 0, 0};
+        reinterpret_cast<int64_t *>(g.block)[threadIdx.x] = head[threadIdx.x];
+    }
+    if (!fits) return;
+    switch (blockIdx.y) {
+    case 0: answer_part<int64_t>(g.block + L.off[1], g.cand_off, (uint64_t)g.n + 1); break;
+    case 1: answer_part<int64_t>(g.block + L.off[2], g.het_off, (uint64_t)g.n + 1); break;
+    case 2: answer_part<int32_t>(g.block + L.off[3], g.cand_idx, (uint64_t)nc); break;
+    case 3: {
+        const uint64_t words = (uint64_t)nc / 4;
+        answer_part<uint32_t>(g.block + L.off[4], g.cand_flags, words);
+        if (blockIdx.x == 0 && threadIdx.x < (unsigned)((uint64_t)nc - 4 * words)) (g.block + L.off[4])[4 * words + threadIdx.x] = g.cand_flags[4 * words + threadIdx.x];
+        break;
+    }
+    default: answer_part<int32_t>(g.block + L.off[5], g.het_idx, (uint64_t)nh); break;
+    }
+}
+bool uz_launch_find_answer(uz_ctx *c, FindAnswer *ans, int64_t room_c, int64_t room_h) {
+    const int32_t n = c->dn_n_of_find;
+    const FindAnswerLayout L0 = uz_find_answer_layout(n, 0, 0);
+    UZ_REQUIRE(uz_find_answer_fits_offsets(L0, ans->bytes), UZ_E_STATE, "uz_launch_find_answer: a block without room for the offsets");
+    FindAnswerArgs g;
+    g.block = ans->block; g.bytes = ans->bytes; g.n = n;
+    g.cand_off = c->cand_off.p; g.het_off = c->het_off.p; g.cand_idx = c->cand_idx.p; g.het_idx = c->het_idx.p; g.cand_flags = c->cand_flags.p;
+    g.room_c = room_c; g.room_h = room_h;
+    const unsigned nbx = (unsigned)std::max<int64_t>(1, std::min<int64_t>(128, ((int64_t)n * 8 + 255) / 256));
+    hipLaunchKernelGGL(k_find_answer, dim3(nbx, 5), dim3(256), 0, c->stream, g);
+    UZ_HIP(hipGetLastError());
+    uz_find_launched(c, 1);
+    UZ_HIP(hipStreamSynchronize(c->stream));
+    uz_find_waited(c);
+    const int64_t *head = reinterpret_cast<const int64_t *>(ans->block);
+    c->n_cand = head[0]; c->n_het = head[1];
+    if (!c->cand_off_h.empty()) { c->cand_off_h[(size_t)n] = head[0]; c->het_off_h[(size_t)n] = head[1]; }
+    ans->need = (uint64_t)head[3];
+    return head[2] != 0;
+}
+
+void uz_launch_find(uz_ctx *c, FamilyDev &f, const SitesDev &s, int mode, bool host_offsets, FindAnswer *ans) {
     const int32_t n = c->dn.n;
+    c->dn_n_of_find = n;
     c->cnt_c.ensure((size_t)n + 1);
     c->cnt_h.ensure((size_t)n + 1);
     c->cand_off.ensure((size_t)n + 1);
     c->het_off.ensure((size_t)n + 1);
-    if (host_offsets || n <= 0) { c->cand_off_h.assign((size_t)n + 1, 0); c->het_off_h.assign((size_t)n + 1, 0); }
+    if ((host_offsets && !ans) || n <= 0) { c->cand_off_h.assign((size_t)n + 1, 0); c->het_off_h.assign((size_t)n + 1, 0); }
     else { c->cand_off_h.resize((size_t)n + 1); c->het_off_h.resize((size_t)n + 1); }
     c->n_cand = c->n_het = 0;
     if (n > 0) {
@@ -1122,15 +1245,25 @@
                                    (const int64_t *)nullptr, (const int64_t *)nullptr, (int32_t *)nullptr,
                                    (uint8_t *)nullptr, (int32_t *)nullptr);
             UZ_HIP(hipGetLastError());
-            const unsigned tiles = (unsigned)(((int64_t)n + 4095) / 4096);
-            c->scan_part.ensure((size_t)2 * tiles);
-            hipLaunchKernelGGL(k_scan2_sums, dim3(tiles), dim3(1024), 0, c->stream, n, c->cnt_c.p, c->cnt_h.p, c->scan_part.p);
-            UZ_HIP(hipGetLastError());
-            hipLaunchKernelGGL(k_scan2, dim3(tiles), dim3(1024), 0, c->stream, n, c->cnt_c.p, c->cnt_h.p, (const int64_t *)c->scan_part.p, c->cand_off.p,
-                               c->het_off.p);
-            UZ_HIP(hipGetLastError());
+            if (n <= UZ_SCAN2_ONE_MAX) {
+                const unsigned tiles = (unsigned)(((int64_t)n + UZ_SCAN2_TILE - 1) / UZ_SCAN2_TILE);
+                hipLaunchKernelGGL(k_scan2_tile, dim3(tiles), dim3(256), 0, c->stream, n, (const int32_t *)c->cnt_c.p, (const int32_t *)c->cnt_h.p, c->cand_off.p,
+                                   c->het_off.p);
+                UZ_HIP(hipGetLastError());
+                uz_find_launched(c, 2);
+            } else {
+                const unsigned tiles = (unsigned)(((int64_t)n + 4095) / 4096);
+                c->scan_part.ensure((size_t)2 * tiles);
+                hipLaunchKernelGGL(k_scan2_sums, dim3(tiles), dim3(1024), 0, c->stream, n, c->cnt_c.p, c->cnt_h.p, c->scan_part.p);
+                UZ_HIP(hipGetLastError());
+                hipLaunchKernelGGL(k_scan2, dim3(tiles), dim3(1024), 0, c->stream, n, c->cnt_c.p, c->cnt_h.p, (const int64_t *)c->scan_part.p, c->cand_off.p,
+                                   c->het_off.p);
+                UZ_HIP(hipGetLastError());
+                uz_find_launched(c, 3);
+            }
         }
         auto fill = [&](int64_t cap_c, int64_t cap_h) {
+            uz_find_launched(c, 1);
             a.cap_c = cap_c; a.cap_h = cap_h;
             ProfScope ps(c, UZ_K_WINDOW_FILL);
             if (mode & UZ_FIND_WHOLE_REGION)
@@ -1147,25 +1280,34 @@
         if (const char *e = getenv("UZ_TEST_FIND_CAP")) { room_c = std::min<int64_t>(room_c, atoll(e)); room_h = std::min<int64_t>(room_h, atoll(e)); }
         const bool tried = room_c > 0 && room_h > 0;
         if (tried) fill(room_c, room_h);
-        if (host_offsets) {
+        if (ans && tried && uz_find_answer_fits_offsets(uz_find_answer_layout(n, 0, 0), ans->bytes)) {
+            if (!uz_launch_find_answer(c, ans, room_c, room_h) && ans->need > ans->bytes) ans->code |= UZ_FA_BLOCK_SMALL;
+        } else if (host_offsets && !ans) {
             const size_t ob = ((size_t)n + 1) * sizeof(int64_t), obr = (ob + 255) & ~(size_t)255;
             c->find_pin.room(2 * obr);
-            uz_kcopy(c, c->find_pin.p, c->cand_off.p, ob);
-            uz_kcopy(c, c->find_pin.p + obr, c->het_off.p, ob);
+            const KCopySeg offs[2] = {{c->find_pin.p, c->cand_off.p, ob}, {c->find_pin.p + obr, c->het_off.p, ob}};
+            uz_kcopy_many(c, offs, 2);
             UZ_HIP(hipStreamSynchronize(c->stream));
+            uz_find_waited(c);
             memcpy(c->cand_off_h.data(), c->find_pin.p, ob);
             memcpy(c->het_off_h.data(), c->find_pin.p + obr, ob);
         } else {
             int64_t *box = reinterpret_cast<int64_t *>(c->hflags + 4);
-            uz_kcopy(c, box, c->cand_off.p + n, sizeof(int64_t));
-            uz_kcopy(c, box + 1, c->het_off.p + n, sizeof(int64_t));
+            const KCopySeg tots[2] = {{box, c->cand_off.p + n, sizeof(int64_t)}, {box + 1, c->het_off.p + n, sizeof(int64_t)}};
+            uz_kcopy_many(c, tots, 2);
             UZ_HIP(hipStreamSynchronize(c->stream));
+            uz_find_waited(c);
             c->cand_off_h[n] = box[0];
             c->het_off_h[n] = box[1];
+            if (ans) {
+                ans->need = uz_find_answer_layout(n, box[0], box[1]).total;
+                if (ans->need > ans->bytes) ans->code |= UZ_FA_BLOCK_SMALL;
+            }
         }
         c->n_cand = c->cand_off_h[n];
         c->n_het = c->het_off_h[n];
         if (!tried || c->n_cand > room_c || c->n_het > room_h) {
+            if (ans) ans->code |= UZ_FA_GREW_LISTS;
             c->cand_idx.ensure((size_t)c->n_cand + 1);
             c->cand_flags.ensure((size_t)c->n_cand + 1);
             c->het_idx.ensure((size_t)c->n_het + 1);
diff --git a/unfazed_amd/csrc/uz_ctx.hpp b/unfazed_amd/csrc/uz_ctx.hpp
--- a/unfazed_amd/csrc/uz_ctx.hpp
+++ b/unfazed_amd/csrc/uz_ctx.hpp
@@ -322,6 +322,10 @@
     DnmsDev dn;
     uint8_t *dn_stage = nullptr;
     PinBuf find_pin;
+    int64_t find_stat[4] = {0, 0, 0, 0};
+    bool find_counting = false;
+    bool find_answer_again = false;
+    int32_t dn_n_of_find = 0;
     size_t dn_stage_cap = 0;
     hipEvent_t dn_stage_done = nullptr;
     DevBuf<int64_t> scan_part;
@@ -451,6 +455,9 @@
 void uz_block_put(uz_ctx *c, DevBlock b);
 
 void uz_kcopy(uz_ctx *c, void *dst, const void *src, size_t bytes);
+#define UZ_KCOPY_SEGS 4
+struct KCopySeg { void *dst; const void *src; size_t bytes; };
+void uz_kcopy_many(uz_ctx *c, const KCopySeg *segs, int n_segs);
 void uz_len_scan(uz_ctx *c, hipStream_t st, int64_t n, const uint32_t *len, uint32_t add, int64_t *off);
 void uz_reads_make_ready(uz_ctx *c, ReadsDev &r);
 void uz_reads_ready_for_threshold(uz_ctx *c, ReadsDev &r, const char *what);
@@ -472,7 +479,16 @@
                           const uint16_t *gq_in, SamplesDev &m);
 void uz_launch_site_scan(uz_ctx *c, FamilyDev &f, const SitesDev &s, bool with_cnv);
 void uz_launch_site_scan_many(uz_ctx *c, FamilyDev *const *fams, int n_fam, const SitesDev &s, bool with_cnv);
-void uz_launch_find(uz_ctx *c, FamilyDev &f, const SitesDev &s, int mode, bool host_offsets = true);
+struct FindCount {
+    uz_ctx *c;
+    explicit FindCount(uz_ctx *c_) : c(c_) { c->find_counting = true; }
+    ~FindCount() { c->find_counting = false; }
+};
+inline void uz_find_launched(uz_ctx *c, int k) { if (c->find_counting) c->find_stat[1] += k; }
+inline void uz_find_waited(uz_ctx *c) { if (c->find_counting) c->find_stat[0]++; }
+struct FindAnswer { uint8_t *block; size_t bytes; int code; uint64_t need; };
+void uz_launch_find(uz_ctx *c, FamilyDev &f, const SitesDev &s, int mode, bool host_offsets = true, FindAnswer *ans = nullptr);
+bool uz_launch_find_answer(uz_ctx *c, FindAnswer *ans, int64_t room_c, int64_t room_h);
 void uz_stage_dnms(uz_ctx *c, const uz_dnms_view *d);
 void uz_launch_cnv(uz_ctx *c, const SitesDev &s, const int32_t *rb_counts_dev, int32_t *cnv_counts, int32_t *cnv_pos, int32_t *origin,
                    int32_t *evidence, int32_t *etype);
diff --git a/unfazed_amd/engine.py b/unfazed_amd/engine.py
--- a/unfazed_amd/engine.py
+++ b/unfazed_amd/engine.py
@@ -31,7 +31,7 @@
     "uz_pinned_alloc", "uz_pinned_free",
     "uz_sites_adopt_device", "uz_family_adopt_device", "uz_reads_adopt_device",
     "uz_sites_free", "uz_reads_free", "uz_drop_derived",
-    "uz_site_scan", "uz_site_scan_many", "uz_site_classes", "uz_find", "uz_find_fetch", "uz_find_cohort",
+    "uz_site_scan", "uz_site_scan_many", "uz_site_classes", "uz_find", "uz_find_fetch", "uz_find_answer", "uz_find_stats", "uz_find_cohort",
     "uz_phase", "uz_phase_begin", "uz_phase_end", "uz_phase_cohort", "uz_phase_cohort_joined", "uz_phase_votes", "uz_phase_groups", "uz_phase_sizing_fetch", "uz_phase_cnv", "uz_phase_cnv_cohort", "uz_phase_cnv_sites",
     "uz_bed_rows", "uz_bed_rows_lists", "uz_vcf_rows", "uz_bcf_rows", "uz_bgzf_deflate",
     "uz_prof_enable", "uz_prof_reset", "uz_prof_get", "uz_prof_units",
@@ -109,6 +109,8 @@
     L.uz_site_classes.argtypes = [vp, C.c_int, vp]
     L.uz_find.argtypes = [vp, C.c_int, vp, C.c_int, vp, vp]
     L.uz_find_fetch.argtypes = [vp, vp, vp, vp]
+    L.uz_find_answer.argtypes = [vp, C.c_int, vp, C.c_int, vp, C.c_size_t, vp]
+    L.uz_find_stats.argtypes = [vp, vp]
     L.uz_find_cohort.argtypes = [vp, vp, C.c_int32, vp, C.c_int, vp, vp]
     L.uz_phase.argtypes = [vp, C.c_int, C.c_int, vp, C.c_int, vp, vp, vp, vp]
     L.uz_phase_begin.argtypes = [vp, C.c_int, C.c_int, vp, C.c_int]
@@ -616,16 +618,64 @@
 
     def find(self, fam: int, dv: abi.Held, params: abi.Params, mode: int, fetch: bool = True, transient: bool = False):
         self.set_params(params)
-        return self._find_out(dv.view.n, fetch, transient,
+        if transient and fetch:
+            return self._find_answer(int(fam), dv, int(mode))
+        return self._find_out(dv.view.n, fetch,
                               lambda co, ho: self._ck(self.L.uz_find(self.h, int(fam), dv.ref(), int(mode), co, ho), "uz_find"))
 
-    def _find_out(self, n, fetch, transient, run):
+    @staticmethod
+    def find_answer_layout(n: int, nc: int, nh: int):
+        sizes = (64, 8 * (n + 1), 8 * (n + 1), 4 * nc, nc, 4 * nh)
+        off, at = [], 0
+        for b in sizes:
+            off.append(at)
+            at += (b + 255) & ~255
+        return off, at
+
+    def _find_answer(self, fam: int, dv: abi.Held, mode: int, block_bytes: Optional[int] = None):
+        n = dv.view.n
+        if not hasattr(self, "_answer_pins"):
+            self._answer_pins, self._answer_turn, self._answer_hint = [None, None, None], 0, 0
+        self._answer_turn = (self._answer_turn + 1) % 3
+
+        def block(need):
+            pin = self._answer_pins[self._answer_turn]
+            if pin is None or pin[1].size < need:
+                if pin is not None:
+                    pin[0].free_all()
+                pool = PinnedPool()
+                pin = self._answer_pins[self._answer_turn] = (pool, pool.alloc(need + need // 4 + (1 << 16)))
+            return pin[1]
+
+        out = np.zeros(4, dtype=np.int64)
+        first = self.find_answer_layout(n, 0, 0)[1] if block_bytes is None else int(block_bytes)
+        buf = block(max(first, self._answer_hint if block_bytes is None else 0, 256))
+        size = buf.size if block_bytes is None else int(block_bytes)
+        self._ck(self.L.uz_find_answer(self.h, fam, dv.ref(), mode, buf.ctypes.data, size, out.ctypes.data), "uz_find_answer")
+        if out[0] != 0:
+            buf = block(int(out[1]))
+            self._ck(self.L.uz_find_answer(self.h, fam, dv.ref(), mode, buf.ctypes.data, buf.size, out.ctypes.data), "uz_find_answer")
+            if out[0] != 0:
+                raise UnfazedHipError("uz_find_answer: no answer on a block of the size it asked for (%d bytes, code %d)" % (int(out[1]), int(out[0])))
+        self._answer_hint = max(self._answer_hint, int(out[1]) + int(out[1]) // 4)
+        nc, nh = int(out[2]), int(out[3])
+        off, _ = self.find_answer_layout(n, nc, nh)
+        co = buf[off[1]: off[1] + 8 * (n + 1)].view(np.int64)
+        ho = buf[off[2]: off[2] + 8 * (n + 1)].view(np.int64)
+        return co, buf[off[3]: off[3] + 4 * nc].view(np.int32), buf[off[4]: off[4] + nc], ho, buf[off[5]: off[5] + 4 * nh].view(np.int32)
+
+    def find_stats(self):
+        out = np.zeros(4, dtype=np.int64)
+        self._ck(self.L.uz_find_stats(self.h, out.ctypes.data), "uz_find_stats")
+        return tuple(int(x) for x in out)
+
+    def _find_out(self, n, fetch, run):
         co = np.zeros(n + 1, dtype=np.int64)
         ho = np.zeros(n + 1, dtype=np.int64)
         run(co.ctypes.data, ho.ctypes.data)
         if not fetch:
             return co, None, None, ho, None
-        ci, cf, hi = self._fetch(int(co[n]), int(ho[n]), transient=transient)
+        ci, cf, hi = self._fetch(int(co[n]), int(ho[n]))
         return co, ci, cf, ho, hi
 
     @staticmethod
@@ -639,29 +689,13 @@
     def find_cohort(self, groups, dv: abi.Held, params: abi.Params, mode: int, fetch: bool = True):
         self.set_params(params)
         arr = self._groups(groups)
-        return self._find_out(dv.view.n, fetch, False,
+        return self._find_out(dv.view.n, fetch,
                               lambda co, ho: self._ck(self.L.uz_find_cohort(self.h, arr, len(groups), dv.ref(), int(mode), co, ho), "uz_find_cohort"))
 
-    def _fetch(self, nc: int, nh: int, transient: bool = False):
-        if transient:
-            if not hasattr(self, "_find_pins"):
-                self._find_pins, self._find_turn = [None, None, None], 0
-            self._find_turn = (self._find_turn + 1) % 3
-            need = 4 * max(1, nc) + 256 + max(1, nc) + 256 + 4 * max(1, nh) + 256
-            pin = self._find_pins[self._find_turn]
-            if pin is None or pin[1].size < need:
-                if pin is not None:
-                    pin[0].free_all()
-                pool = PinnedPool()
-                pin = self._find_pins[self._find_turn] = (pool, pool.alloc(need + need // 4 + (1 << 16)))
-            buf = pin[1]
-            a = (4 * max(1, nc) + 255) & ~255
-            b = a + ((max(1, nc) + 255) & ~255)
-            ci, cf, hi = buf[: 4 * max(1, nc)].view(np.int32), buf[a: a + max(1, nc)], buf[b: b + 4 * max(1, nh)].view(np.int32)
-        else:
-            ci = np.zeros(max(1, nc), dtype=np.int32)
-            cf = np.zeros(max(1, nc), dtype=np.uint8)
-            hi = np.zeros(max(1, nh), dtype=np.int32)
+    def _fetch(self, nc: int, nh: int):
+        ci = np.zeros(max(1, nc), dtype=np.int32)
+        cf = np.zeros(max(1, nc), dtype=np.uint8)
+        hi = np.zeros(max(1, nh), dtype=np.int32)
         self._ck(self.L.uz_find_fetch(self.h, ci.ctypes.data, cf.ctypes.data, hi.ctypes.data), "uz_find_fetch")
         return ci[:nc], cf[:nc], hi[:nh]
 
```

Result: faster. 13.07 million DNMs/s (median of 6 runs) (+5.5%).
